# iwanders/spread_spectrum_watermarking

Hardware: AMD Instinct MI355X
Metric: Mpixels/sec embed+extract (4K batch) (higher is better)
Workload: dtype f64

## Files before the change

### include/ssw.h

```cpp
#ifndef SSW_H
#define SSW_H

#include <stddef.h>
#include <stdint.h>

#ifdef __cplusplus
extern "C" {
#endif

typedef enum ssw_status {
    SSW_OK = 0,
    SSW_ERR_BAD_ARG = 1,
    SSW_ERR_BAD_DIMS = 2,
    SSW_ERR_LENGTH_MISMATCH = 3,
    SSW_ERR_K_TOO_LARGE = 4,
    SSW_ERR_NOT_BASE = 5,
    SSW_ERR_UNSUPPORTED = 6,
    SSW_ERR_CONSUMED = 7,
    SSW_ERR_HIP = 8,
    SSW_ERR_NO_DEVICE = 9,
    SSW_ERR_OUT_OF_MEMORY = 10
} ssw_status;

typedef enum ssw_ordering {
    SSW_ORDER_ENERGY = 0,
    SSW_ORDER_ENERGY_ORTHOGONAL = 1,
    SSW_ORDER_LEGACY = 2,
    SSW_ORDER_CUSTOM = 3
} ssw_ordering;

typedef enum ssw_method {
    SSW_OPTION1 = 1,
    SSW_OPTION2 = 2,
    SSW_OPTION3 = 3,
    SSW_METHOD_CUSTOM = 4
} ssw_method;

typedef enum ssw_dct_type {
    SSW_DCT2 = 0,
    SSW_DCT2_ORTHOGONAL = 1,
    SSW_DCT3 = 2
} ssw_dct_type;

typedef enum ssw_precision {
    SSW_PRECISION_F32 = 0,
    SSW_PRECISION_F64 = 1
} ssw_precision;

typedef struct ssw_config {
    int32_t ordering;
    int32_t method;
    float alpha;
    int32_t precision;
} ssw_config;

typedef struct ssw_ctx ssw_ctx;
typedef struct ssw_writer ssw_writer;
typedef struct ssw_reader ssw_reader;

const char* ssw_version(void);
int ssw_build_all_strategies(void);
enum { SSW_PLAN_PAIR_F64 = 1, SSW_PLAN_ROWS_DEEP = 2, SSW_PLAN_COLS_DEEP = 4, SSW_PLAN_ROWS_LEVEL2 = 8, SSW_PLAN_COLS_LEVEL2 = 16,
       SSW_PLAN_CLASS_MAJOR = 32, SSW_PLAN_FUSED_COLS = 64 };
int ssw_ctx_transform_plan(ssw_ctx* ctx, size_t n_frames, size_t w, size_t h, int dct_type, uint32_t* flags);
const char* ssw_status_string(int status);
const char* ssw_last_error(void);
void ssw_config_default(ssw_config* cfg);

int ssw_ctx_create(int device_id, ssw_ctx** out);
int ssw_ctx_destroy(ssw_ctx* ctx);
int ssw_ctx_synchronize(ssw_ctx* ctx);
void* ssw_ctx_stream(ssw_ctx* ctx);
int ssw_ctx_set_stream(ssw_ctx* ctx, void* hip_stream);
int ssw_ctx_wait_event(ssw_ctx* ctx, void* hip_event);
int ssw_ctx_record_event(ssw_ctx* ctx, void* hip_event);
int ssw_ctx_set_chunk_frames(ssw_ctx* ctx, size_t frames);
size_t ssw_ctx_pass_frames(ssw_ctx* ctx, size_t n_frames, size_t w, size_t h);

int ssw_ctx_set_overlap(ssw_ctx* ctx, int enable);
int ssw_ctx_set_prune(ssw_ctx* ctx, int enable);
int ssw_ctx_get_prune_stats(ssw_ctx* ctx, uint64_t* stats);
int ssw_ctx_get_select_stats(ssw_ctx* ctx, uint64_t* stats);

#define SSW_DCT_FOLDING_DEFAULT 5
int ssw_ctx_set_dct_folding(ssw_ctx* ctx, int level);
int ssw_ctx_set_odd_split(ssw_ctx* ctx, int enable);

int ssw_tuning_set(const char* name, long long value);
int ssw_tuning_get(const char* name, long long* value);
int ssw_tuning_reset(const char* name);

typedef enum ssw_stage {
    SSW_STAGE_RGB_TO_YIQ = 0,
    SSW_STAGE_DCT_ROW = 1,
    SSW_STAGE_DCT_COL = 2,
    SSW_STAGE_SELECT = 3,
    SSW_STAGE_EMBED = 4,
    SSW_STAGE_EXTRACT = 5,
    SSW_STAGE_SIMILARITY = 6,
    SSW_STAGE_YIQ_TO_RGB = 7,
    SSW_STAGE_RESIZE = 8,
    SSW_STAGE_CONVERT = 9,
    SSW_STAGE_DCT_PREP = 10,
    SSW_STAGE_DCT_ROW_MAIN = 11,
    SSW_STAGE_DCT_COL_MAIN = 12,
    SSW_STAGE_LOCATE = 13,
    SSW_STAGE_LOCATE_COARSE = 14,
    SSW_STAGE_COUNT = 15
} ssw_stage;
int ssw_ctx_enable_timing(ssw_ctx* ctx, int enable);
int ssw_ctx_reset_timing(ssw_ctx* ctx);
int ssw_ctx_get_timing(ssw_ctx* ctx, double* ms, uint64_t* launches);
int ssw_ctx_get_work(ssw_ctx* ctx, double* work);
int ssw_ctx_get_traffic(ssw_ctx* ctx, double* bytes);

int ssw_dev_mem_info(ssw_ctx* ctx, size_t* free_bytes, size_t* total_bytes);
int ssw_dev_alloc(ssw_ctx* ctx, size_t bytes, void** dev_ptr);
int ssw_dev_free(ssw_ctx* ctx, void* dev_ptr);
int ssw_copy_to_dev(ssw_ctx* ctx, void* dev_dst, const void* host_src, size_t bytes);
int ssw_copy_to_host(ssw_ctx* ctx, void* host_dst, const void* dev_src, size_t bytes);

int ssw_host_alloc(ssw_ctx* ctx, size_t bytes, void** host_ptr);
int ssw_host_free(ssw_ctx* ctx, void* host_ptr);
int ssw_ctx_set_copy_threads(ssw_ctx* ctx, int threads);
typedef enum ssw_transfer_stat {
    SSW_TRANSFER_H2D_BYTES = 0,
    SSW_TRANSFER_D2H_BYTES = 1,
    SSW_TRANSFER_H2D_SECONDS = 2,
    SSW_TRANSFER_D2H_SECONDS = 3,
    SSW_TRANSFER_STAGED_BYTES = 4,
    SSW_TRANSFER_DIRECT_BYTES = 5,
    SSW_TRANSFER_STAT_COUNT = 6
} ssw_transfer_stat;
int ssw_ctx_get_transfer_stats(ssw_ctx* ctx, double* stats, int reset);


int ssw_rgb_to_yiq(ssw_ctx* ctx, const float* dev_rgb, size_t n_frames, size_t w, size_t h,
                   float* dev_y, float* dev_i, float* dev_q);
int ssw_yiq_to_rgb(ssw_ctx* ctx, const float* dev_y, const float* dev_i, const float* dev_q,
                   size_t n_frames, size_t w, size_t h, float* dev_rgb);
int ssw_dct2d(ssw_ctx* ctx, int dct_type, int precision, size_t n_frames, size_t w, size_t h,
              float* dev_planes);

int ssw_topk_indices(ssw_ctx* ctx, const float* dev_coef, size_t n_frames, size_t w, size_t h,
                     int ordering, size_t k, uint32_t* dev_indices);

int ssw_embed_coefficients(ssw_ctx* ctx, float* dev_coef, size_t n_frames, size_t plane_len,
                           const uint32_t* dev_indices, size_t k, int method, float alpha,
                           const float* dev_marks, size_t n_marks);
int ssw_extract_coefficients(ssw_ctx* ctx, const float* dev_base, const float* dev_derived,
                             size_t n_frames, size_t plane_len, const uint32_t* dev_indices,
                             size_t k, int method, float alpha, float* dev_out);
int ssw_similarity_batch(ssw_ctx* ctx, const float* dev_extracted, const float* dev_marks,
                         size_t n_pairs, size_t k, float* dev_sims);

int ssw_similarity_matrix(ssw_ctx* ctx, const float* dev_extracted, size_t n_extracted, const float* dev_marks,
                          size_t n_marks, size_t k, float* dev_sims);

int ssw_batch_embed(ssw_ctx* ctx, const ssw_config* cfg, const float* dev_rgb, size_t n_frames,
                    size_t w, size_t h, const float* dev_marks, size_t k, float* dev_rgb_out,
                    float* dev_coef_out, uint32_t* dev_indices_out);
int ssw_batch_extract(ssw_ctx* ctx, const ssw_config* cfg, const float* dev_base_rgb,
                      const float* dev_derived_rgb, size_t n_frames, size_t w, size_t h, size_t k,
                      float* dev_extracted, const float* dev_marks, float* dev_sims);
// ... 113 lines not shown
```

### spread_spectrum_watermarking_amd/_lib.py

```python
from __future__ import annotations

import ctypes as C
import os

_HERE = os.path.dirname(os.path.abspath(__file__))
LIB_PATH = os.environ.get("SSW_LIB_PATH") or os.path.join(_HERE, "lib", "libssw_hip.so")

SSW_OK = 0
STATUS_NAMES = {
    0: "SSW_OK", 1: "SSW_ERR_BAD_ARG", 2: "SSW_ERR_BAD_DIMS", 3: "SSW_ERR_LENGTH_MISMATCH",
    4: "SSW_ERR_K_TOO_LARGE", 5: "SSW_ERR_NOT_BASE", 6: "SSW_ERR_UNSUPPORTED", 7: "SSW_ERR_CONSUMED",
    8: "SSW_ERR_HIP", 9: "SSW_ERR_NO_DEVICE", 10: "SSW_ERR_OUT_OF_MEMORY",
}
(SSW_ERR_BAD_ARG, SSW_ERR_BAD_DIMS, SSW_ERR_LENGTH_MISMATCH, SSW_ERR_K_TOO_LARGE, SSW_ERR_NOT_BASE,
 SSW_ERR_UNSUPPORTED, SSW_ERR_CONSUMED, SSW_ERR_HIP, SSW_ERR_NO_DEVICE, SSW_ERR_OUT_OF_MEMORY) = range(1, 11)

ORDER_ENERGY, ORDER_ENERGY_ORTHOGONAL, ORDER_LEGACY, ORDER_CUSTOM = 0, 1, 2, 3
OPTION1, OPTION2, OPTION3, METHOD_CUSTOM = 1, 2, 3, 4
DCT2, DCT2_ORTHOGONAL, DCT3 = 0, 1, 2
PRECISION_F32, PRECISION_F64 = 0, 1
STAGES = ["rgb_to_yiq", "dct_row", "dct_col", "select", "embed", "extract", "similarity", "yiq_to_rgb",
          "resize", "convert", "dct_prep", "dct_row_main", "dct_col_main", "locate", "locate_coarse"]
DCT_FOLDING_DEFAULT = 5
TRACE_NONE = 0xFFFFFFFF
PLAN_FLAGS = {"pair_f64": 1, "rows_deep": 2, "cols_deep": 4, "rows_level2": 8, "cols_level2": 16, "class_major": 32, "fused_cols": 64}
TRANSFER_STATS = ["h2d_bytes", "d2h_bytes", "h2d_seconds", "d2h_seconds", "staged_bytes", "direct_bytes"]


class Config(C.Structure):
    _fields_ = [("ordering", C.c_int32), ("method", C.c_int32), ("alpha", C.c_float), ("precision", C.c_int32)]


class Placement(C.Structure):
    _fields_ = [("w", C.c_uint32), ("h", C.c_uint32), ("channels", C.c_uint32),
                ("x", C.c_uint32), ("y", C.c_uint32), ("pw", C.c_uint32), ("ph", C.c_uint32)]


class ScaleRange(C.Structure):
    _fields_ = [("wmin", C.c_uint32), ("wmax", C.c_uint32)]


_vp, _f32p, _u32p, _u64p, _sz = C.c_void_p, C.c_void_p, C.c_void_p, C.c_void_p, C.c_size_t
_cfgp = C.POINTER(Config)
_plp = C.POINTER(Placement)

SIGNATURES = {
    "ssw_version": (C.c_char_p, []),
    "ssw_build_all_strategies": (C.c_int, []),
    "ssw_ctx_transform_plan": (C.c_int, [_vp, _sz, _sz, _sz, C.c_int, C.POINTER(C.c_uint32)]),
    "ssw_status_string": (C.c_char_p, [C.c_int]),
    "ssw_last_error": (C.c_char_p, []),
    "ssw_config_default": (None, [_cfgp]),
    "ssw_ctx_create": (C.c_int, [C.c_int, C.POINTER(_vp)]),
    "ssw_ctx_destroy": (C.c_int, [_vp]),
    "ssw_ctx_synchronize": (C.c_int, [_vp]),
    "ssw_ctx_stream": (_vp, [_vp]),
    "ssw_ctx_set_stream": (C.c_int, [_vp, _vp]),
    "ssw_ctx_wait_event": (C.c_int, [_vp, _vp]),
    "ssw_ctx_record_event": (C.c_int, [_vp, _vp]),
    "ssw_ctx_set_chunk_frames": (C.c_int, [_vp, _sz]),
    "ssw_ctx_pass_frames": (_sz, [_vp, _sz, _sz, _sz]),
    "ssw_ctx_set_dct_folding": (C.c_int, [_vp, C.c_int]),
    "ssw_ctx_enable_timing": (C.c_int, [_vp, C.c_int]),
    "ssw_ctx_reset_timing": (C.c_int, [_vp]),
    "ssw_ctx_get_timing": (C.c_int, [_vp, C.POINTER(C.c_double), C.POINTER(C.c_uint64)]),
    "ssw_ctx_get_work": (C.c_int, [_vp, C.POINTER(C.c_double)]),
    "ssw_ctx_get_traffic": (C.c_int, [_vp, C.POINTER(C.c_double)]),
    "ssw_ctx_set_overlap": (C.c_int, [_vp, C.c_int]),
    "ssw_ctx_set_prune": (C.c_int, [_vp, C.c_int]),
    "ssw_ctx_set_odd_split": (C.c_int, [_vp, C.c_int]),
    "ssw_tuning_set": (C.c_int, [C.c_char_p, C.c_longlong]),
    "ssw_tuning_get": (C.c_int, [C.c_char_p, C.POINTER(C.c_longlong)]),
    "ssw_tuning_reset": (C.c_int, [C.c_char_p]),
    "ssw_ctx_get_prune_stats": (C.c_int, [_vp, C.POINTER(C.c_uint64)]),
    "ssw_ctx_get_select_stats": (C.c_int, [_vp, C.POINTER(C.c_uint64)]),
    "ssw_dev_mem_info": (C.c_int, [_vp, C.POINTER(_sz), C.POINTER(_sz)]),
    "ssw_dev_alloc": (C.c_int, [_vp, _sz, C.POINTER(_vp)]),
    "ssw_dev_free": (C.c_int, [_vp, _vp]),
    "ssw_copy_to_dev": (C.c_int, [_vp, _vp, _vp, _sz]),
    "ssw_copy_to_host": (C.c_int, [_vp, _vp, _vp, _sz]),
    "ssw_host_alloc": (C.c_int, [_vp, _sz, C.POINTER(_vp)]),
    "ssw_host_free": (C.c_int, [_vp, _vp]),
    "ssw_ctx_set_copy_threads": (C.c_int, [_vp, C.c_int]),
    "ssw_ctx_get_transfer_stats": (C.c_int, [_vp, C.POINTER(C.c_double), C.c_int]),
    "ssw_rgb_to_yiq": (C.c_int, [_vp, _f32p, _sz, _sz, _sz, _f32p, _f32p, _f32p]),
    "ssw_yiq_to_rgb": (C.c_int, [_vp, _f32p, _f32p, _f32p, _sz, _sz, _sz, _f32p]),
    "ssw_dct2d": (C.c_int, [_vp, C.c_int, C.c_int, _sz, _sz, _sz, _f32p]),
    "ssw_topk_indices": (C.c_int, [_vp, _f32p, _sz, _sz, _sz, C.c_int, _sz, _u32p]),
    "ssw_embed_coefficients": (C.c_int, [_vp, _f32p, _sz, _sz, _u32p, _sz, C.c_int, C.c_float, _f32p, _sz]),
    "ssw_extract_coefficients": (C.c_int, [_vp, _f32p, _f32p, _sz, _sz, _u32p, _sz, C.c_int, C.c_float, _f32p]),
    "ssw_similarity_batch": (C.c_int, [_vp, _f32p, _f32p, _sz, _sz, _f32p]),
    "ssw_similarity_matrix": (C.c_int, [_vp, _f32p, _sz, _f32p, _sz, _sz, _f32p]),
    "ssw_batch_embed": (C.c_int, [_vp, _cfgp, _f32p, _sz, _sz, _sz, _f32p, _sz, _f32p, _f32p, _u32p]),
    "ssw_batch_extract": (C.c_int, [_vp, _cfgp, _f32p, _f32p, _sz, _sz, _sz, _sz, _f32p, _f32p, _f32p]),
    "ssw_convert_rgb8_to_f32": (C.c_int, [_vp, _vp, _sz, _f32p]),
    "ssw_convert_f32_to_rgb8": (C.c_int, [_vp, _f32p, _sz, _vp]),
    "ssw_resize_rgb8": (C.c_int, [_vp, _vp, _sz, _sz, _sz, _sz, _sz, _vp]),
    "ssw_batch_embed_rgb8": (C.c_int, [_vp, _cfgp, _vp, _sz, _sz, _sz, _f32p, _sz, _vp]),
    "ssw_batch_embed_host_rgb8": (C.c_int, [_vp, _cfgp, C.POINTER(_vp), _sz, _sz, _sz, _f32p, _sz, C.POINTER(_vp)]),
    "ssw_batch_extract_host_rgb8": (C.c_int, [_vp, _cfgp, C.POINTER(_vp), C.POINTER(_vp), _sz, _sz, _sz, _sz, _f32p, _f32p, _f32p]),
    "ssw_convert_rgb16_to_f32": (C.c_int, [_vp, _vp, _sz, _f32p]),
    "ssw_convert_f32_to_rgb16": (C.c_int, [_vp, _f32p, _sz, _vp]),
    "ssw_batch_embed_rgb16": (C.c_int, [_vp, _cfgp, _vp, _sz, _sz, _sz, _f32p, _sz, _f32p]),
    "ssw_batch_extract_rgb16": (C.c_int, [_vp, _cfgp, _vp, _vp, _sz, _sz, _sz, _sz, _f32p, _f32p, _f32p]),
    "ssw_batch_extract_rgb8": (C.c_int, [_vp, _cfgp, _vp, _vp, _sz, _sz, _sz, _sz, _f32p, _f32p, _f32p]),
    "ssw_writer_create": (C.c_int, [_vp, _vp, _sz, _sz, _cfgp, C.POINTER(_vp)]),
    "ssw_writer_create_rgb8": (C.c_int, [_vp, _vp, _sz, _sz, _cfgp, C.POINTER(_vp)]),
    "ssw_writer_create_rgb16": (C.c_int, [_vp, _vp, _sz, _sz, _cfgp, C.POINTER(_vp)]),
    "ssw_writer_coefficients": (C.c_int, [_vp, _vp]),
    "ssw_writer_embed": (C.c_int, [_vp, C.POINTER(_vp), C.POINTER(_sz), _sz]),
    "ssw_writer_result": (C.c_int, [_vp, _vp]),
    "ssw_writer_mark": (C.c_int, [_vp, C.POINTER(_vp), C.POINTER(_sz), _sz, _vp]),
    "ssw_writer_result_rgb8": (C.c_int, [_vp, _vp]),
    "ssw_writer_mark_rgb8": (C.c_int, [_vp, C.POINTER(_vp), C.POINTER(_sz), _sz, _vp]),
    "ssw_fingerprint_embed": (C.c_int, [_vp, _cfgp, _f32p, _sz, _sz, _f32p, _sz, _sz, _f32p, _u32p]),
    "ssw_fingerprint_embed_rgb8": (C.c_int, [_vp, _cfgp, _vp, _sz, _sz, _f32p, _sz, _sz, _vp, _u32p]),
    "ssw_fingerprint_trace": (C.c_int, [_vp, _cfgp, _f32p, _f32p, _sz, _sz, _sz, _sz, _f32p, _sz, C.c_float, _f32p, _f32p, _u32p, _f32p, _u32p]),
    "ssw_fingerprint_trace_rgb8": (C.c_int, [_vp, _cfgp, _vp, _vp, _sz, _sz, _sz, _sz, _f32p, _sz, C.c_float, _f32p, _f32p, _u32p, _f32p, _u32p]),
    "ssw_fingerprint_trace_host_rgb8": (C.c_int, [_vp, _cfgp, _vp, C.POINTER(_vp), _sz, _sz, _sz, _sz, _f32p, _sz, C.c_float, _f32p, _f32p, _u32p,
                                                  _f32p, _u32p]),
    "ssw_reader_trace_host_rgb8": (C.c_int, [_vp, C.POINTER(_vp), _sz, _sz, _f32p, _sz, C.c_float, _f32p, _f32p, _u32p, _f32p, _u32p]),
    "ssw_restore_rgb8": (C.c_int, [_vp, _vp, _sz, _sz, C.POINTER(_vp), _plp, _sz, _vp]),
    "ssw_locate_rgb8": (C.c_int, [_vp, _vp, _sz, _sz, C.POINTER(_vp), _plp, _sz, C.POINTER(C.c_uint64)]),
    "ssw_locate_scaled_rgb8": (C.c_int, [_vp, _vp, _sz, _sz, C.POINTER(_vp), _plp, C.POINTER(ScaleRange), _sz, C.POINTER(C.c_uint64)]),
    "ssw_locate_rung_boxes": (C.c_int, [_vp, _vp, _sz, _sz, _sz, _sz, _sz, _vp]),
    "ssw_fingerprint_trace_restored_host_rgb8": (C.c_int, [_vp, _cfgp, _vp, _sz, _sz, C.POINTER(_vp), _plp, _sz, _sz, _f32p, _sz, C.c_float,
                                                           _f32p, _f32p, _u32p, _f32p, _u32p]),
    "ssw_reader_trace_restored_host_rgb8": (C.c_int, [_vp, _vp, C.POINTER(_vp), _plp, _sz, _sz, _f32p, _sz, C.c_float, _f32p, _f32p, _u32p,
                                                      _f32p, _u32p]),
    "ssw_writer_mark_copies": (C.c_int, [_vp, _f32p, _sz, _sz, _vp]),
    "ssw_writer_mark_copies_rgb8": (C.c_int, [_vp, _f32p, _sz, _sz, _vp]),
    "ssw_writer_destroy": (C.c_int, [_vp]),
    "ssw_reader_create": (C.c_int, [_vp, _vp, _sz, _sz, C.c_int, _cfgp, C.POINTER(_vp)]),
    "ssw_reader_create_rgb8": (C.c_int, [_vp, _vp, _sz, _sz, C.c_int, _cfgp, C.POINTER(_vp)]),
    "ssw_reader_create_rgb16": (C.c_int, [_vp, _vp, _sz, _sz, C.c_int, _cfgp, C.POINTER(_vp)]),
    "ssw_reader_coefficients": (C.c_int, [_vp, _vp]),
    "ssw_reader_indices": (C.c_int, [_vp, _sz, _vp]),
    "ssw_reader_extract": (C.c_int, [_vp, _vp, _vp, _sz]),
    "ssw_reader_destroy": (C.c_int, [_vp]),
    "ssw_similarity": (C.c_int, [_vp, _vp, _sz, _vp, _sz, C.POINTER(C.c_float)]),
    "ssw_synth_frames": (C.c_int, [_vp, C.c_uint32, C.c_uint32, _sz, _sz, _sz, _f32p]),
}

_lib = None


class SswLibraryMissing(ImportError):
    pass


def load() -> C.CDLL:
    global _lib
    if _lib is not None:
        return _lib
    if not os.path.exists(LIB_PATH):
        raise SswLibraryMissing(
            f"{LIB_PATH} not found: build it with `python -c 'import __graft_entry__ as g; g.build()'` "
# ... 28 lines not shown
```

### spread_spectrum_watermarking_amd/api.py

```python
from __future__ import annotations

import ctypes as C
import math
from dataclasses import dataclass, field
from typing import Callable, Optional, Sequence, Tuple

import numpy as np

from . import _lib as L
from ._lib import SswError, check


class Context:

    def __init__(self, device_id: int = 0):
        self._lib = L.load()
        h = C.c_void_p()
        check(self._lib.ssw_ctx_create(device_id, C.byref(h)), "ssw_ctx_create")
        self.handle = h
        self.device_id = device_id

    def close(self):
        if getattr(self, "handle", None):
            self._lib.ssw_ctx_destroy(self.handle)
            self.handle = None

    def __del__(self):
        try:
            self.close()
        except Exception:
            pass

    def synchronize(self):
        check(self._lib.ssw_ctx_synchronize(self.handle), "ssw_ctx_synchronize")

    def set_stream(self, hip_stream=None):
        check(self._lib.ssw_ctx_set_stream(self.handle, C.c_void_p(hip_stream) if hip_stream else None), "ssw_ctx_set_stream")

    def wait_event(self, hip_event):
        check(self._lib.ssw_ctx_wait_event(self.handle, C.c_void_p(hip_event)), "ssw_ctx_wait_event")

    def record_event(self, hip_event):
        check(self._lib.ssw_ctx_record_event(self.handle, C.c_void_p(hip_event)), "ssw_ctx_record_event")

    def set_chunk_frames(self, n: int):
        check(self._lib.ssw_ctx_set_chunk_frames(self.handle, n), "ssw_ctx_set_chunk_frames")

    def pass_frames(self, n_frames: int, w: int, h: int) -> int:
        return int(self._lib.ssw_ctx_pass_frames(self.handle, n_frames, w, h))

    def set_dct_folding(self, level=True):
        lvl = (L.DCT_FOLDING_DEFAULT if level else 0) if isinstance(level, bool) else int(level)
        check(self._lib.ssw_ctx_set_dct_folding(self.handle, lvl), "ssw_ctx_set_dct_folding")

    def enable_timing(self, on: bool = True):
        check(self._lib.ssw_ctx_enable_timing(self.handle, int(on)), "ssw_ctx_enable_timing")

    def reset_timing(self):
        check(self._lib.ssw_ctx_reset_timing(self.handle), "ssw_ctx_reset_timing")

    def timing(self) -> dict:
        ms = (C.c_double * len(L.STAGES))()
        n = (C.c_uint64 * len(L.STAGES))()
        work = (C.c_double * len(L.STAGES))()
        check(self._lib.ssw_ctx_get_timing(self.handle, ms, n), "ssw_ctx_get_timing")
        check(self._lib.ssw_ctx_get_work(self.handle, work), "ssw_ctx_get_work")
        traffic = (C.c_double * len(L.STAGES))()
        check(self._lib.ssw_ctx_get_traffic(self.handle, traffic), "ssw_ctx_get_traffic")
        return {s: {"ms": ms[i], "launches": int(n[i]), "work": work[i], "bytes": traffic[i]} for i, s in enumerate(L.STAGES)}

    def transform_plan(self, n_frames: int, w: int, h: int, dct_type: int = L.DCT2) -> dict:
        f = C.c_uint32()
        check(self._lib.ssw_ctx_transform_plan(self.handle, n_frames, w, h, dct_type, C.byref(f)), "ssw_ctx_transform_plan")
        return {name: bool(f.value & bit) for name, bit in L.PLAN_FLAGS.items()}

    def set_overlap(self, on: bool = True):
        check(self._lib.ssw_ctx_set_overlap(self.handle, int(on)), "ssw_ctx_set_overlap")

    def set_prune(self, on: bool = True):
        check(self._lib.ssw_ctx_set_prune(self.handle, int(on)), "ssw_ctx_set_prune")

    def set_odd_split(self, on: bool = True):
        check(self._lib.ssw_ctx_set_odd_split(self.handle, int(on)), "ssw_ctx_set_odd_split")

    def prune_stats(self) -> dict:
        st = (C.c_uint64 * 3)()
        check(self._lib.ssw_ctx_get_prune_stats(self.handle, st), "ssw_ctx_get_prune_stats")
        return {"pruned_chunks": int(st[0]), "redone_chunks": int(st[1]), "columns_needed": int(st[2])}

    def select_stats(self) -> dict:
        st = (C.c_uint64 * 2)()
        check(self._lib.ssw_ctx_get_select_stats(self.handle, st), "ssw_ctx_get_select_stats")
        return {"frames": int(st[0]), "exact_fallback_frames": int(st[1])}

    def set_copy_threads(self, n: int = 0):
        check(self._lib.ssw_ctx_set_copy_threads(self.handle, int(n)), "ssw_ctx_set_copy_threads")

    def transfer_stats(self, reset: bool = False) -> dict:
        st = (C.c_double * len(L.TRANSFER_STATS))()
        check(self._lib.ssw_ctx_get_transfer_stats(self.handle, st, int(reset)), "ssw_ctx_get_transfer_stats")
        return {n: float(st[i]) for i, n in enumerate(L.TRANSFER_STATS)}

    def pinned_empty(self, shape, dtype) -> np.ndarray:
        dt = np.dtype(dtype)
        n = int(np.prod(shape)) * dt.itemsize
        p = C.c_void_p()
        check(self._lib.ssw_host_alloc(self.handle, n, C.byref(p)), "ssw_host_alloc")
        return np.asarray(_PinnedBlock(self, p, n))[:n].view(dt).reshape(shape)

    def mem_info(self):
        free, total = C.c_size_t(), C.c_size_t()
        check(self._lib.ssw_dev_mem_info(self.handle, C.byref(free), C.byref(total)), "ssw_dev_mem_info")
        return int(free.value), int(total.value)

    def alloc(self, nbytes: int) -> "DeviceBuffer":
        return DeviceBuffer(self, nbytes)

    def to_device(self, array: np.ndarray) -> "DeviceBuffer":
        a = np.ascontiguousarray(array)
        buf = DeviceBuffer(self, a.nbytes)
        check(self._lib.ssw_copy_to_dev(self.handle, buf.ptr, a.ctypes.data, a.nbytes), "ssw_copy_to_dev")
        return buf


class _PinnedBlock:

    def __init__(self, ctx: Context, ptr, nbytes: int):
        self.ctx, self.ptr, self.nbytes = ctx, ptr, nbytes
        self.__array_interface__ = {"data": (int(ptr.value), False), "shape": (max(nbytes, 1),), "typestr": "|u1", "version": 3}

    def __del__(self):
        try:
            if self.ptr and self.ctx.handle:
                self.ctx._lib.ssw_host_free(self.ctx.handle, self.ptr)
            self.ptr = None
        except Exception:
            pass


class DeviceBuffer:
    def __init__(self, ctx: Context, nbytes: int):
        self.ctx, self.nbytes = ctx, nbytes
        p = C.c_void_p()
        check(ctx._lib.ssw_dev_alloc(ctx.handle, nbytes, C.byref(p)), "ssw_dev_alloc")
        self.ptr = p

    def to_host(self, dtype, shape) -> np.ndarray:
        out = np.empty(shape, dtype)
        assert out.nbytes <= self.nbytes
        check(self.ctx._lib.ssw_copy_to_host(self.ctx.handle, out.ctypes.data, self.ptr, out.nbytes), "ssw_copy_to_host")
        return out

    def free(self):
        if self.ptr and self.ctx.handle:
            self.ctx._lib.ssw_dev_free(self.ctx.handle, self.ptr)
        self.ptr = None

    def __del__(self):
        try:
            self.free()
        except Exception:
            pass


_default_ctx: Optional[Context] = None


class tuning:

    def __init__(self, **values):
        self._values = values
# ... 644 lines not shown
```

### spread_spectrum_watermarking_amd/csrc/dct_pair_common.hpp

```cpp
#pragma once
#include "dct_common.hpp"
#include "dct_pair_class.hpp"

namespace ssw {

typedef unsigned int u32x4 __attribute__((ext_vector_type(4)));
typedef unsigned int u32x2 __attribute__((ext_vector_type(2)));
typedef unsigned int u32x3 __attribute__((ext_vector_type(3)));
template <typename T> using vec4_t = T __attribute__((ext_vector_type(4)));
template <typename T> using vec2_t = T __attribute__((ext_vector_type(2)));

template <typename T> struct KBlock { static constexpr unsigned KB = 64 / sizeof(T); };
template <typename T>
__host__ __device__ inline size_t blk_index(size_t line, unsigned k, size_t rows) {
    constexpr unsigned KB = KBlock<T>::KB;
    return ((size_t)(k / KB) * rows + line) * KB + (k % KB);
}

template <typename T>
struct PairOutT {
    float* out;
    T* tmp;
    unsigned W, H;
    unsigned n;
    unsigned c1, c2, cs;
    const float* iq_i = nullptr;
    const float* iq_q = nullptr;
    void* rgb = nullptr;
    unsigned rgb_u8 = 0;
    unsigned wide = 0;
    unsigned bn32 = 0;
    unsigned pm = 0;
    unsigned np1 = 0xFFFFFFFFu, p2lo = 0;
    unsigned fold0 = 0;
    T* tmp_out = nullptr;
    unsigned cm = 0;
    unsigned tcm = 0;
    unsigned cmt = 0;
    unsigned ft = 0, gsh = 31, e2off = 0;
    T* cop = nullptr;
    unsigned cop_k16 = 0, cop_lines = 0, cop_hup = 0;
    const double *crot1 = nullptr, *crot2 = nullptr, *crot3 = nullptr;
    unsigned xperm = 0;
};

struct ForwardClassLayout {
    unsigned n, t;
    bool level2;
    enum { R1 = 0, R2, E2P, E2M, O2P, O2M, EP, EM, OP, OM, NCLASS1 };
    enum { R1A = 0, R1B, R2A, R2B, F_E2P, F_E2M, F_O2P, F_O2M, EEP, EEM, EOP, EOM, O5, O11, O3, O13, NCLASS2 };
    __host__ __device__ ForwardClassLayout(unsigned n_, unsigned t_ = 0, bool level2_ = false) : n(n_), t(t_ ? t_ : n_), level2(level2_) {}
    __host__ __device__ int classes() const { return level2 ? (int)NCLASS2 : (int)NCLASS1; }
    __host__ __device__ unsigned mod(int c) const { return level2 ? 16u : ((c >= E2P && c <= O2M) ? 16u : 8u); }
    __host__ __device__ unsigned res(int c) const {
        if (level2) {
            const unsigned char r[16] = {0, 8, 4, 12, 2, 14, 10, 6, 1, 15, 9, 7, 5, 11, 3, 13};
            return r[c & 15];
        }
        const unsigned char r[10] = {0, 4, 2, 14, 10, 6, 1, 7, 5, 3};
        return r[c];
    }
    __host__ __device__ unsigned group(int c) const { return t / mod(c); }
    __host__ __device__ unsigned base(int c) const {
        const unsigned e = t / 8, s = t / 16;
        if (level2) return (unsigned)c * s;
        return c < 2 ? c * e : c < 6 ? 2 * e + (c - 2) * s : t / 2 + (c - 6) * e;
    }
    __host__ __device__ unsigned pos(int c, unsigned i) const {
        const unsigned g = group(c);
        return (i / g) * t + base(c) + i % g;
    }
    __host__ __device__ unsigned natural(unsigned p) const {
        const unsigned e = t / 8, s = t / 16, tb = (p / t) * t;
        p -= tb;
        int c;
        unsigned i;
        if (level2) { c = (int)(p / s); i = p - c * s; }
        else if (p < 2 * e) { c = (int)(p / e); i = p - c * e; }
        else if (p < t / 2) { const unsigned q = p - 2 * e; c = 2 + (int)(q / s); i = q - (q / s) * s; }
        else { const unsigned q = p - t / 2; c = 6 + (int)(q / e); i = q - (q / e) * e; }
        return tb + mod(c) * i + res(c);
    }
};
__host__ __device__ inline unsigned class_tile(unsigned n) { return n % 128 == 0 ? 128u : n; }

__host__ __device__ inline unsigned inverse_class_pos(unsigned m, unsigned len, unsigned t = 0, bool l2 = false) {
    t = t ? t : len;
    const unsigned tb = (m / t) * t, r = m - tb;
    if (l2) {
        const unsigned run = (0x17523460u >> (4 * (r & 7u))) & 7u;
        return tb + run * (t / 8) + (r >> 3);
    }
    const unsigned c = r & 3u, q = t / 4;
    return tb + (c == 0 ? 0u : c == 3 ? q : c == 1 ? 2 * q : 3 * q) + (r >> 2);
}
__host__ __device__ inline unsigned inverse_class_natural(unsigned p, unsigned len, unsigned t = 0, bool l2 = false) {
    t = t ? t : len;
    const unsigned tb = (p / t) * t, r = p - tb;
    if (l2) {
        const unsigned q = t / 8, run = r / q, i = r - run * q;
        return tb + 8 * i + ((0x61523470u >> (4 * run)) & 7u);
    }
    const unsigned q = t / 4, c = r / q, i = r - c * q;
    return tb + 4 * i + (c == 0 ? 0u : c == 1 ? 3u : c == 2 ? 1u : 2u);
}

__device__ inline float pair_clamp01(float x) {
    if (x < 0.0f) return 0.0f;
    if (x > 1.0f) return 1.0f;
    return x;
}
template <typename T, int NB>
__device__ inline void pair_store_rgb_batch(const PairOutT<T>& po, size_t base, const unsigned (&px)[NB], const float (&y)[NB], bool ok) {
    if (!ok) return;
    const float* __restrict__ ip = po.iq_i + base;
    const float* __restrict__ qp = po.iq_q + base;
    float iv[NB], qv[NB];
#pragma unroll
    for (int t = 0; t < NB; ++t) {
        iv[t] = ip[px[t]];
        qv[t] = qp[px[t]];
    }
#pragma unroll
    for (int t = 0; t < NB; ++t) {
        const float r = pair_clamp01(1.0f * y[t] + 0.948262f * iv[t] + 0.624013f * qv[t]);
        const float g = pair_clamp01(1.0f * y[t] + -0.276066f * iv[t] + -0.639810f * qv[t]);
// ... 61 lines not shown
```

### spread_spectrum_watermarking_amd/csrc/dct_pair_f64.hip

```cpp
#include "dct_pair_common.hpp"

#include <cstdlib>
#include <type_traits>

#ifdef SSW_TILE_TRACE
namespace ssw {
__device__ unsigned long long* g_tile_trace = nullptr;
__device__ unsigned int g_tile_trace_cap = 0;
__device__ unsigned int g_tile_trace_n = 0;
__device__ unsigned int* g_tile_kstep = nullptr;
extern "C" int ssw_debug_set_tile_kstep(void* dev_ptr) {
    unsigned int* p = static_cast<unsigned int*>(dev_ptr);
    return hipMemcpyToSymbol(HIP_SYMBOL(g_tile_kstep), &p, sizeof(p)) == hipSuccess ? 0 : -1;
}
extern "C" int ssw_debug_set_tile_trace(void* dev_ptr, unsigned cap) {
    unsigned long long* p = static_cast<unsigned long long*>(dev_ptr);
    unsigned zero = 0;
    if (hipMemcpyToSymbol(HIP_SYMBOL(g_tile_trace), &p, sizeof(p)) != hipSuccess) return -1;
    if (hipMemcpyToSymbol(HIP_SYMBOL(g_tile_trace_cap), &cap, sizeof(cap)) != hipSuccess) return -1;
    if (hipMemcpyToSymbol(HIP_SYMBOL(g_tile_trace_n), &zero, sizeof(zero)) != hipSuccess) return -1;
    return 0;
}
extern "C" int ssw_debug_get_tile_trace_count(unsigned* n) {
    return hipMemcpyFromSymbol(n, HIP_SYMBOL(g_tile_trace_n), sizeof(*n)) == hipSuccess ? 0 : -1;
}
}
#endif
#include "dct_pair_f64_kernel.hpp"
#if defined(SSW_TILE_TRACE) && !defined(SSW_TILE_TRACE_FWD_ONLY)
#define SSW_INV_PART -1
#include "dct_pair_f64_inv.inc"
#endif

namespace ssw {



int launch_dct_pair_gemm_multi_f64(hipStream_t st, bool is_row, bool inverse, int n_classes, const PairClassDesc* desc, float* out,
                                   double* tmp, size_t n_frames, size_t w, size_t h, Epilogue ep, const RgbSink* sink, double* tmp_out,
                                   const PairLayout& lay, const FuseCols* fuse) {
    if (n_frames == 0 || n_classes == 0) return SSW_OK;
    if (n_classes < 0 || n_classes > 8 || !desc) return SSW_ERR_BAD_ARG;
    if (w > 0xFFFFFFull || h > 0xFFFFFFull) return SSW_ERR_BAD_DIMS;
    const bool fuse_rows = fuse && fuse->mode == FUSE_ROWS_COP, fuse_cols = fuse && fuse->mode == FUSE_COLS;
    if (fuse && (!(fuse_rows || fuse_cols) || fuse_rows != is_row || inverse || w % 128 != 0 || h % 16 != 0 ||
                 pair_kpad(h / 8) != dct_pair_fused_units(h))) return SSW_ERR_BAD_ARG;
    if (fuse_rows && (!lay.class_major || sink || !fuse->cop || !fuse->rot1 || !fuse->rot2 || !fuse->rot3)) return SSW_ERR_BAD_ARG;
    const size_t lines = fuse_rows ? n_frames * 16 * dct_pair_fused_units(h) : is_row ? n_frames * h : n_frames * w;
    const size_t len = is_row ? w : h;
    if (lines > 0xFFFFFFFFull) return SSW_ERR_BAD_DIMS;
    const unsigned L = (unsigned)lines;
    const bool with_sink = sink && sink->rgb;
    PairMulti ml;
    PairInstance inst{0, false, 0};
    unsigned tiles_n = 0, leff0 = 0;
    const bool tile48 = tuning(TUNE_TILE48) != 0;
    for (int c = 0; c < n_classes; ++c) {
        PairInstance ic{0, false, 0};
        PairClassArgs& ca = ml.c[c];
        SSW_TRY(pair_class_args(desc[c].cls, is_row, inverse, len, lay, with_sink, tmp_out != nullptr, tile48, ca, ic));
        ca.x1 = desc[c].x1; ca.x2 = desc[c].x2; ca.y1 = desc[c].y1; ca.y2 = desc[c].y2;
        const unsigned ninv = inverse ? (unsigned)(len / pair_class_row(desc[c].cls).inv_ndiv) : 0u;
        if (c == 0) { inst = ic; leff0 = ninv; }
        else if (!(ic == inst) && !(ic.epi == inst.epi && ic.samex == inst.samex && n_classes > 1)) return SSW_ERR_BAD_ARG;
        if (ninv != leff0) return SSW_ERR_BAD_ARG;
        if ((unsigned long long)ml.c[c].Kp * L * 8 > 0xFFFFFFFFull) return SSW_ERR_BAD_DIMS;
        tiles_n += ml.c[c].tiles_n;
    }
    if (n_classes > 1) inst.subname = inverse ? inst.subname : 3;
    const bool small = (unsigned long long)((L + 127) / 128) * tiles_n < 448;
    if (fuse && small) return SSW_ERR_BAD_ARG;
    const unsigned BM = small ? 64 : 128;
    if (small)
        for (int c = 0; c < n_classes; ++c)
            if (ml.c[c].bn32 == 2) { tiles_n -= ml.c[c].tiles_n; ml.c[c].bn32 = 0; ml.c[c].tiles_n = (ml.c[c].NP + 63) / 64; tiles_n += ml.c[c].tiles_n; }
    const unsigned tiles_m = (L + BM - 1) / BM;
    if (small && n_classes == 1) {
        const int force = (int)tuning(TUNE_BN32);
        auto balance = [](unsigned long long n) { return (double)n / (256.0 * (double)((n + 255) / 256)); };
        const unsigned tn32 = (ml.c[0].NP + 31) / 32;
        const bool bn32 = force >= 0 ? force != 0 : 0.92 * balance((unsigned long long)tiles_m * tn32) > balance((unsigned long long)tiles_m * tiles_n);
        if (bn32) { ml.c[0].tiles_n = tiles_n = tn32; ml.c[0].bn32 = 1; }
    }
    const unsigned long long nblk = (unsigned long long)tiles_m * tiles_n;
    if (nblk > 0x7FFFFFFFull) return SSW_ERR_BAD_DIMS;
    ml.n_classes = (unsigned)n_classes; ml.L = L; ml.tiles_m = tiles_m; ml.tiles_n_total = tiles_n;
    PairOut po{out, tmp, (unsigned)w, (unsigned)h, (unsigned)(inverse ? leff0 : len), 0, 1, 2};
    po.tmp_out = tmp_out;
    const PairClass c0 = desc[0].cls;
    if (lay.class_major && inverse && pair_class_row(c0).split && c0 != PairClass::R2A) { po.cm = lay.rows_l2 ? 2u : 1u; po.cmt = lay.tile; }
    if (lay.class_major && inverse && c0 == PairClass::R2A) po.cm = 1;
    if (lay.class_major && inverse && is_row && lay.rows_l2 && (c0 == PairClass::E2 || c0 == PairClass::O2)) po.tcm = 1;
    if (lay.class_major && !inverse) po.ft = lay.tile;
    if (fuse_rows) {
        if (inst.samex || inst.epi != EPI_FWD || po.ft != 128) return SSW_ERR_BAD_ARG;
        po.cop = fuse->cop; po.cop_k16 = (unsigned)pair_kpad(h / 8); po.cop_lines = (unsigned)(n_frames * w);
        po.cop_hup = (unsigned)dct_pair_fused_units(h);
        po.crot1 = fuse->rot1; po.crot2 = fuse->rot2; po.crot3 = fuse->rot3;
        inst.epi = EPI_FWD_COLOP;
    }
    if (fuse_cols) po.xperm = 1;
    auto al = [](const void* p, unsigned a) { return (reinterpret_cast<uintptr_t>(p) & (a - 1)) == 0; };
    po.wide = (!is_row && w % 4 == 0 && al(out, 16) && (n_frames * w) % 4 == 0 && (!tmp || al(tmp, 16)) && (!tmp_out || al(tmp_out, 16))) ? 1u : 0u;
    if (with_sink && !(al(sink->iq_i, 16) && al(sink->iq_q, 16) && al(sink->rgb, sink->u8 ? 4 : 16))) po.wide = 0;
    if (with_sink) {
        if (is_row) return SSW_ERR_BAD_ARG;
        po.iq_i = sink->iq_i; po.iq_q = sink->iq_q; po.rgb = sink->rgb; po.rgb_u8 = sink->u8 ? 1u : 0u;
    }
    ml.po = po;
    switch (inst.epi) {
    case EPI_FWD_COLOP:
        if (inst.subname == 4) SSW_LAUNCH_PAIR_BM(false, EPI_FWD_COLOP, false, 4, 128);
        else SSW_LAUNCH_PAIR_BM(false, EPI_FWD_COLOP, false, 3, 128);
        break;
    case EPI_FWD_ADJ: SSW_LAUNCH_PAIR(false, EPI_FWD_ADJ, false); break;
    case EPI_FWD:
        if (inst.subname == 4) SSW_LAUNCH_PAIR_SUB(false, EPI_FWD, false, 4);
        else if (inst.subname == 3) { if (is_row) SSW_LAUNCH_PAIR_SUB(false, EPI_FWD, false, 3); else SSW_LAUNCH_PAIR_SUB(true, EPI_FWD, false, 3); }
        else if (inst.samex) SSW_LAUNCH_ROWCOL(EPI_FWD, true);
        else SSW_LAUNCH_ROWCOL(EPI_FWD, false);
        break;
    default: return launch_pair_gemm_inverse_instances(st, ml, ep, inst, is_row, small, nblk);
    }
    SSW_HIP_CHECK(hipGetLastError());
    return SSW_OK;
}

int launch_dct_pair_gemm_rows_subset_f64(hipStream_t st, const double* x, const double* y, unsigned cap, unsigned Kp, float* out,
                                         unsigned out_stride, unsigned off, size_t lines) {
    if (lines == 0 || cap == 0) return SSW_OK;
    if (lines > 0xFFFFFFFFull || (cap & 1)) return SSW_ERR_BAD_DIMS;
    const unsigned L = (unsigned)lines, NP = cap / 2;
    const unsigned tiles_m = (L + 127) / 128, tiles_n = (NP + 63) / 64;
    const unsigned long long nblk = (unsigned long long)tiles_m * tiles_n;
    if (nblk > 0x7FFFFFFFull) return SSW_ERR_BAD_DIMS;
    if ((unsigned long long)Kp * L * sizeof(double) > 0xFFFFFFFFull) return SSW_ERR_BAD_DIMS;
    PairMulti ml;
    ml.c[0] = PairClassArgs{x, x, y, y + (size_t)NP * 8, NP, Kp, cap, tiles_n, off, off + NP, 1, 0, 0xFFFFFFFFu, 0, 0, 0};
    ml.n_classes = 1; ml.L = L; ml.tiles_m = tiles_m; ml.tiles_n_total = tiles_n;
    ml.po = PairOut{out, nullptr, out_stride, 0, 0, off, off + NP, 1};
    const Epilogue ep{1.f, 1.f};
    pair_gemm_f64_kernel<false, EPI_FWD, true, 2><<<(unsigned)nblk, PT, 0, st>>>(ml, ep);
    SSW_HIP_CHECK(hipGetLastError());
    return SSW_OK;
}

int launch_dct_pair_gemm_rows_subset_split_f64(hipStream_t st, const double* x1, const double* x2, const double* y1, const double* y2,
                                               unsigned cap, unsigned Kp, float* out, unsigned out_stride, unsigned off, size_t lines) {
    if (lines == 0 || cap == 0) return SSW_OK;
    if (lines > 0xFFFFFFFFull) return SSW_ERR_BAD_DIMS;
    const unsigned L = (unsigned)lines, NP = cap;
    const unsigned tiles_m = (L + 127) / 128, tiles_n = (NP + 63) / 64;
    const unsigned long long nblk = (unsigned long long)tiles_m * tiles_n;
    if (nblk > 0x7FFFFFFFull) return SSW_ERR_BAD_DIMS;
    if ((unsigned long long)Kp * L * sizeof(double) > 0xFFFFFFFFull) return SSW_ERR_BAD_DIMS;
    PairMulti ml;
    ml.c[0] = PairClassArgs{x1, x2, y1, y2, NP, Kp, cap, tiles_n, off, 0, 1, 2, 0xFFFFFFFFu, 0, 0, 0};
    ml.n_classes = 1; ml.L = L; ml.tiles_m = tiles_m; ml.tiles_n_total = tiles_n;
    ml.po = PairOut{out, nullptr, out_stride, 0, 0, off, 0, 1};
    const Epilogue ep{1.f, 1.f};
    pair_gemm_f64_kernel<false, EPI_FWD, false, 3><<<(unsigned)nblk, PT, 0, st>>>(ml, ep);
    SSW_HIP_CHECK(hipGetLastError());
    return SSW_OK;
}

int launch_dct_pair_gemm_rows_subset_merged_f64(hipStream_t st, const PairSubsetClass* classes, unsigned n_classes, float* out,
                                                unsigned out_stride, size_t lines) {
    if (lines == 0) return SSW_OK;
    if (lines > 0xFFFFFFFFull) return SSW_ERR_BAD_DIMS;
    const unsigned L = (unsigned)lines, tiles_m = (L + 127) / 128;
    for (int split = 0; split < 2; ++split) {
        PairMulti ml;
        ml.n_classes = 0; ml.L = L; ml.tiles_m = tiles_m; ml.tiles_n_total = 0;
        auto flush = [&]() -> int {
            if (ml.n_classes == 0) return SSW_OK;
            const unsigned long long nblk = (unsigned long long)tiles_m * ml.tiles_n_total;
            if (nblk > 0x7FFFFFFFull) return SSW_ERR_BAD_DIMS;
            ml.po = PairOut{out, nullptr, out_stride, 0, 0, 0, 0, 1};
            const Epilogue ep{1.f, 1.f};
            if (split) pair_gemm_f64_kernel<false, EPI_FWD, false, 3><<<(unsigned)nblk, PT, 0, st>>>(ml, ep);
            else       pair_gemm_f64_kernel<false, EPI_FWD, true, 2><<<(unsigned)nblk, PT, 0, st>>>(ml, ep);
            SSW_HIP_CHECK(hipGetLastError());
            ml.n_classes = 0; ml.tiles_n_total = 0;
            return SSW_OK;
        };
        for (unsigned c = 0; c < n_classes; ++c) {
            const PairSubsetClass& k = classes[c];
            if ((k.x2 != nullptr) != (split != 0) || k.cap == 0) continue;
            if (!split && (k.cap & 1)) return SSW_ERR_BAD_DIMS;
            if ((unsigned long long)k.Kp * L * sizeof(double) > 0xFFFFFFFFull) return SSW_ERR_BAD_DIMS;
            const unsigned NP = split ? k.cap : k.cap / 2, tiles_n = (NP + 63) / 64;
            if (split) ml.c[ml.n_classes] = PairClassArgs{k.x1, k.x2, k.y1, k.y2, NP, k.Kp, k.cap, tiles_n, k.off, 0, 1, 2, 0xFFFFFFFFu, 0, 0, 0};
            else       ml.c[ml.n_classes] = PairClassArgs{k.x1, k.x1, k.y1, k.y1 + (size_t)NP * 8, NP, k.Kp, k.cap, tiles_n, k.off, k.off + NP, 1, 0, 0xFFFFFFFFu, 0, 0, 0};
            ml.tiles_n_total += tiles_n;
            if (++ml.n_classes == 8) SSW_TRY(flush());
        }
        SSW_TRY(flush());
    }
    return SSW_OK;
}
// ... 3 lines not shown
```

### spread_spectrum_watermarking_amd/csrc/dct_pair_f64_kernel.hpp

```cpp
#pragma once
#include "dct_pair_common.hpp"
#include "dct_pair_colops.hpp"

#include <cstdlib>
#include <type_traits>


namespace ssw {

constexpr int PT = 256;
constexpr int PBK = 8;
constexpr int RGB_NB = 2;

#ifdef SSW_TILE_TRACE
#define SSW_TT(i) do { if (threadIdx.x == 0) tt[i] = wall_clock64(); } while (0)
#define SSW_KT(t) do { if (threadIdx.x == 0 && (t) < 32u) kst_lds[t] = (unsigned)wall_clock64(); } while (0)
#else
#define SSW_TT(i) do { } while (0)
#define SSW_KT(t) do { } while (0)
#endif
typedef PairOutT<double> PairOut;


struct PairMulti {
    PairClassArgs c[8];
    unsigned n_classes, L, tiles_m, tiles_n_total;
    PairOut po;
};

template <bool COLS, int EPI, bool SAMEX, int SUB = 0, int BM = 128>
__global__ __launch_bounds__(PT, 2) void pair_gemm_f64_kernel(const PairMulti ml, Epilogue ep) {
#if defined(__HIP_DEVICE_COMPILE__)
    constexpr int NX = SAMEX ? 1 : 2;
    constexpr int BN = 64, XQ = BM / 64;
    constexpr int STG = NX * BM * PBK + 2 * BN * PBK;
    constexpr int SXD = 2 * STG;
    constexpr int TRD = COLS ? 4 * 32 * (BM / 2 + 16) / 2 : 0;
#ifdef SSW_TILE_TRACE
    __shared__ __attribute__((aligned(16))) double lds[(SXD > TRD ? SXD : TRD) + 16];
    unsigned* kst_lds = reinterpret_cast<unsigned*>(lds + (SXD > TRD ? SXD : TRD));
#else
    __shared__ __attribute__((aligned(16))) double lds[SXD > TRD ? SXD : TRD];
#endif

#ifdef SSW_TILE_TRACE
    unsigned long long tt[5] = {0, 0, 0, 0, 0};
    const unsigned long long cyc0 = clock64();
    unsigned kslot = 0xFFFFFFFFu;
    if (threadIdx.x == 0 && g_tile_trace) kslot = atomicAdd(&g_tile_trace_n, 1u);
#endif
    SSW_TT(0);
    unsigned tm, tn, cls = 0;
    tile_of_block(blockIdx.x, gridDim.x, ml.tiles_m, ml.tiles_n_total, tm, tn);
    while (cls + 1 < ml.n_classes && tn >= ml.c[cls].tiles_n) { tn -= ml.c[cls].tiles_n; ++cls; }
    const PairClassArgs& ca = ml.c[cls];
    const double* __restrict__ X1g = ca.x1;
    const double* __restrict__ X2g = ca.x2;
    const double* __restrict__ Y1g = ca.y1;
    const double* __restrict__ Y2g = ca.y2;
    const unsigned L = ml.L, NP = ca.NP, Kp = ca.Kp, yrows = ca.yrows;
    PairOut po = ml.po;
    po.c1 = ca.c1; po.c2 = ca.c2; po.cs = ca.cs; po.pm = ca.pm; po.np1 = ca.np1; po.p2lo = ca.p2lo; po.bn32 = ca.bn32; po.fold0 = ca.fold0;
    po.gsh = ca.gsh; po.e2off = ca.e2off;
    const unsigned m0 = tm * BM, p0 = tn * (po.bn32 == 1 ? 32u : po.bn32 == 2 ? 48u : (unsigned)BN);
    const unsigned tid = threadIdx.x;
    const unsigned lane = tid & 63, wave = tid >> 6;
    const unsigned li = lane & 15, lq = lane >> 4;

    const unsigned wv = (unsigned)__builtin_amdgcn_readfirstlane((int)wave);
    const unsigned drow = 16 * wave + (lane >> 2), dch = lane & 3;
    unsigned xoff[XQ];
#pragma unroll
    for (int q = 0; q < XQ; ++q) {
        const unsigned j = drow + 64 * q;
        unsigned r = m0 + ((COLS && BM == 128 && po.xperm) ? fwd_cm128_pos(j) : j);
        r = r < L ? r : L - 1;
        xoff[q] = (r - m0) * 64u + 16u * (dch ^ ((j >> 2) & 3u));
    }
    unsigned yr = p0 + drow;
    yr = yr < NP ? yr : NP - 1;
    const unsigned yoff = (yr - p0) * 64u + 16u * (dch ^ ((drow >> 2) & 3u));
#ifdef SSW_ABL_X0
    const size_t m0x = 0;
#else
    const size_t m0x = m0;
#endif
    const __amdgpu_buffer_rsrc_t x1r = __builtin_amdgcn_make_buffer_rsrc((void*)(X1g + m0x * 8), 0, 0xFFFFFFFFu, 0x00020000);
    const __amdgpu_buffer_rsrc_t x2r = __builtin_amdgcn_make_buffer_rsrc((void*)(X2g + m0x * 8), 0, 0xFFFFFFFFu, 0x00020000);
    const __amdgpu_buffer_rsrc_t y1r = __builtin_amdgcn_make_buffer_rsrc((void*)(Y1g + (size_t)p0 * 8), 0, 0xFFFFFFFFu, 0x00020000);
    const __amdgpu_buffer_rsrc_t y2r = __builtin_amdgcn_make_buffer_rsrc((void*)(Y2g + (size_t)p0 * 8), 0, 0xFFFFFFFFu, 0x00020000);
    const unsigned xstep = L * 64u, ystep = yrows * 64u;

    constexpr int LPT = XQ * NX + 2;
    typedef __attribute__((address_space(3))) void* lds_ptr_t;
    auto issue = [&](unsigned t, unsigned sb) {
        const unsigned xadv = t * xstep, yadv = t * ystep;
        double* b = lds + sb + 16 * wv * PBK;
#pragma unroll
        for (int q = 0; q < XQ; ++q) {
            __builtin_amdgcn_raw_ptr_buffer_load_lds(x1r, (lds_ptr_t)(b + 64 * q * PBK), 16, xoff[q], xadv, 0, 0);
            if (!SAMEX) __builtin_amdgcn_raw_ptr_buffer_load_lds(x2r, (lds_ptr_t)(b + BM * PBK + 64 * q * PBK), 16, xoff[q], xadv, 0, 0);
        }
        __builtin_amdgcn_raw_ptr_buffer_load_lds(y1r, (lds_ptr_t)(b + NX * BM * PBK), 16, yoff, yadv, 0, 0);
        __builtin_amdgcn_raw_ptr_buffer_load_lds(y2r, (lds_ptr_t)(b + NX * BM * PBK + BN * PBK), 16, yoff, yadv, 0, 0);
    };
    auto run = [&](auto nic, auto njc) {
    constexpr int NI = decltype(nic)::value;
    constexpr int NJ = decltype(njc)::value;
    constexpr int NJA = NJ < 2 ? 2 : NJ;
    constexpr bool FULL = NI == BM / 32;
    const unsigned wm = FULL ? (wave >> 1) * (BM / 2) : wave * (BM / 4), wn = FULL ? (wave & 1) * 32 : 0;
    f64x4 acc1[NI][NJA], acc2[NI][NJA];
#pragma unroll
    for (int i = 0; i < NI; ++i)
#pragma unroll
        for (int j = 0; j < NJA; ++j) { acc1[i][j] = (f64x4){0, 0, 0, 0}; acc2[i][j] = (f64x4){0, 0, 0, 0}; }

    const unsigned fsw = (li >> 2) & 3;
    unsigned rdx[2], rdy[2];
#pragma unroll
    for (int sh = 0; sh < 2; ++sh) {
        rdx[sh] = (wm + li) * PBK + 2 * ((2 * sh + (lq >> 1)) ^ fsw) + (lq & 1);
        rdy[sh] = NX * BM * PBK + (wn + li) * PBK + 2 * ((2 * sh + (lq >> 1)) ^ fsw) + (lq & 1);
    }
    struct Frag { double x1[NI], x2[NI], y1[NJA], y2[NJA]; };
    auto fread = [&](unsigned sb, auto shc, Frag& f) {
        constexpr int sh = decltype(shc)::value;
        const double* b = lds + sb;
#pragma unroll
        for (int jn = 0; jn < NJ; ++jn) {
            f.y1[jn] = b[rdy[sh] + 16 * jn * PBK];
            f.y2[jn] = b[rdy[sh] + BN * PBK + 16 * jn * PBK];
        }
#pragma unroll
        for (int i = 0; i < NI; ++i) {
            f.x1[i] = b[rdx[sh] + 16 * i * PBK];
            if (!SAMEX) f.x2[i] = b[rdx[sh] + BM * PBK + 16 * i * PBK];
// ... 109 lines not shown
                    double s = a1 + a2, d = a1 - a2;
                    if (jn == 0 && has0) {
                        const bool p = COLS ? (lq == 0 && r == 0) : (li == 0);
                        s = p ? a1 : s;
                        d = p ? 0.0 - a2 : d;
                    }
                    acc1[i][jn][r] = s;
                    acc2[i][jn][r] = d;
                }
    }
    const bool second_out = po.pm != 2;
    auto p2 = [&](unsigned pair) { return (po.fold0 && pair == 0) ? po.fold0 : pair; };

    const unsigned n = po.n, W = po.W, H = po.H;
    auto opos = [&](unsigned m, unsigned len) { return (!COLS && po.cm) ? inverse_class_pos(m, len, 0, po.cm == 2) : m; };
    auto tpos = [&](unsigned m) { return (!COLS && po.tcm) ? inverse_class_pos(m, n / 2, 0, false) : m; };
    auto oposf = [&](unsigned m, unsigned len) { return (!COLS && po.cm) ? inverse_class_pos(m, len, po.cmt, po.cm == 2) : m; };
    auto fpos1 = [&](unsigned pair) {
        return po.ft ? po.c1 + (pair >> po.gsh) * po.ft + (pair & ((1u << po.gsh) - 1u)) : po.c1 + po.cs * pair;
    };
    auto fpos2 = [&](unsigned pair) {
        const unsigned q = p2(pair), e = q - po.e2off;
        return po.ft ? po.c2 + (e >> po.gsh) * po.ft + (e & ((1u << po.gsh) - 1u)) : po.c2 + po.cs * q;
    };
    auto emit = [&](float* lp, double* tp, double* to, unsigned es, unsigned pair, double a1, double a2) {
        if (EPI == EPI_FWD || EPI == EPI_FWD_ADJ) {
            const unsigned i1 = fpos1(pair), i2 = fpos2(pair);
            if (EPI == EPI_FWD_ADJ) {
                const f32x2 v = {apply_epilogue(ep, (float)a1, i1), apply_epilogue(ep, (float)a2, i2)};
                *reinterpret_cast<f32x2*>(lp + i1) = v;
            } else {
                if (pair < po.np1) lp[i1 * es] = apply_epilogue(ep, (float)a1, i1);
                if (pair >= po.p2lo && second_out) lp[i2 * es] = apply_epilogue(ep, (float)a2, i2);
            }
        } else if (EPI == EPI_INV) {
            lp[pair * es] = apply_epilogue(ep, (float)(a1 + a2), pair);
            lp[(n - 1 - pair) * es] = apply_epilogue(ep, (float)(a1 - a2), n - 1 - pair);
        } else if (EPI == EPI_INV_E) {
            tp[pair * es] = a1 + a2;
            tp[(n / 2 - 1 - pair) * es] = a1 - a2;
        } else if (EPI == EPI_INV_OT) {
            const unsigned n1 = po.c1 + po.cs * pair, n2 = po.c2 + po.cs * p2(pair);
            if (n1 < n / 2) { const double e1 = tp[tpos(n1) * es]; to[opos(n1, n) * es] = e1 + a1; to[opos(n - 1 - n1, n) * es] = e1 - a1; }
            if (n2 < n / 2) { const double e2 = tp[tpos(n2) * es]; to[opos(n2, n) * es] = e2 + a2; to[opos(n - 1 - n2, n) * es] = e2 - a2; }
        } else {
            const unsigned n1 = po.c1 + po.cs * pair, n2 = po.c2 + po.cs * p2(pair);
            if (n1 < n / 2) {
                const double e1 = tp[opos(n1, n / 2) * es];
                lp[oposf(n1, n) * es] = apply_epilogue(ep, (float)(e1 + a1), n1);
                lp[oposf(n - 1 - n1, n) * es] = apply_epilogue(ep, (float)(e1 - a1), n - 1 - n1);
            }
            if (n2 < n / 2) {
                const double e2 = tp[opos(n2, n / 2) * es];
                lp[oposf(n2, n) * es] = apply_epilogue(ep, (float)(e2 + a2), n2);
                lp[oposf(n - 1 - n2, n) * es] = apply_epilogue(ep, (float)(e2 - a2), n - 1 - n2);
            }
        }
    };
    if constexpr (!COLS && EPI == EPI_FWD_COLOP) {
        constexpr int NIT = 32 * NJ, NC = (NIT + 63) / 64;
        constexpr int NPT = FULL ? 64 : 16 * NJ, NLT = 2 * NPT;
        static_assert(4 * NIT * 16 * 4 <= (int)sizeof(lds) && 4 * NLT * 64 <= (int)sizeof(lds), "transpose area, store slabs");
        static_assert(BM == 128, "a tile is one k-block of eight units");
        __syncthreads();
        float* tw = reinterpret_cast<float*>(lds) + wave * (NIT * 16);
        auto lds_order = [&]() {
            __builtin_amdgcn_fence(__ATOMIC_RELEASE, "wavefront");
            __builtin_amdgcn_wave_barrier();
            __builtin_amdgcn_fence(__ATOMIC_ACQUIRE, "wavefront");
        };
        const unsigned Hc = po.H, HU = Hc / 16;
        const unsigned tpf = po.cop_hup / 8;
        const unsigned z = tm / tpf, g = tm - z * tpf;
        const unsigned u0 = (unsigned)__builtin_amdgcn_readfirstlane((int)(wm / 16));
        const bool plain = ep.first == 1.0f && ep.base == 1.0f;
        auto lpos = [&](unsigned f, unsigned v) { return f * 16u + 4u * ((v >> 2) ^ ((f >> 2) & 3u)) + (v & 3u); };
        float f1[NJ], f2[NJ];
#pragma unroll
        for (int jn = 0; jn < NJ; ++jn) {
            const unsigned pair = p0 + wn + 16 * jn + li;
            f1[jn] = fpos1(pair) == 0 ? ep.first : ep.base;
            f2[jn] = fpos2(pair) == 0 ? ep.first : ep.base;
        }
        double o[NC][NI][16];
#pragma unroll
        for (int i = 0; i < NI; ++i) {
            lds_order();
#pragma unroll
            for (int jn = 0; jn < NJ; ++jn)
#pragma unroll
                for (int r = 0; r < 4; ++r) {
                    float v1 = (float)acc1[i][jn][r], v2 = (float)acc2[i][jn][r];
                    if (!plain) { v1 *= f1[jn]; v2 *= f2[jn]; }
                    tw[lpos(32 * jn + li, lq + 4 * r)] = v1;
                    tw[lpos(32 * jn + 16 + li, lq + 4 * r)] = v2;
                }
            lds_order();
            const unsigned e = (unsigned)__builtin_amdgcn_readfirstlane((int)(8 * g + u0 + i));
            const bool unit_ok = e < HU;
            const ColL2Tab tab = col_l2_tab(po.crot1, po.crot2, po.crot3, unit_ok ? e : 0u, Hc);
#pragma unroll
            for (int c = 0; c < NC; ++c) {
                const unsigned f = (lane + 64 * c) < (unsigned)NIT ? lane + 64 * c : 0u;
                float x[16];
#pragma unroll
                for (int q = 0; q < 4; ++q) {
                    const f32x4 t4 = *reinterpret_cast<const f32x4*>(tw + lpos(f, 4 * q));
                    x[4 * q] = t4[0]; x[4 * q + 1] = t4[1]; x[4 * q + 2] = t4[2]; x[4 * q + 3] = t4[3];
                }
                col_l2_unit(x, tab, o[c][i]);
                if (!unit_ok) {
#pragma unroll
                    for (int a = 0; a < 16; ++a) o[c][i][a] = 0.0;
                }
            }
        }
        double* slab = lds;
        unsigned tl[NC];
#pragma unroll
        for (int c = 0; c < NC; ++c) {
            const unsigned f = lane + 64 * c, pl = wn + 16 * (f >> 5) + (f & 15u);
            tl[c] = f < (unsigned)NIT ? 16u * (pl >> 3) + 8u * ((f >> 4) & 1u) + (pl & 7u) : 0u;
        }
        constexpr int NSW = (NLT * 4 + 255) / 256;
        bool st_ok[NSW];
        size_t st_off[NSW];
        unsigned st_lds[NSW];
#pragma unroll
        for (int j = 0; j < NSW; ++j) {
            const unsigned idx = tid + 256 * j, T = idx >> 2, p4 = idx & 3u;
            const unsigned pl = ((T >> 4) << 3) | (T & 7u), pair = p0 + pl;
            const bool second = ((T >> 3) & 1u) != 0;
            st_ok[j] = T < (unsigned)NLT && pair < NP && (second ? (pair >= po.p2lo && second_out) : pair < po.np1);
            const unsigned mc = st_ok[j] ? (second ? fpos2(pair) : fpos1(pair)) : 0u;
            st_off[j] = ((size_t)g * po.cop_lines + (size_t)z * po.W + mc) * 8u + 2u * p4;
            st_lds[j] = (T < (unsigned)NLT ? T : 0u) * 8u + 2u * (p4 ^ ((T >> 2) & 3u));
        }
        const size_t pstride = (size_t)po.cop_lines * po.cop_k16;
#pragma unroll
        for (int rnd = 0; rnd < 4; ++rnd) {
            __syncthreads();
#pragma unroll
            for (int c = 0; c < NC; ++c) {
                if ((lane + 64 * c) >= (unsigned)NIT) continue;
#pragma unroll
                for (int a = 0; a < 4; ++a)
#pragma unroll
                    for (int i = 0; i < NI; i += 2) {
                        const unsigned ch = ((u0 + i) >> 1) ^ ((tl[c] >> 2) & 3u);
                        *reinterpret_cast<f64x2*>(slab + (a * NLT + tl[c]) * 8 + 2 * ch) = (f64x2){o[c][i][4 * rnd + a], o[c][i + 1][4 * rnd + a]};
                    }
            }
            __syncthreads();
#pragma unroll
            for (int j = 0; j < NSW; ++j) {
                if (!st_ok[j]) continue;
#pragma unroll
                for (int a = 0; a < 4; ++a) {
                    const f64x2 v = *reinterpret_cast<const f64x2*>(slab + a * NLT * 8 + st_lds[j]);
                    *reinterpret_cast<f64x2*>(po.cop + (size_t)(4 * rnd + a) * pstride + st_off[j]) = v;
                }
            }
        }
        trace_end();
        return;
    }
    if constexpr (!COLS && (EPI == EPI_FWD || EPI == EPI_INV_O || EPI == EPI_INV_OT)) {
        const unsigned rows_valid = L - m0 < (unsigned)BM ? L - m0 : (unsigned)BM;
        const unsigned long long region = (unsigned long long)rows_valid * W * 4ull;
        if (region < 0x80000000ull && (EPI == EPI_FWD || (EPI == EPI_INV_O && n == W) || EPI == EPI_INV_OT)) {
            constexpr unsigned OOB = 0x80000000u;
            const bool plain = ep.first == 1.0f && ep.base == 1.0f;
            const __amdgpu_buffer_rsrc_t orr = __builtin_amdgcn_make_buffer_rsrc((void*)(po.out + (size_t)m0 * W), 0, (unsigned)region, 0x00020000);
            const unsigned swm = __builtin_amdgcn_readfirstlane(wm);
            auto st = [&](float v, unsigned voff, unsigned soff) {
                __builtin_amdgcn_raw_buffer_store_b32(__float_as_uint(v), orr, voff, soff, 0);
            };
            if constexpr (EPI == EPI_FWD) {
                unsigned vo1[NJ], vo2[NJ];
                float f1[NJ], f2[NJ];
#pragma unroll
                for (int jn = 0; jn < NJ; ++jn) {
                    const unsigned pair = p0 + wn + 16 * jn + li;
                    const unsigned i1 = fpos1(pair), i2 = fpos2(pair);
                    vo1[jn] = (pair < NP && pair < po.np1) ? (lq * W + i1) * 4u : OOB;
                    vo2[jn] = (pair < NP && pair >= po.p2lo && second_out) ? (lq * W + i2) * 4u : OOB;
                    f1[jn] = i1 == 0 ? ep.first : ep.base;
                    f2[jn] = i2 == 0 ? ep.first : ep.base;
                }
#pragma unroll
                for (int i = 0; i < NI; ++i)
#pragma unroll
                    for (int r = 0; r < 4; ++r) {
                        const unsigned soff = (swm + 16 * i + 4 * r) * W * 4u;
#pragma unroll
                        for (int jn = 0; jn < NJ; ++jn) {
                            float v1 = (float)acc1[i][jn][r], v2 = (float)acc2[i][jn][r];
                            if (!plain) { v1 *= f1[jn]; v2 *= f2[jn]; }
                            st(v1, vo1[jn], soff);
                            st(v2, vo2[jn], soff);
                        }
                    }
            } else if constexpr (EPI == EPI_INV_OT) {
                const unsigned tregion = rows_valid * n * 8u;
                const __amdgpu_buffer_rsrc_t irr = __builtin_amdgcn_make_buffer_rsrc((void*)(po.tmp + (size_t)m0 * (n / 2)), 0, tregion / 2, 0x00020000);
                const __amdgpu_buffer_rsrc_t trr = __builtin_amdgcn_make_buffer_rsrc((void*)(po.tmp_out + (size_t)m0 * n), 0, tregion, 0x00020000);
                unsigned vt[NJ][2], vp[NJ][2], vm[NJ][2];
#pragma unroll
                for (int jn = 0; jn < NJ; ++jn) {
                    const unsigned pair = p0 + wn + 16 * jn + li;
#pragma unroll
                    for (int h2 = 0; h2 < 2; ++h2) {
                        const unsigned nn = h2 ? po.c2 + po.cs * p2(pair) : po.c1 + po.cs * pair;
                        const bool ok = pair < NP && nn < n / 2;
                        vt[jn][h2] = ok ? (lq * (n / 2) + tpos(nn)) * 8u : OOB;
                        vp[jn][h2] = ok ? (lq * n + opos(nn, n)) * 8u : OOB;
                        vm[jn][h2] = ok ? (lq * n + opos(n - 1 - nn, n)) * 8u : OOB;
                    }
                }
                auto std64 = [&](double v, unsigned voff, unsigned soff) {
                    const u32x2 raw = {(unsigned)__double2loint(v), (unsigned)__double2hiint(v)};
                    __builtin_amdgcn_raw_buffer_store_b64(raw, trr, voff, soff, 0);
                };
                auto load_e = [&](int i, double (&e)[4][NJ][2]) {
// ... 450 lines not shown
```

### spread_spectrum_watermarking_amd/csrc/select.hip

```cpp
#include "ssw_internal.hpp"
#include "embed_fn.hpp"

#include <atomic>

#include <type_traits>

namespace ssw {

typedef float f32x4 __attribute__((ext_vector_type(4)));

constexpr int DIGIT_BITS = 11;
constexpr int NBINS = 1 << DIGIT_BITS;
constexpr size_t MAX_K = 16384;
constexpr unsigned SAMPLE_STRIDE = 64, SAMPLE_STRIDE_MID = 128, SAMPLE_STRIDE_LONG = 256;
static inline unsigned sample_stride_for(size_t k) { return k >= 8192 ? SAMPLE_STRIDE_LONG : k >= 4096 ? SAMPLE_STRIDE_MID : SAMPLE_STRIDE; }
constexpr unsigned FINISH_THREADS = 1024;

size_t select_max_k() { return MAX_K; }
size_t select_cand_capacity(size_t k) { size_t c = 16 * k; return c < 65536 ? 65536 : c; }

struct KeyParams {
    int ordering;
    unsigned w;
    float s[2][2];
// ... 326 lines not shown
            base = __shfl(base, __builtin_ctzll(m), 64);
            const unsigned pos = base + (unsigned)__popcll(m & ((1ull << lane) - 1ull));
            if (keep && pos < n_pow2) lbuf[pos] = comp;
        };
        walk(take);
        __syncthreads();
        const unsigned gathered = (unsigned)lstate[4];
        for (unsigned i = tid; i < n_pow2; i += blockDim.x)
            if (i >= gathered) lbuf[i] = 0ull;
        __syncthreads();
    }
    if (n_pow2 <= blockDim.x) {
        const unsigned N = blockDim.x;
        uint64_t v = tid < n_pow2 ? lbuf[tid] : 0ull;
        __syncthreads();
        for (unsigned size = 2; size <= N; size <<= 1) {
            const bool up = (tid & size) == 0;
            for (unsigned stride = size >> 1; stride > 0; stride >>= 1) {
                uint64_t other;
                if (stride >= 64) {
                    lbuf[tid] = v;
                    __syncthreads();
                    other = lbuf[tid ^ stride];
                    __syncthreads();
                } else {
                    const uint32_t lo = __shfl_xor((uint32_t)v, (int)stride, 64);
                    const uint32_t hi = __shfl_xor((uint32_t)(v >> 32), (int)stride, 64);
                    other = ((uint64_t)hi << 32) | lo;
                }
                const bool lower = (tid & stride) == 0;
                const uint64_t mx = v > other ? v : other, mn = v > other ? other : v;
                v = (lower == up) ? mx : mn;
            }
        }
        if (tid < k) indices[tid] = ~(uint32_t)(v & 0xFFFFFFFFull);
        return;
    }
    if (blockDim.x == FINISH_THREADS && n_pow2 <= 16 * FINISH_THREADS) {
        const unsigned gathered = (unsigned)lstate[4] < n_pow2 ? (unsigned)lstate[4] : n_pow2;
        const unsigned rows = (gathered + FINISH_THREADS - 1) / FINISH_THREADS;
        block_radix_sort_desc(lbuf, rows, reinterpret_cast<uint16_t*>(lhist), lpart, 0);
        for (unsigned i = tid; i < k; i += blockDim.x) indices[i] = ~(uint32_t)(lbuf[i] & 0xFFFFFFFFull);
        return;
    }
    for (unsigned size = 2; size <= n_pow2; size <<= 1) {
        for (unsigned stride = size >> 1; stride > 0; stride >>= 1) {
            for (unsigned i = tid; i < n_pow2 / 2; i += blockDim.x) {
                const unsigned lo = 2 * i - (i & (stride - 1));
                const unsigned hi = lo + stride;
                const bool desc = ((lo & size) == 0);
                const uint64_t a = lbuf[lo], b = lbuf[hi];
                if ((a < b) == desc) { lbuf[lo] = b; lbuf[hi] = a; }
            }
            __syncthreads();
        }
    }
    for (unsigned i = tid; i < k; i += blockDim.x) indices[i] = ~(uint32_t)(lbuf[i] & 0xFFFFFFFFull);
}

__global__ __launch_bounds__(FINISH_THREADS) void select_finish_kernel(
    const float* __restrict__ coef, size_t plane_len, KeyParams kp, uint32_t* __restrict__ ctrl,
    uint32_t* __restrict__ hist, const uint64_t* __restrict__ cand, size_t cap, size_t k, unsigned n_pow2,
    uint32_t* __restrict__ indices, uint32_t* __restrict__ fallbacks) {
    extern __shared__ __attribute__((aligned(16))) unsigned char smem_raw[];
    uint64_t* lbuf = reinterpret_cast<uint64_t*>(smem_raw);
    uint64_t* lstate = lbuf + (n_pow2 > blockDim.x ? n_pow2 : blockDim.x);
    uint32_t* lhist = reinterpret_cast<uint32_t*>(lstate + 8);
    uint32_t* lpart = lhist + NBINS;
    const size_t f = blockIdx.x;
    const uint32_t n = ctrl[f * 4 + 1];
    __syncthreads();
    for (unsigned i = threadIdx.x; i < NBINS; i += blockDim.x) hist[f * NBINS + i] = 0;
    if (threadIdx.x == 0) { ctrl[f * 4 + 0] = 0; ctrl[f * 4 + 1] = 0; }
    if (n >= k && n <= cap) {
        CandSource src{cand + f * cap};
        block_select_sort(src, n, k, n_pow2, lhist, lpart, lbuf, lstate, indices + f * k);
    } else {
        if (threadIdx.x == 0 && fallbacks) atomicAdd(fallbacks, 1u);
        PlaneSource src{coef + f * plane_len, kp};
        block_select_sort(src, plane_len - 1, k, n_pow2, lhist, lpart, lbuf, lstate, indices + f * k);
    }
}

int launch_topk(hipStream_t st, const float* coef, size_t n_frames, size_t w, size_t h, int ordering,
                size_t k, const SelectWorkspace& ws, uint32_t* indices) {
    const size_t plane_len = w * h;
    if (n_frames == 0 || k == 0) return SSW_OK;
    if (plane_len > 0xFFFFFFFFull) return SSW_ERR_BAD_DIMS;
    if (k > plane_len - 1) return SSW_ERR_K_TOO_LARGE;
    if (k > MAX_K) return SSW_ERR_UNSUPPORTED;
    if (ws.frames < n_frames || ws.cap < select_cand_capacity(k)) return SSW_ERR_BAD_ARG;
    if (ordering < SSW_ORDER_ENERGY || ordering > SSW_ORDER_LEGACY) return SSW_ERR_UNSUPPORTED;

    KeyParams kp;
    kp.ordering = ordering;
    kp.w = (unsigned)w;
    {
        const float s_k0_w = sqrtf(1.0f / (4.0f * (float)w));
        const float s_k0_h = sqrtf(1.0f / (4.0f * (float)h));
        const float s_w = sqrtf(1.0f / (2.0f * (float)w));
        const float s_h = sqrtf(1.0f / (2.0f * (float)h));
        for (int fr = 0; fr < 2; ++fr)
            for (int fc = 0; fc < 2; ++fc) {
                volatile float sc = 1.0f;
                sc = sc * (fr ? s_k0_w : s_w);
                sc = sc * (fc ? s_k0_h : s_h);
                kp.s[fr][fc] = sc;
            }
    }
    const unsigned stride_s = sample_stride_for(k);
    const size_t groups = (plane_len + stride_s * 4 - 1) / (stride_s * 4);
    size_t sb = (groups + 256 * 2 - 1) / (256 * 2);
    if (sb < 1) sb = 1;
    if (sb > 256) sb = 256;

    uint32_t m = (uint32_t)((3 * k + stride_s - 1) / stride_s);
    if (m < 32) m = 32;
    select_sample_kernel<<<dim3((unsigned)sb, (unsigned)n_frames), 256, 0, st>>>(coef, plane_len, kp, ws.hist, stride_s);
    size_t bpf = (plane_len + 256 * 32 - 1) / (256 * 32);
    if (bpf < 1) bpf = 1;
    if (bpf > 2048) bpf = 2048;
    if (ordering == SSW_ORDER_ENERGY)
        select_compact_kernel<true><<<dim3((unsigned)bpf, (unsigned)n_frames), 256, 0, st>>>(coef, plane_len, kp, ws.ctrl, ws.hist, m, ws.cand, ws.cap);
    else
        select_compact_kernel<false><<<dim3((unsigned)bpf, (unsigned)n_frames), 256, 0, st>>>(coef, plane_len, kp, ws.ctrl, ws.hist, m, ws.cand, ws.cap);
    unsigned n_pow2 = 2;
    while (n_pow2 < k) n_pow2 <<= 1;
    const size_t smem = (size_t)(n_pow2 > FINISH_THREADS ? n_pow2 : FINISH_THREADS) * sizeof(uint64_t) + 8 * sizeof(uint64_t) +
                        (NBINS + 256) * sizeof(uint32_t);
    constexpr size_t LDS_LIMIT = 160 * 1024;
    {
        static std::atomic<bool> attr_set[64];
        int dev = 0;
        SSW_HIP_CHECK(hipGetDevice(&dev));
        if (dev < 0 || dev >= 64 || !attr_set[dev].load(std::memory_order_acquire)) {
            SSW_HIP_CHECK(hipFuncSetAttribute(reinterpret_cast<const void*>(select_finish_kernel),
                                              hipFuncAttributeMaxDynamicSharedMemorySize, (int)LDS_LIMIT));
            if (dev >= 0 && dev < 64) attr_set[dev].store(true, std::memory_order_release);
        }
    }
    select_finish_kernel<<<(unsigned)n_frames, FINISH_THREADS, smem, st>>>(coef, plane_len, kp, ws.ctrl, ws.hist,
                                                                            ws.cand, ws.cap, k, n_pow2, indices, ws.fallbacks);
    SSW_HIP_CHECK(hipGetLastError());
    return SSW_OK;
}

__device__ inline float extract_fn(int method, float alpha, float base, float derived) {
    if (method == SSW_OPTION1) return (derived - base) / alpha;
    if (method == SSW_OPTION2) return (derived - base) / (base * alpha);
    return logf(derived / base) / alpha;
}

__global__ __launch_bounds__(256) void embed_kernel(float* __restrict__ coef, size_t plane_len,
                                                    const uint32_t* __restrict__ indices, size_t idx_stride,
                                                    const float* __restrict__ marks,
                                                    const uint32_t* __restrict__ mark_offsets,
                                                    const uint32_t* __restrict__ mark_lens, size_t n_marks,
                                                    size_t max_len, size_t mark_stride, int method, float alpha) {
    const size_t f = blockIdx.y;
    const size_t i = blockIdx.x * (size_t)blockDim.x + threadIdx.x;
    if (i >= max_len) return;
    const uint32_t j = indices[f * idx_stride + i];
    float* c = coef + f * plane_len + j;
    const float original = *c;
    if (n_marks == 1) {
        const size_t off = mark_offsets ? mark_offsets[f] : f * mark_stride;
        const size_t len = mark_lens ? mark_lens[f] : max_len;
        if (i < len) *c = insert_fn(method, alpha, original, marks[off + i]);
    } else {
        float cur = original;
        for (size_t m = 0; m < n_marks; ++m) {
            const size_t off = mark_offsets ? mark_offsets[f * n_marks + m] : (f * n_marks + m) * mark_stride;
            const size_t len = mark_lens ? mark_lens[f * n_marks + m] : max_len;
            if (i < len) {
                const float updated = insert_fn(method, alpha, original, marks[off + i]);
                const float change = updated - original;
                cur += change;
            }
        }
        *c = cur;
    }
}

int launch_embed(hipStream_t st, float* coef, size_t n_frames, size_t plane_len,
                 const uint32_t* indices, size_t idx_stride, const float* marks,
                 const uint32_t* mark_offsets, const uint32_t* mark_lens, size_t n_marks,
                 size_t max_len, size_t mark_stride, int method, float alpha) {
    if (n_frames == 0 || n_marks == 0 || max_len == 0) return SSW_OK;
    const dim3 grid((unsigned)((max_len + 255) / 256), (unsigned)n_frames);
    embed_kernel<<<grid, 256, 0, st>>>(coef, plane_len, indices, idx_stride, marks, mark_offsets,
                                       mark_lens, n_marks, max_len, mark_stride, method, alpha);
    SSW_HIP_CHECK(hipGetLastError());
// ... 242 lines not shown
```

### spread_spectrum_watermarking_amd/csrc/ssw_host.hpp

```cpp
#pragma once

#include <functional>
#include <vector>

#include "ssw_internal.hpp"

namespace ssw {
namespace host {

struct DeviceGuard {
    int prev = -1, dev;
    explicit DeviceGuard(int d) : dev(d) {
        if (hipGetDevice(&prev) != hipSuccess) prev = -1;
        if (prev != dev) (void)hipSetDevice(dev);
    }
    ~DeviceGuard() {
        if (prev >= 0 && prev != dev) (void)hipSetDevice(prev);
    }
    DeviceGuard(const DeviceGuard&) = delete;
    DeviceGuard& operator=(const DeviceGuard&) = delete;
};

struct CtxGuard {
    DeviceGuard dg;
    ssw_ctx* prev;
    explicit CtxGuard(ssw_ctx* ctx);
    ~CtxGuard();
};
size_t plane_pool_flush(ssw_ctx* ctx);

int dev_malloc(void** p, size_t bytes);
#define SSW_ALLOC(pp, bytes) SSW_TRY(::ssw::host::dev_malloc((void**)(pp), (bytes)))
int grow(ssw_ctx::Buf& b, size_t bytes);
void release(ssw_ctx::Buf& b);
int grow_select(hipStream_t st, SelectWorkspace& s, size_t frames, size_t k);
void release_select(SelectWorkspace& s);

int upload(ssw_ctx* ctx, void* dev_dst, const void* host_src, size_t bytes, hipStream_t st);
int download(ssw_ctx* ctx, void* host_dst, const void* dev_src, size_t bytes, hipStream_t st);
int upload_nowait(ssw_ctx* ctx, void* dev_dst, const void* host_src, size_t bytes, hipStream_t st, bool* async_out);
int download_nowait(ssw_ctx* ctx, void* host_dst, const void* dev_src, size_t bytes, hipStream_t st, bool* async_out);
void transfer_destroy(ssw_ctx* ctx);
int transfer_set_threads(ssw_ctx* ctx, int threads);
int transfer_stats(ssw_ctx* ctx, double* out, bool reset);

struct StageTimer {
    ssw_ctx* ctx;
    int stage;
    hipStream_t st;
    hipEvent_t a = nullptr, b = nullptr;
    bool armed = false;
    int alias = -1;
    StageTimer(ssw_ctx* c, int s, hipStream_t stream, double work = 0.0, int alias_stage = -1);
    ~StageTimer();
    void traffic(double bytes);
    StageTimer(const StageTimer&) = delete;
    StageTimer& operator=(const StageTimer&) = delete;
};
int flush_timers(ssw_ctx* ctx);
inline void untimed_work(ssw_ctx* ctx) { if (ctx) ctx->tail_fresh = false; }

int get_basis(ssw_ctx* ctx, size_t n, bool inverse, bool f64, BasisKind kind, const void** out);

bool valid_method(int m);
bool valid_ordering(int o);
bool valid_precision(int p);
int check_config(const ssw_config* cfg);
size_t effective_chunk(const ssw_ctx* ctx, size_t w, size_t h, size_t n_frames);

struct Stage {
    bool hbm;
    std::function<int(hipStream_t)> run;
    int tag = 0;
};
typedef std::vector<Stage> Chain;

struct Xform {
    int type, precision;
    size_t n, w, h;
    float* data;
    float* tmp;
    const void* rgb = nullptr;
    int rgb_u8 = 0;
    float* iq_i = nullptr;
    float* iq_q = nullptr;
    void* rgb_out = nullptr;
    bool rgb_out_u8 = false;
    size_t full_h = 0;
    bool natural_order = false;
};
int build_transform(ssw_ctx* ctx, ssw_ctx::Lane& ws, const Xform& x, Chain& ch, bool* fused_rgb = nullptr);
bool can_fuse_rgb(const ssw_ctx* ctx, bool f64, size_t w, size_t h, const float* y, const float* tmp, const void* rgb, int u8);
int build_forward_from_rgb(ssw_ctx* ctx, ssw_ctx::Lane& ws, int precision, const void* rgb, int u8, size_t n, size_t w,
                           size_t h, float* y, float* i, float* q, float* tmp, Chain& ch);
bool can_split_forward_rows(const ssw_ctx* ctx, bool f64, size_t w, size_t h, size_t bands, const float* y, const float* tmp, const void* rgb, int u8);
int build_forward_rows_band(ssw_ctx* ctx, ssw_ctx::Lane& ws, int precision, const void* rgb, int u8, size_t w, size_t rows,
                            size_t frame_h, float* tmp, float* i, float* q, Chain& ch);
int build_forward_cols_after_rows(ssw_ctx* ctx, ssw_ctx::Lane& ws, int precision, size_t w, size_t h, float* tmp, float* y, Chain& ch);
int run_serial(Chain& ch, hipStream_t st);
int dct2d_planes(ssw_ctx* ctx, int type, int precision, size_t n, size_t w, size_t h, float* data, float* tmp);

int topk(ssw_ctx* ctx, hipStream_t st, SelectWorkspace& sel, const float* coef, size_t n, size_t w, size_t h, int ordering,
         size_t k, uint32_t* idx);

int batch_embed_impl(ssw_ctx* ctx, const ssw_config* cfg, const void* dev_rgb, int u8_in, size_t n_frames, size_t w,
                     size_t h, const float* dev_marks, size_t k, void* dev_rgb_out, bool u8_out, float* dev_coef_out,
                     uint32_t* dev_indices_out);
int batch_extract_impl(ssw_ctx* ctx, const ssw_config* cfg, const void* dev_base_rgb, const void* dev_derived_rgb, int u8,
                       size_t n_frames, size_t w, size_t h, size_t k, float* dev_extracted, const float* dev_marks,
                       float* dev_sims);

int trace_base(ssw_ctx* ctx, const ssw_config& c, const void* dev_base_rgb, int u8, size_t w, size_t h, size_t k, const float** y,
               const uint32_t** idx);
int trace_extract(ssw_ctx* ctx, const ssw_config& c, const float* base_y, const uint32_t* base_idx, const void* dev_suspect_rgb, int u8,
                  size_t n_frames, size_t w, size_t h, size_t k, float* dev_extracted);
int trace_check_args(const ssw_ctx* ctx, const ssw_config* cfg, size_t w, size_t h, size_t k, const void* marks, size_t n_marks,
                     const void* sims, const void* best, const void* best_sim, const void* n_exceed);
int trace_score(ssw_ctx* ctx, const float* dev_extracted, size_t n_suspects, const float* dev_marks, size_t n_marks, size_t k,
                float threshold, float* dev_sims, uint32_t* dev_best, float* dev_best_sim, uint32_t* dev_n_exceed);
int stream_trace_rgb8(ssw_ctx* ctx, const ssw_config& c, const float* base_y, const uint32_t* base_idx, const uint8_t* const* host_suspects,
                      size_t n_suspects, size_t w, size_t h, size_t k, const float* host_marks, size_t n_marks, float threshold,
                      float* host_extracted, float* host_sims, uint32_t* host_best, float* host_best_sim, uint32_t* host_n_exceed,
                      const ssw_placement* placements = nullptr, const uint8_t* dev_base = nullptr);

struct RestoreJob { const uint8_t* src; uint8_t* out; ssw_placement p; };
bool restore_untouched(const ssw_placement& p, size_t w, size_t h);
bool restore_reads_base(const ssw_placement& p, size_t w, size_t h);
int restore_normalise(const ssw_placement* pl, size_t n, size_t w, size_t h, std::vector<ssw_placement>* out);
int restore_prepare(ssw_ctx* ctx, const std::vector<ssw_placement>& pl);
int restore_enqueue(ssw_ctx* ctx, const uint8_t* dev_base, size_t w, size_t h, const RestoreJob* jobs, size_t n);
struct LocWindow { uint32_t x0, x1, y0, y1; bool share; };
int locate_impl(ssw_ctx* ctx, const uint8_t* dev_base, size_t w, size_t h, const void* const* dev_suspects,
                const std::vector<ssw_placement>& pl, uint64_t* host_res, const std::vector<LocWindow>* win = nullptr);
int get_taps(ssw_ctx* ctx, size_t in_len, size_t out_len, DeviceTaps* out);

int fingerprint_copies(ssw_ctx* ctx, const ssw_config& c, const float* coef, const uint32_t* idx, size_t k_eff, const float* iq_i,
                       const float* iq_q, size_t w, size_t h, const float* marks, size_t mark_stride, size_t n_copies, void* out,
                       bool u8_out, float* t32);

int extract_single_pruned(ssw_ctx* ctx, int precision, const void* derived_rgb, int u8, size_t w, size_t h, const float* base_y,
                          const uint32_t* idx, size_t k, int method, float alpha, float* dev_out, uint32_t** dev_info,
                          bool* applicable);

}
}
```

### spread_spectrum_watermarking_amd/csrc/ssw_internal.hpp

```cpp
#pragma once

#include <hip/hip_runtime.h>

#include <cstddef>
#include <cstdint>
#include <map>
#include <string>
#include <tuple>
#include <utility>
#include <vector>

#include "../../include/ssw.h"
#include "dct_plan.hpp"
#include "dct_pair_class.hpp"

namespace ssw {

void set_last_error(const std::string& s);

#define SSW_HIP_CHECK(expr)                                                              \
    do {                                                                                 \
        hipError_t e__ = (expr);                                                         \
        if (e__ != hipSuccess) {                                                         \
            ::ssw::set_last_error(std::string(#expr) + ": " + hipGetErrorString(e__));   \
            return (e__ == hipErrorOutOfMemory) ? SSW_ERR_OUT_OF_MEMORY : SSW_ERR_HIP;   \
        }                                                                                \
    } while (0)

#define SSW_TRY(expr)                         \
    do {                                      \
        int s__ = (expr);                     \
        if (s__ != SSW_OK) return s__;        \
    } while (0)


int launch_rgb_to_yiq(hipStream_t st, const float* rgb, size_t npix, float* y, float* i, float* q);
int launch_yiq_to_rgb(hipStream_t st, const float* y, const float* i, const float* q, size_t npix,
                      float* rgb);
int launch_synth(hipStream_t st, uint32_t seed, uint32_t first_frame, size_t n_frames, size_t w,
                 size_t h, float* rgb);

size_t dense_basis_kpad(size_t n);
int launch_make_basis_f32(hipStream_t st, size_t n, bool inverse, float* out);
int launch_make_basis_f64(hipStream_t st, size_t n, bool inverse, double* out);

struct Epilogue {
    float first, base;
};
int launch_dct_rows(hipStream_t st, int precision, const float* in, float* out, size_t rows, size_t w,
                    const void* basis, Epilogue ep);
int launch_dct_cols(hipStream_t st, int precision, const float* in, float* out, size_t n_frames,
                    size_t w, size_t h, const void* basis, Epilogue ep);
int launch_dct_rows_f64out(hipStream_t st, const float* in, double* out, size_t rows, size_t w, const double* basis);
int launch_dct_cols_f64out(hipStream_t st, const float* in, double* out, size_t n_frames, size_t w, size_t h, const double* basis);

size_t dct_pair_kpad(size_t n);
size_t dct_pair_operand_elems(size_t n_frames, size_t w, size_t h);
int launch_make_half_basis_blocked(hipStream_t st, size_t n, bool inverse, int parity, double* out);
int launch_dct_pair_prep(hipStream_t st, bool is_row, bool inverse, const float* in, size_t n_frames, size_t w, size_t h,
                         double* o1, double* o2);
int launch_dct_pair_prep4(hipStream_t st, bool is_row, bool inverse, const float* in, size_t n_frames, size_t w, size_t h,
                          double* q1, double* q2, double* p);
enum { SSW_PIX_F32 = 0, SSW_PIX_U8 = 1, SSW_PIX_U16 = 2 };
inline size_t pix_bytes(int fmt) { return fmt == SSW_PIX_U8 ? 1 : fmt == SSW_PIX_U16 ? 2 : 4; }
inline unsigned pix_align_mask(int fmt) { return fmt == SSW_PIX_U8 ? 3u : fmt == SSW_PIX_U16 ? 7u : 15u; }
inline int pix_src_kind(int fmt) { return fmt + 1; }
int launch_dct_pair_prep4_rows_rgb(hipStream_t st, int u8, const void* rgb, size_t n_frames, size_t w, size_t h,
                                   double* q1, double* q2, double* p, float* ip, float* qp);
int launch_dct_pair_prep8_rows(hipStream_t st, int src_kind, const void* src, size_t n_frames, size_t w, size_t h,
                               double* r1, double* r2, double* m, double* p, float* ip, float* qp);
struct RgbSink {
    const float* iq_i = nullptr;
    const float* iq_q = nullptr;
    void* rgb = nullptr;
    bool u8 = false;
};
int launch_dct_pair_prep8_cols(hipStream_t st, const float* in, size_t n_frames, size_t w, size_t h,
                               double* r1, double* r2, double* m, double* p);
enum { FUSE_ROWS_COP = 1, FUSE_COLS = 2 };
struct FuseCols { int mode = 0; double* cop = nullptr; const double *rot1 = nullptr, *rot2 = nullptr, *rot3 = nullptr; };
struct PairClassDesc { PairClass cls; const double *x1, *x2, *y1, *y2; };
int launch_dct_pair_gemm_multi_f64(hipStream_t st, bool is_row, bool inverse, int n_classes, const PairClassDesc* desc, float* out,
                                   double* tmp, size_t n_frames, size_t w, size_t h, Epilogue ep, const RgbSink* sink = nullptr,
                                   double* tmp_out = nullptr, const PairLayout& layout = PairLayout(), const FuseCols* fuse = nullptr);

int launch_dct_pair_gemm_rows_subset_f64(hipStream_t st, const double* x, const double* y, unsigned cap, unsigned Kp, float* out,
                                         unsigned out_stride, unsigned off, size_t lines);
int launch_dct_pair_gemm_rows_subset_split_f64(hipStream_t st, const double* x1, const double* x2, const double* y1, const double* y2,
                                               unsigned cap, unsigned Kp, float* out, unsigned out_stride, unsigned off, size_t lines);
struct PairSubsetClass {
    const double *x1, *x2, *y1, *y2;
    unsigned cap, Kp, off;
};
int launch_dct_pair_gemm_rows_subset_merged_f64(hipStream_t st, const PairSubsetClass* classes, unsigned n_classes, float* out,
                                                unsigned out_stride, size_t lines);
size_t dct_pair_split_kpad(size_t len);
enum { TUNE_EFOLD_MIN, TUNE_EFOLD_INV_MIN, TUNE_EFOLD_COLS_MIN, TUNE_CLASS_TILE, TUNE_DEEP_MIN_ROWS, TUNE_DEEP_MIN_COLS, TUNE_PREP_STAGED,
       TUNE_MERGE_MAX_LINES, TUNE_BN32, TUNE_BAND_SPLIT, TUNE_FUSE_COLS, TUNE_UPLOAD_BANDS, TUNE_SPECULATE_K, TUNE_PREP_LIGHT, TUNE_LANE_STAGGER, TUNE_DERIVED_FUSED, TUNE_TILE48, TUNE_COUNT };
long long tuning(int which);
int launch_prep16_cols_l2(hipStream_t st, const float* in, size_t n_frames, size_t w, size_t h, double* base,
                          const double* rot1, const double* rot2, const double* rot3, bool class_major, bool in_l2, unsigned K16);
int launch_prep16_inv_cols_l2(hipStream_t st, const float* in, size_t n_frames, size_t w, size_t h, double* base,
                              const double* rot1, const double* rot2, const double* rot3, bool class_major, bool in_l2, unsigned K16);
int launch_prep16_cols_staged(hipStream_t st, const float* in, size_t n_frames, size_t w, size_t h, double* base,
                              const double* rot1, const double* rot2, bool class_major, bool semi, unsigned K8, unsigned K16, bool efold);
int launch_prep16_inv_cols_staged(hipStream_t st, const float* in, size_t n_frames, size_t w, size_t h, double* base,
                                  const double* rot1, const double* rot2, bool class_major, bool semi, unsigned K8, unsigned K16, bool l2);
int launch_prep16_inv_rows_l2(hipStream_t st, const float* in, size_t rows, size_t w, double* base,
                              const double* rot1, const double* rot2, const double* rot3, unsigned K16);
int launch_prep16_inv_rows_staged(hipStream_t st, const float* in, size_t rows, size_t w, double* base,
                                  const double* rot1, const double* rot2, unsigned K8, unsigned K16);
size_t dct_pair_split_elems(size_t n_frames, size_t w, size_t h);
size_t dct_pair_split_basis_rows(size_t len, int which);
int launch_make_split_basis_blocked(hipStream_t st, size_t n, bool inverse, int which, double* out);
int launch_make_rot_table(hipStream_t st, size_t n, double* out);
int launch_dct_pair_rotate(hipStream_t st, const double* p, const double* rot, double* sp, size_t lines, size_t len);
size_t dct_pair_semi_deep_elems(size_t lines, size_t len);
int launch_dct_pair_prep16_inv_rows(hipStream_t st, const float* in, size_t n_frames, size_t w, size_t h, double* base,
                                    const double* rot1, const double* rot2, const double* rot3, PrepFamily prep);
int launch_dct_pair_prep16_inv_cols(hipStream_t st, const float* in, size_t n_frames, size_t w, size_t h, double* base,
                                    const double* rot1, const double* rot2, const double* rot3, PrepFamily prep, const PairLayout& lay);
int launch_dct_pair_prep16_cols(hipStream_t st, const float* in, size_t n_frames, size_t w, size_t h, double* base,
                                const double* rot1, const double* rot2, const double* rot3, PrepFamily prep, const PairLayout& lay);
size_t dct_pair_deep_elems(size_t lines, size_t len);
int launch_dct_pair_prep16_rows(hipStream_t st, int src_kind, const void* src, size_t n_frames, size_t w, size_t h, double* base,
                                const double* rot1, const double* rot2, const double* rot3, float* ip, float* qp, bool l2, bool unit_order = false);
inline size_t dct_pair_fused_units(size_t h) { return ((h / 16 + 7) / 8) * 8; }

constexpr unsigned PRUNE_NO_REM = 0xFFFFFFFFu;
constexpr uint32_t PRUNE_NEG = 0x40000000u;
constexpr unsigned SSW_PRUNE_INFO = 16;
struct PruneClass { unsigned mod, rem, cap, off, rem2 = PRUNE_NO_REM, radd = 0; };
struct PrunePlan {
    unsigned n_classes = 0;
    PruneClass c[9];
    unsigned W = 0, cap_total = 0;
};
static_assert(SSW_PRUNE_INFO >= 1 + sizeof(PrunePlan::c) / sizeof(PruneClass), "a chunk's info block holds the flag and one count per class");
int launch_prune_build(hipStream_t st, const uint32_t* idx, size_t n_frames, size_t k, const PrunePlan& plan,
                       uint32_t* flag , uint32_t* rows , uint32_t* pos , uint32_t* info );
struct PruneGatherJob {
    const uint32_t* rows;
    const char* src;
    char* dst;
    unsigned cap, src_rows, kblocks, first_block;
    bool negate;
    bool frag = false;
};
struct PruneGatherJobs {
    PruneGatherJob j[18];
    unsigned n;
};
int launch_prune_gather_bases(hipStream_t st, PruneGatherJobs jobs);
int launch_extract_pruned(hipStream_t st, const float* base, const float* compact, size_t n_frames, size_t w, size_t h,
                          size_t cap, const uint32_t* pos, const uint32_t* indices, size_t k, int method, float alpha,
                          float* out);

struct SelectWorkspace {
    uint32_t* hist = nullptr;
    uint32_t* ctrl = nullptr;
    uint64_t* cand = nullptr;
    size_t frames = 0, cap = 0;
    uint32_t* fallbacks = nullptr;
};
size_t select_cand_capacity(size_t k);
size_t select_max_k();
int launch_topk(hipStream_t st, const float* coef, size_t n_frames, size_t w, size_t h, int ordering,
                size_t k, const SelectWorkspace& ws, uint32_t* indices);
struct ResizeTaps {
    uint32_t max_taps = 0;
    std::vector<uint32_t> left, count;
    std::vector<float> weights;
};
struct DeviceTaps {
    uint32_t* left = nullptr;
    uint32_t* count = nullptr;
    float* weights = nullptr;
    uint32_t max_taps = 0;
    uint32_t span[8] = {0};
    bool quad_uniform = false;
};
void build_resize_taps(size_t in_len, size_t out_len, ResizeTaps& t);
int launch_u8_to_f32(hipStream_t st, const uint8_t* in, size_t n, float* out);
int launch_f32_to_u8(hipStream_t st, const float* in, size_t n, uint8_t* out);
int launch_rgb8_to_yiq(hipStream_t st, const uint8_t* rgb, size_t npix, float* y, float* i, float* q);
int launch_u16_to_f32(hipStream_t st, const uint16_t* in, size_t n, float* out);
int launch_f32_to_u16(hipStream_t st, const float* in, size_t n, uint16_t* out);
int launch_rgb16_to_yiq(hipStream_t st, const uint16_t* rgb, size_t npix, float* y, float* i, float* q);
int launch_yiq_to_rgb8(hipStream_t st, const float* y, const float* i, const float* q, size_t npix, uint8_t* rgb);
size_t resize_tmp_bytes(const uint8_t* in, size_t n_frames, size_t w, size_t h, size_t nw, size_t nh, const DeviceTaps& vt,
                        const DeviceTaps& ht, const uint8_t* out);
int launch_resize_rgb8(hipStream_t st, const uint8_t* in, size_t n_frames, size_t w, size_t h, size_t nw, size_t nh,
                       const DeviceTaps& vt, const DeviceTaps& ht, float* tmp, uint8_t* out);

int full_sort_scratch_bytes(size_t plane_len, size_t n_frames, size_t* bytes);
int launch_full_sort(hipStream_t st, const float* coef, size_t n_frames, size_t w, size_t h, int ordering, void* scratch,
                     size_t scratch_bytes, uint32_t* indices_out, size_t k);
int launch_embed(hipStream_t st, float* coef, size_t n_frames, size_t plane_len,
                 const uint32_t* indices, size_t idx_stride, const float* marks,
                 const uint32_t* mark_offsets, const uint32_t* mark_lens, size_t n_marks,
                 size_t max_len, size_t mark_stride , int method, float alpha);
int launch_extract(hipStream_t st, const float* base, const float* derived, size_t n_frames,
                   size_t plane_len, const uint32_t* indices, size_t k, int method, float alpha,
                   float* out);
int launch_similarity(hipStream_t st, const float* extracted, const float* marks, size_t n_pairs,
                      size_t k, float* sims);
int launch_extract_shared(hipStream_t st, const float* base, const float* derived, size_t n_frames, size_t plane_len,
                          const uint32_t* indices, size_t k, int method, float alpha, float* out);
int launch_extract_shared_pruned(hipStream_t st, const float* base, const float* compact, size_t n_frames, size_t w, size_t h,
                                 size_t cap, const uint32_t* pos, const uint32_t* indices, size_t k, int method, float alpha,
                                 float* out);
int launch_trace_finish(hipStream_t st, const float* sims, size_t n_rows, size_t n_marks, float threshold, const float* extracted,
                        const float* marks, size_t k, uint32_t* best, float* best_sim, uint32_t* n_exceed);
int launch_gemm_nt_f32(hipStream_t st, const float* A, size_t M, const float* B, size_t N, size_t K, float* out);
int launch_sim_den(hipStream_t st, const float* extracted, size_t n_ext, size_t k, float* den);
int launch_sim_scale(hipStream_t st, float* sims, const float* den, size_t n_ext, size_t n_marks);
int launch_widen_indices(hipStream_t st, const uint32_t* in, size_t n, uint64_t* out);

}

namespace ssw { namespace host { struct Transfer; } }

struct ssw_ctx {
    int device = 0;
    hipStream_t stream = nullptr;
    hipStream_t own_stream = nullptr;
    size_t chunk_frames = 0;

    std::map<std::tuple<size_t, bool, bool, ssw::BasisKind>, void*> basis;
    bool fold = true;
    int fold_level = SSW_DCT_FOLDING_DEFAULT;

    struct Buf {
        void* p = nullptr;
        size_t bytes = 0;
    };
    struct Lane {
        Buf plane[4];
        Buf operand[6];
        Buf idx;
        ssw::SelectWorkspace sel;
        Buf compact[2];
        Buf gathered;
        Buf prune_u32;
        hipStream_t cur = nullptr;
        hipEvent_t done = nullptr;
    };
    static constexpr int MAX_LANES = 2;
    Lane lane[MAX_LANES];
    hipStream_t aux_stream = nullptr;
    bool overlap = true;
    bool prune = true;
    bool split = true;
    std::vector<hipEvent_t> sync_events;
    size_t sync_next = 0;
    Buf overflow;
    uint64_t pruned_chunks = 0, redone_chunks = 0;
    uint64_t pruned_columns = 0;
    hipStream_t copy_stream = nullptr;
    struct FrameStage {
        Buf buf;
        static constexpr int MAX_BANDS = 4;
        hipEvent_t uploaded[MAX_BANDS] = {nullptr, nullptr, nullptr, nullptr};
        hipEvent_t consumed = nullptr;
        bool in_use = false;
    };
    FrameStage frame_stage[2];
    unsigned frame_stage_next = 0;
    size_t expected_k = 0;
    std::multimap<size_t, void*> plane_pool;
    size_t plane_pool_bytes = 0;
    struct RgbSpare { void* p; size_t bytes; hipEvent_t released; };
    std::vector<RgbSpare> rgb_spares;
    std::vector<void*> retired;
    uint32_t* select_fallbacks = nullptr;
    uint64_t select_frames = 0;
    ssw::host::Transfer* xfer = nullptr;
    hipStream_t down_stream = nullptr;
    struct HostStream {
        static constexpr int NB = 3;
        Buf in[NB], in2[NB], out[NB];
        Buf marks, ext, sims;
        hipEvent_t up_done[NB] = {}, k_done[NB] = {}, down_done[NB] = {};
        bool active = false;
    };
    HostStream hs;
    Buf small;
    Buf sort_scratch;
    Buf resize_tmp;
    Buf restore_base;
    Buf trace[6];
    Buf locate[6];
    Buf fingerprint[6];
    std::map<std::pair<size_t, size_t>, ssw::DeviceTaps> taps;

    bool timing = false;
    double stage_ms[SSW_STAGE_COUNT] = {0};
    uint64_t stage_launches[SSW_STAGE_COUNT] = {0};
    double stage_bytes[SSW_STAGE_COUNT] = {0};
    double stage_work[SSW_STAGE_COUNT] = {0};
    struct Pending {
        int stage;
        hipEvent_t a, b;
        int alias = -1;
    };
    std::vector<Pending> pending;
    std::vector<hipEvent_t> free_events;
    hipEvent_t tail_event = nullptr;
    hipStream_t tail_stream = nullptr;
    bool tail_fresh = false;
};
namespace ssw { inline PlanSettings plan_settings(const ssw_ctx* ctx) { return PlanSettings{ctx->fold, ctx->fold_level, ctx->split}; } }
```

### spread_spectrum_watermarking_amd/csrc/ssw_lib.hip

```cpp
#include <algorithm>
#include <cmath>
#include <cstdlib>
#include <cstring>
#include <new>

#include "resize_common.hpp"
#include "ssw_host.hpp"

namespace ssw {
static thread_local std::string g_last_error;
void set_last_error(const std::string& s) { g_last_error = s; }
}

using namespace ssw;
using namespace ssw::host;

struct ssw_writer {
    ssw_ctx* ctx;
    size_t w, h;
    ssw_config cfg;
    float *y = nullptr, *i = nullptr, *q = nullptr;
    float* y0 = nullptr;
    uint32_t* idx = nullptr;
    size_t idx_k = 0;
// ... 229 lines not shown
    }
}

const char* ssw_last_error(void) { return g_last_error.c_str(); }

void ssw_config_default(ssw_config* cfg) {
    if (!cfg) return;
    cfg->ordering = SSW_ORDER_ENERGY;
    cfg->method = SSW_OPTION2;
    cfg->alpha = 0.1f;
    cfg->precision = SSW_PRECISION_F64;
}

int ssw_ctx_create(int device_id, ssw_ctx** out) {
    if (!out) return SSW_ERR_BAD_ARG;
    *out = nullptr;
    int count = 0;
    if (hipGetDeviceCount(&count) != hipSuccess || count <= 0) {
        set_last_error("hipGetDeviceCount: no device");
        return SSW_ERR_NO_DEVICE;
    }
    if (device_id < 0 || device_id >= count) return SSW_ERR_BAD_ARG;
    DeviceGuard g(device_id);
    ssw_ctx* ctx = new (std::nothrow) ssw_ctx();
    if (!ctx) return SSW_ERR_OUT_OF_MEMORY;
    ctx->device = device_id;
    hipError_t e = hipStreamCreateWithFlags(&ctx->own_stream, hipStreamNonBlocking);
    if (e != hipSuccess) { delete ctx; set_last_error(hipGetErrorString(e)); return SSW_ERR_HIP; }
    ctx->stream = ctx->own_stream;
    e = hipStreamCreateWithFlags(&ctx->aux_stream, hipStreamNonBlocking);
    if (e != hipSuccess) { (void)hipStreamDestroy(ctx->own_stream); delete ctx; set_last_error(hipGetErrorString(e)); return SSW_ERR_HIP; }
    e = hipStreamCreateWithFlags(&ctx->copy_stream, hipStreamNonBlocking);
    if (e != hipSuccess) {
        (void)hipStreamDestroy(ctx->aux_stream); (void)hipStreamDestroy(ctx->own_stream);
        delete ctx; set_last_error(hipGetErrorString(e)); return SSW_ERR_HIP;
    }
    if (hipMalloc((void**)&ctx->select_fallbacks, sizeof(uint32_t)) != hipSuccess ||
        hipMemset(ctx->select_fallbacks, 0, sizeof(uint32_t)) != hipSuccess) {
        (void)hipGetLastError();
        if (ctx->select_fallbacks) (void)hipFree(ctx->select_fallbacks);
        (void)hipStreamDestroy(ctx->copy_stream); (void)hipStreamDestroy(ctx->aux_stream); (void)hipStreamDestroy(ctx->own_stream);
        delete ctx; set_last_error("hipMalloc: selection counter"); return SSW_ERR_OUT_OF_MEMORY;
    }
    const char* ov = std::getenv("SSW_OVERLAP");
    if (ov) ctx->overlap = std::atoi(ov) != 0;
    const char* pr = std::getenv("SSW_PRUNE");
    if (pr) ctx->prune = std::atoi(pr) != 0;
    const char* sp = std::getenv("SSW_ODD_SPLIT");
    if (sp) ctx->split = std::atoi(sp) != 0;
    *out = ctx;
    return SSW_OK;
}

int ssw_ctx_destroy(ssw_ctx* ctx) {
    if (!ctx) return SSW_OK;
    CtxGuard g(ctx);
    (void)hipStreamSynchronize(ctx->stream);
    if (ctx->aux_stream) (void)hipStreamSynchronize(ctx->aux_stream);
    if (ctx->copy_stream) (void)hipStreamSynchronize(ctx->copy_stream);
    if (ctx->down_stream) (void)hipStreamSynchronize(ctx->down_stream);
    transfer_destroy(ctx);
    for (int s = 0; s < ssw_ctx::HostStream::NB; ++s) {
        release(ctx->hs.in[s]); release(ctx->hs.in2[s]); release(ctx->hs.out[s]);
        for (hipEvent_t e : {ctx->hs.up_done[s], ctx->hs.k_done[s], ctx->hs.down_done[s]}) if (e) (void)hipEventDestroy(e);
    }
    release(ctx->hs.marks); release(ctx->hs.ext); release(ctx->hs.sims);
    for (void* p : ctx->retired) (void)hipFree(p);
    ctx->retired.clear();
    (void)plane_pool_flush(ctx);
    for (auto& fs : ctx->frame_stage) {
        release(fs.buf);
        for (hipEvent_t e : fs.uploaded)
            if (e) (void)hipEventDestroy(e);
        if (fs.consumed) (void)hipEventDestroy(fs.consumed);
    }
    for (auto& kv : ctx->basis) (void)hipFree(kv.second);
    for (auto& ln : ctx->lane) {
        for (auto& b : ln.plane) release(b);
        for (auto& b : ln.operand) release(b);
        for (auto& b : ln.compact) release(b);
        release(ln.idx);
        release(ln.gathered);
        release(ln.prune_u32);
        release_select(ln.sel);
    }
    if (ctx->select_fallbacks) (void)hipFree(ctx->select_fallbacks);
    release(ctx->overflow);
    release(ctx->small);
    release(ctx->sort_scratch);
    release(ctx->resize_tmp);
    release(ctx->restore_base);
    for (auto& b : ctx->fingerprint) release(b);
    for (auto& b : ctx->trace) release(b);
    for (auto& b : ctx->locate) release(b);
    for (auto& kv : ctx->taps) { (void)hipFree(kv.second.left); (void)hipFree(kv.second.count); (void)hipFree(kv.second.weights); }
    for (auto& e : ctx->sync_events) (void)hipEventDestroy(e);
    for (auto& p : ctx->pending) { (void)hipEventDestroy(p.a); (void)hipEventDestroy(p.b); }
    for (auto& e : ctx->free_events) (void)hipEventDestroy(e);
    if (ctx->aux_stream) (void)hipStreamDestroy(ctx->aux_stream);
    if (ctx->copy_stream) (void)hipStreamDestroy(ctx->copy_stream);
    if (ctx->down_stream) (void)hipStreamDestroy(ctx->down_stream);
    (void)hipStreamDestroy(ctx->own_stream);
    delete ctx;
    return SSW_OK;
}

int ssw_ctx_synchronize(ssw_ctx* ctx) {
    if (!ctx) return SSW_ERR_BAD_ARG;
    CtxGuard g(ctx);
    SSW_HIP_CHECK(hipStreamSynchronize(ctx->stream));
    return SSW_OK;
}

void* ssw_ctx_stream(ssw_ctx* ctx) { return ctx ? (void*)ctx->stream : nullptr; }

int ssw_ctx_set_stream(ssw_ctx* ctx, void* hip_stream) {
    if (!ctx) return SSW_ERR_BAD_ARG;
    CtxGuard g(ctx);
    SSW_TRY(flush_timers(ctx));
    SSW_HIP_CHECK(hipStreamSynchronize(ctx->stream));
    ctx->stream = hip_stream ? (hipStream_t)hip_stream : ctx->own_stream;
    return SSW_OK;
}

int ssw_ctx_wait_event(ssw_ctx* ctx, void* hip_event) {
    if (!ctx || !hip_event) return SSW_ERR_BAD_ARG;
    CtxGuard g(ctx);
    SSW_HIP_CHECK(hipStreamWaitEvent(ctx->stream, (hipEvent_t)hip_event, 0));
    return SSW_OK;
}

int ssw_ctx_record_event(ssw_ctx* ctx, void* hip_event) {
    if (!ctx || !hip_event) return SSW_ERR_BAD_ARG;
    CtxGuard g(ctx);
    SSW_HIP_CHECK(hipEventRecord((hipEvent_t)hip_event, ctx->stream));
    return SSW_OK;
}

int ssw_ctx_set_chunk_frames(ssw_ctx* ctx, size_t frames) {
    if (!ctx) return SSW_ERR_BAD_ARG;
    ctx->chunk_frames = frames;
    return SSW_OK;
}

size_t ssw_ctx_pass_frames(ssw_ctx* ctx, size_t n_frames, size_t w, size_t h) {
    return ctx ? effective_chunk(ctx, w, h, n_frames) : 0;
}

int ssw_ctx_set_dct_folding(ssw_ctx* ctx, int enable) {
    if (!ctx) return SSW_ERR_BAD_ARG;
    if (enable < 0 || enable > 6) return SSW_ERR_BAD_ARG;
    ctx->fold = enable != 0;
    ctx->fold_level = enable;
    return SSW_OK;
}

int ssw_ctx_enable_timing(ssw_ctx* ctx, int enable) {
    if (!ctx) return SSW_ERR_BAD_ARG;
    CtxGuard g(ctx);
    SSW_TRY(flush_timers(ctx));
    ctx->timing = enable != 0;
    return SSW_OK;
}

int ssw_ctx_reset_timing(ssw_ctx* ctx) {
    if (!ctx) return SSW_ERR_BAD_ARG;
    CtxGuard g(ctx);
    SSW_TRY(flush_timers(ctx));
    for (int s = 0; s < SSW_STAGE_COUNT; ++s) { ctx->stage_ms[s] = 0; ctx->stage_launches[s] = 0; ctx->stage_work[s] = 0; ctx->stage_bytes[s] = 0; }
    ctx->pruned_chunks = ctx->redone_chunks = ctx->pruned_columns = 0;
    ctx->select_frames = 0;
    SSW_HIP_CHECK(hipStreamSynchronize(ctx->stream));
    if (ctx->aux_stream) SSW_HIP_CHECK(hipStreamSynchronize(ctx->aux_stream));
    SSW_HIP_CHECK(hipMemset(ctx->select_fallbacks, 0, sizeof(uint32_t)));
    return SSW_OK;
}

int ssw_ctx_get_timing(ssw_ctx* ctx, double* ms, uint64_t* launches) {
    if (!ctx) return SSW_ERR_BAD_ARG;
    CtxGuard g(ctx);
    SSW_TRY(flush_timers(ctx));
    for (int s = 0; s < SSW_STAGE_COUNT; ++s) {
        if (ms) ms[s] = ctx->stage_ms[s];
        if (launches) launches[s] = ctx->stage_launches[s];
    }
    return SSW_OK;
}

int ssw_ctx_get_work(ssw_ctx* ctx, double* work) {
    if (!ctx || !work) return SSW_ERR_BAD_ARG;
    CtxGuard g(ctx);
    SSW_TRY(flush_timers(ctx));
    for (int s = 0; s < SSW_STAGE_COUNT; ++s) work[s] = ctx->stage_work[s];
    return SSW_OK;
}

int ssw_ctx_get_traffic(ssw_ctx* ctx, double* bytes) {
    if (!ctx || !bytes) return SSW_ERR_BAD_ARG;
    CtxGuard g(ctx);
    SSW_TRY(flush_timers(ctx));
    for (int s = 0; s < SSW_STAGE_COUNT; ++s) bytes[s] = ctx->stage_bytes[s];
    return SSW_OK;
}

int ssw_ctx_set_overlap(ssw_ctx* ctx, int enable) {
    if (!ctx) return SSW_ERR_BAD_ARG;
    ctx->overlap = enable != 0;
    return SSW_OK;
}

int ssw_ctx_set_prune(ssw_ctx* ctx, int enable) {
    if (!ctx) return SSW_ERR_BAD_ARG;
    ctx->prune = enable != 0;
    return SSW_OK;
}

int ssw_ctx_set_odd_split(ssw_ctx* ctx, int enable) {
    if (!ctx) return SSW_ERR_BAD_ARG;
    ctx->split = enable != 0;
    return SSW_OK;
}

int ssw_ctx_get_prune_stats(ssw_ctx* ctx, uint64_t* stats) {
    if (!ctx || !stats) return SSW_ERR_BAD_ARG;
    stats[0] = ctx->pruned_chunks;
    stats[1] = ctx->redone_chunks;
    stats[2] = ctx->pruned_columns;
    return SSW_OK;
}

int ssw_ctx_get_select_stats(ssw_ctx* ctx, uint64_t* stats) {
    if (!ctx || !stats) return SSW_ERR_BAD_ARG;
    CtxGuard g(ctx);
    stats[0] = ctx->select_frames;
    stats[1] = 0;
    if (ctx->select_fallbacks) {
        uint32_t v = 0;
        SSW_HIP_CHECK(hipStreamSynchronize(ctx->stream));
        if (ctx->aux_stream) SSW_HIP_CHECK(hipStreamSynchronize(ctx->aux_stream));
        SSW_HIP_CHECK(hipMemcpy(&v, ctx->select_fallbacks, sizeof(v), hipMemcpyDeviceToHost));
        stats[1] = v;
    }
    return SSW_OK;
}

int ssw_dev_mem_info(ssw_ctx* ctx, size_t* free_bytes, size_t* total_bytes) {
    if (!ctx || !free_bytes || !total_bytes) return SSW_ERR_BAD_ARG;
    CtxGuard g(ctx);
    SSW_HIP_CHECK(hipMemGetInfo(free_bytes, total_bytes));
    return SSW_OK;
}

int ssw_dev_alloc(ssw_ctx* ctx, size_t bytes, void** dev_ptr) {
    if (!ctx || !dev_ptr) return SSW_ERR_BAD_ARG;
    CtxGuard g(ctx);
    SSW_ALLOC(dev_ptr, bytes);
    return SSW_OK;
}
int ssw_dev_free(ssw_ctx* ctx, void* dev_ptr) {
    if (!ctx) return SSW_ERR_BAD_ARG;
    CtxGuard g(ctx);
    SSW_HIP_CHECK(hipStreamSynchronize(ctx->stream));
    if (dev_ptr) SSW_HIP_CHECK(hipFree(dev_ptr));
    return SSW_OK;
}
int ssw_copy_to_dev(ssw_ctx* ctx, void* dev_dst, const void* host_src, size_t bytes) {
    if (!ctx || (bytes && (!dev_dst || !host_src))) return SSW_ERR_BAD_ARG;
    CtxGuard g(ctx);
    SSW_TRY(upload(ctx, dev_dst, host_src, bytes, ctx->stream));
    SSW_HIP_CHECK(hipStreamSynchronize(ctx->stream));
    return SSW_OK;
}
int ssw_copy_to_host(ssw_ctx* ctx, void* host_dst, const void* dev_src, size_t bytes) {
    if (!ctx || (bytes && (!host_dst || !dev_src))) return SSW_ERR_BAD_ARG;
    CtxGuard g(ctx);
    return download(ctx, host_dst, dev_src, bytes, ctx->stream);
}

int ssw_host_alloc(ssw_ctx* ctx, size_t bytes, void** host_ptr) {
    if (!ctx || !host_ptr) return SSW_ERR_BAD_ARG;
    *host_ptr = nullptr;
    CtxGuard g(ctx);
    const hipError_t e = hipHostMalloc(host_ptr, bytes ? bytes : 16, hipHostMallocDefault);
    if (e != hipSuccess) {
        (void)hipGetLastError();
        *host_ptr = nullptr;
        set_last_error(std::string("hipHostMalloc(") + std::to_string(bytes) + " bytes): " + hipGetErrorString(e));
        return SSW_ERR_OUT_OF_MEMORY;
    }
    return SSW_OK;
}
int ssw_host_free(ssw_ctx* ctx, void* host_ptr) {
    if (!ctx) return SSW_ERR_BAD_ARG;
    CtxGuard g(ctx);
    if (host_ptr) SSW_HIP_CHECK(hipHostFree(host_ptr));
    return SSW_OK;
}
int ssw_ctx_set_copy_threads(ssw_ctx* ctx, int threads) {
    if (!ctx || threads < 0) return SSW_ERR_BAD_ARG;
    return transfer_set_threads(ctx, threads);
}
int ssw_ctx_get_transfer_stats(ssw_ctx* ctx, double* stats, int reset) {
    if (!ctx) return SSW_ERR_BAD_ARG;
    return transfer_stats(ctx, stats, reset != 0);
}

int ssw_rgb_to_yiq(ssw_ctx* ctx, const float* dev_rgb, size_t n_frames, size_t w, size_t h,
                   float* dev_y, float* dev_i, float* dev_q) {
    if (!ctx || !dev_rgb || !dev_y || ((dev_i == nullptr) != (dev_q == nullptr))) return SSW_ERR_BAD_ARG;
    CtxGuard g(ctx);
    StageTimer t(ctx, SSW_STAGE_RGB_TO_YIQ, ctx->stream);
// ... 699 lines not shown
```

### spread_spectrum_watermarking_amd/csrc/ssw_pipeline.hip

```cpp
#include <algorithm>
#include <cmath>
#include <cstring>

#include "ssw_host.hpp"
#include "dct_pair_split.hpp"

#include <array>
#include <cstdlib>

namespace ssw {
namespace host {

namespace { thread_local ssw_ctx* tl_ctx = nullptr; }
CtxGuard::CtxGuard(ssw_ctx* ctx) : dg(ctx->device), prev(tl_ctx) {
    tl_ctx = ctx;
    if (prev != ctx) { ctx->tail_event = nullptr; ctx->tail_fresh = false; }
    if (prev != ctx && !ctx->retired.empty()) {
        for (void* p : ctx->retired) (void)hipFree(p);
        ctx->retired.clear();
    }
}
CtxGuard::~CtxGuard() { tl_ctx = prev; }

size_t plane_pool_flush(ssw_ctx* ctx) {
// ... 43 lines not shown
        if (tl_ctx) tl_ctx->retired.push_back(b.p);
        else SSW_HIP_CHECK(hipFree(b.p));
        b.p = nullptr; b.bytes = 0;
    }
    SSW_ALLOC(&b.p, bytes);
    b.bytes = bytes ? bytes : 16;
    return SSW_OK;
}

void release(ssw_ctx::Buf& b) {
    if (b.p) (void)hipFree(b.p);
    b.p = nullptr;
    b.bytes = 0;
}

void release_select(SelectWorkspace& s) {
    if (s.hist) (void)hipFree(s.hist);
    if (s.ctrl) (void)hipFree(s.ctrl);
    if (s.cand) (void)hipFree(s.cand);
    s = SelectWorkspace();
}

int grow_select(hipStream_t st, SelectWorkspace& s, size_t frames, size_t k) {
    const size_t want = select_cand_capacity(k);
    if (s.frames >= frames && s.cap >= want && s.hist) return SSW_OK;
    const size_t nf = std::max(frames, s.frames), cap = std::max(want, s.cap);
    release_select(s);
    SSW_ALLOC(&s.hist, nf * 2048 * sizeof(uint32_t));
    SSW_ALLOC(&s.ctrl, nf * 4 * sizeof(uint32_t));
    SSW_ALLOC(&s.cand, nf * cap * sizeof(uint64_t));
    SSW_HIP_CHECK(hipMemsetAsync(s.hist, 0, nf * 2048 * sizeof(uint32_t), st));
    SSW_HIP_CHECK(hipMemsetAsync(s.ctrl, 0, nf * 4 * sizeof(uint32_t), st));
    untimed_work(tl_ctx);
    s.frames = nf;
    s.cap = cap;
    return SSW_OK;
}

static hipEvent_t timer_event(ssw_ctx* ctx, hipStream_t st) {
    if (ctx->tail_event && ctx->tail_fresh && ctx->tail_stream == st) return ctx->tail_event;
    hipEvent_t e = nullptr;
    if (!ctx->free_events.empty()) { e = ctx->free_events.back(); ctx->free_events.pop_back(); }
    else if (hipEventCreateWithFlags(&e, hipEventReleaseToDevice) != hipSuccess) return nullptr;
    if (hipEventRecord(e, st) != hipSuccess) { ctx->free_events.push_back(e); return nullptr; }
    ctx->tail_event = e; ctx->tail_stream = st; ctx->tail_fresh = true;
    return e;
}
StageTimer::StageTimer(ssw_ctx* c, int s, hipStream_t stream, double work, int alias_stage) : ctx(c), stage(s), st(stream), alias(alias_stage) {
    if (!ctx->timing) return;
    ctx->stage_work[stage] += work;
    if (alias >= 0) ctx->stage_work[alias] += work;
    const bool gemm = stage == SSW_STAGE_DCT_ROW || stage == SSW_STAGE_DCT_COL || stage == SSW_STAGE_DCT_ROW_MAIN || stage == SSW_STAGE_DCT_COL_MAIN;
    if (!gemm) ctx->stage_bytes[stage] += work;
    a = timer_event(ctx, st);
    ctx->tail_fresh = false;
    armed = a != nullptr;
}
void StageTimer::traffic(double bytes) {
    if (ctx->timing) ctx->stage_bytes[stage] += bytes;
}
StageTimer::~StageTimer() {
    if (!ctx->timing || !armed) return;
    b = timer_event(ctx, st);
    if (b) ctx->pending.push_back({stage, a, b, alias});
}

int flush_timers(ssw_ctx* ctx) {
    std::vector<hipEvent_t> used;
    for (auto& p : ctx->pending) {
        float ms = 0.f;
        SSW_HIP_CHECK(hipEventSynchronize(p.b));
        SSW_HIP_CHECK(hipEventElapsedTime(&ms, p.a, p.b));
        ctx->stage_ms[p.stage] += ms;
        ctx->stage_launches[p.stage] += 1;
        if (p.alias >= 0) { ctx->stage_ms[p.alias] += ms; ctx->stage_launches[p.alias] += 1; }
        used.push_back(p.a);
        used.push_back(p.b);
    }
    ctx->pending.clear();
    std::sort(used.begin(), used.end());
    used.erase(std::unique(used.begin(), used.end()), used.end());
    for (hipEvent_t e : used) ctx->free_events.push_back(e);
    ctx->tail_event = nullptr; ctx->tail_fresh = false;
    return SSW_OK;
}

int get_basis(ssw_ctx* ctx, size_t n, bool inverse, bool f64, BasisKind kind, const void** out) {
    typedef BasisKind B;
    auto key = std::make_tuple(n, inverse, f64, kind);
    auto it = ctx->basis.find(key);
    if (it != ctx->basis.end()) { *out = it->second; return SSW_OK; }
    void* p = nullptr;
    if (kind != B::Dense && !f64) return SSW_ERR_BAD_ARG;
    const bool half = kind == B::HalfEven || kind == B::HalfOdd, rot = kind == B::Rot;
    const int split_which = kind == B::SinELaunch ? 4 : (int)kind - (int)B::CosE;
    const size_t elems = kind == B::Dense ? n * dense_basis_kpad(n)
                       : rot  ? n / 2
                       : half ? (n / 2) * dct_pair_kpad(n)
                              : dct_pair_split_basis_rows(n, split_which) * dct_pair_split_kpad(n);
    SSW_ALLOC(&p, std::max<size_t>(elems, 1) * (f64 ? sizeof(double) : sizeof(float)));
    int rc = rot  ? launch_make_rot_table(ctx->stream, n, (double*)p)
             : half ? launch_make_half_basis_blocked(ctx->stream, n, inverse, kind == B::HalfOdd ? 1 : 0, (double*)p)
             : kind != B::Dense ? launch_make_split_basis_blocked(ctx->stream, n, inverse, split_which, (double*)p)
             : f64  ? launch_make_basis_f64(ctx->stream, n, inverse, (double*)p)
                    : launch_make_basis_f32(ctx->stream, n, inverse, (float*)p);
    untimed_work(ctx);
    if (rc != SSW_OK) { (void)hipFree(p); return rc; }
    ctx->basis[key] = p;
    *out = p;
    return SSW_OK;
}

bool valid_method(int m) { return m == SSW_OPTION1 || m == SSW_OPTION2 || m == SSW_OPTION3; }
bool valid_ordering(int o) { return o == SSW_ORDER_ENERGY || o == SSW_ORDER_ENERGY_ORTHOGONAL || o == SSW_ORDER_LEGACY; }
bool valid_precision(int p) { return p == SSW_PRECISION_F32 || p == SSW_PRECISION_F64; }

int check_config(const ssw_config* cfg) {
    if (!cfg) return SSW_ERR_BAD_ARG;
    if (cfg->method == SSW_METHOD_CUSTOM || cfg->ordering == SSW_ORDER_CUSTOM) return SSW_ERR_UNSUPPORTED;
    if (!valid_method(cfg->method) || !valid_ordering(cfg->ordering) || !valid_precision(cfg->precision))
        return SSW_ERR_BAD_ARG;
    return SSW_OK;
}

namespace {
size_t lane_bytes_held(const ssw_ctx* ctx) {
    size_t held = 0;
    for (const auto& ln : ctx->lane) {
        for (const auto& b : ln.plane) held += b.bytes;
        for (const auto& b : ln.operand) held += b.bytes;
        for (const auto& b : ln.compact) held += b.bytes;
        held += ln.idx.bytes + ln.gathered.bytes + ln.prune_u32.bytes;
    }
    return held;
}
}

size_t effective_chunk(const ssw_ctx* ctx, size_t w, size_t h, size_t n_frames) {
    size_t c = ctx->chunk_frames;
    if (c == 0) {
        const size_t px = std::max<size_t>(w * h, 1);
        c = std::max<size_t>(1, ((size_t)1 << 30) / px);
        const size_t per_frame = dct_pair_operand_elems(1, w, h) * sizeof(double);
        if (per_frame) c = std::max<size_t>(1, std::min(c, (size_t)0xFFFFFFFFull / per_frame));
        if (c >= 16) c &= ~(size_t)7;
        c = std::min(c, std::max<size_t>(n_frames, 1));
        size_t free_b = 0, total_b = 0;
        DeviceGuard g(ctx->device);
        if (hipMemGetInfo(&free_b, &total_b) == hipSuccess) {
            const size_t budget = (free_b + lane_bytes_held(ctx) + ctx->plane_pool_bytes) / 2;
            size_t c1 = std::max<size_t>(1, std::min(c, budget / (44 * px)));
            if (ctx->overlap && n_frames > c1) c1 = std::max<size_t>(1, std::min(c1, budget / (2 * 44 * px)));
            c = c1;
        } else {
            (void)hipGetLastError();
        }
    }
    return std::min(c, std::max<size_t>(n_frames, 1));
}

namespace {

bool aligned_planes(const float* a, const float* b) { return ((reinterpret_cast<uintptr_t>(a) | reinterpret_cast<uintptr_t>(b)) & 15) == 0; }
struct PassBuild {
    ssw_ctx* ctx; Xform x; PassPlan p;
    bool first_pass, is_row, inverse, from_rgb;
// ... 151 lines not shown
    PairClassDesc even;
    SSW_TRY(odd_half(b, pp, x2, odd));
    SSW_TRY(class_desc(b, PairClass::EvenHalf, xx1, xx2, even));
    const double f_main = odd.flop, f_all = f_main + b.flop(PairClass::EvenHalf);
    const RgbSink sink = rgb_sink(b, fused_rgb);
    ch.push_back({false, [=](hipStream_t st) -> int {
        StageTimer t(ctx, b.st_pass, st, f_all);
        t.traffic(b.gemm_bytes(b.inverse ? 8.0 : 0.0));
        SSW_TRY(b.gemm(st, 1, &even, tmpE));
        StageTimer tm(ctx, b.st_main, st, f_main);
        return odd_gemm(b, odd, st, tmpE, sink.rgb ? &sink : nullptr);
    }});
    return SSW_OK;
}

int build_pair_three(const PassBuild& b, ssw_ctx::Lane& ws, Chain& ch) {
    ssw_ctx* ctx = b.ctx;
    PairPlanes pp;
    SSW_TRY(pair_planes(b, ws, pp));
    for (int i = 0; i < 4; ++i) SSW_TRY(grow(ws.operand[i], pp.bytes));
    double *d1 = (double*)ws.operand[1].p, *d2 = (double*)ws.operand[0].p, *r1 = (double*)ws.operand[2].p, *r2 = (double*)ws.operand[3].p;
    ch.push_back({true, [=](hipStream_t st) -> int {
        StageTimer t(ctx, b.st_prep, st, b.prep_bytes);
        if (!b.is_row) SSW_TRY(launch_dct_pair_prep8_cols(st, b.src, b.n, b.w, b.h, r1, r2, d2, d1));
        else SSW_TRY(launch_dct_pair_prep8_rows(st, b.rgb_kind(), b.prep_src(), b.n, b.w, b.h, r1, r2, d2, d1, b.prep_i(), b.prep_q()));
        return odd_rotate(b, pp, st, d1);
    }});
    OddHalfLaunch odd;
    PairClassDesc r, m;
    SSW_TRY(odd_half(b, pp, d1, odd));
    SSW_TRY(class_desc(b, PairClass::R1R2, r1, r2, r));
    SSW_TRY(class_desc(b, PairClass::OddHalf2, d2, d2, m));
    const double f_main = odd.flop, f_all = f_main + b.flop(PairClass::R1R2) + b.flop(PairClass::OddHalf2);
    ch.push_back({false, [=](hipStream_t st) -> int {
        StageTimer t(ctx, b.st_pass, st, f_all);
        t.traffic(b.gemm_bytes(0.0));
        SSW_TRY(b.gemm(st, 1, &r));
        SSW_TRY(b.gemm(st, 1, &m));
        StageTimer tm(ctx, b.st_main, st, f_main);
        return odd_gemm(b, odd, st, nullptr, nullptr);
    }});
    return SSW_OK;
}


int build_deep(const PassBuild& b, ssw_ctx::Lane& ws, Chain& ch) {
    typedef PairClass C;
    ssw_ctx* ctx = b.ctx;
    PairPlanes pp;
    const void *rot2 = nullptr, *rot3 = nullptr;
    SSW_TRY(pair_planes(b, ws, pp));
    SSW_TRY(deep_rot(b, false, &rot2, &rot3));
    double* sp = pp.sp;
    ch.push_back({true, [=](hipStream_t st) -> int {
        StageTimer t(ctx, b.st_prep, st, b.prep_bytes);
        if (!b.is_row) return launch_dct_pair_prep16_cols(st, b.src, b.n, b.w, b.h, sp, (const double*)pp.rot, (const double*)rot2, nullptr, b.p.prep, b.p.layout);
        return launch_dct_pair_prep16_rows(st, b.rgb_kind(), b.prep_src(), b.n, b.w, b.h, sp, (const double*)pp.rot, (const double*)rot2, nullptr,
                                           b.prep_i(), b.prep_q(), false);
    }});
    const double f_main = b.flop(C::O), f_all = f_main + b.flop(C::E) + b.flop(C::R1R2) + b.flop(C::E2) + b.flop(C::O2);
    std::array<PairClassDesc, 5> merged, single;
    SSW_TRY(deep_descs(b, pp, false, {C::R1R2, C::E2, C::O2, C::O, C::E}, merged.data()));
    SSW_TRY(deep_descs(b, pp, false, {C::R1R2, C::E2, C::O2, C::E, C::O}, single.data()));
    ch.push_back({false, [=](hipStream_t st) -> int {
        StageTimer t(ctx, b.st_pass, st, f_all);
        t.traffic(b.gemm_bytes(0.0));
        auto launch = [&](int nc, const PairClassDesc* d) { return b.gemm(st, nc, d, nullptr, nullptr, nullptr, b.gemm_layout()); };
        if (!b.p.merge) return launch_classes(ctx, st, false, 5, single.data(), launch, b.st_main, f_main);
        StageTimer tm(ctx, b.st_main, st, f_all);
        return launch(5, merged.data());
    }});
    return SSW_OK;
}

int build_deep_l2(const PassBuild& b, ssw_ctx::Lane& ws, Chain& ch) {
    ssw_ctx* ctx = b.ctx;
    const bool fused = b.p.strategy == PassStrategy::FusedRows || b.p.strategy == PassStrategy::FusedCols;
    PairPlanes pp;
    const void *rot2 = nullptr, *rot3 = nullptr;
    SSW_TRY(pair_planes(b, ws, pp));
    SSW_TRY(deep_rot(b, true, &rot2, &rot3));
    const size_t n = b.n, w = b.w, h = b.h;
    FuseCols fc;
    double pad = 1.0;
    double bytes = b.gemm_bytes(0.0);
    float* out = b.dst;
    if (fused) {
        const size_t cplane = n * w * dct_pair_split_kpad(h / 2);
        SSW_TRY(grow(ws.operand[0], 16 * cplane * sizeof(double)));
        double* cop = (double*)ws.operand[0].p;
        fc = FuseCols{FUSE_COLS};
        if (!b.is_row) { pp.l2 = cop; pp.l2_plane = cplane; }
        else {
            const void *crot1 = nullptr, *crot2 = nullptr, *crot3 = nullptr;
            SSW_TRY(get_basis(ctx, h, false, true, BasisKind::Rot, &crot1));
            SSW_TRY(get_basis(ctx, h / 2, false, true, BasisKind::Rot, &crot2));
            SSW_TRY(get_basis(ctx, h / 4, false, true, BasisKind::Rot, &crot3));
            const size_t lpad = n * 16 * dct_pair_fused_units(h);
            pp.l2_plane = lpad * dct_pair_split_kpad(b.len / 2);
            pad = (double)lpad / (double)(n * h);
            fc = FuseCols{FUSE_ROWS_COP, cop, (const double*)crot1, (const double*)crot2, (const double*)crot3};
            bytes = b.px * 16.0;
            out = nullptr;
        }
    }
    double* sp = pp.sp;
    if (!fused || b.is_row)
        ch.push_back({true, [=](hipStream_t st) -> int {
            StageTimer t(ctx, b.st_prep, st, b.prep_bytes);
            if (!b.is_row) return launch_dct_pair_prep16_cols(st, b.src, n, w, h, sp, (const double*)pp.rot, (const double*)rot2, (const double*)rot3,
                                                              b.p.prep, b.p.layout);
            return launch_dct_pair_prep16_rows(st, b.rgb_kind(), b.prep_src(), n, w, h, sp, (const double*)pp.rot, (const double*)rot2,
                                               (const double*)rot3, b.prep_i(), b.prep_q(), true, fused);
        }});
    const double f_main = b.flop(PairClass::O5), f_all = 8.0 * f_main;
    std::array<PairClassDesc, 8> d;
    for (int c = 0; c < 8; ++c) SSW_TRY(deep_desc(b, pp, true, kLevel2Classes[c], d[c]));
    ch.push_back({false, [=](hipStream_t st) -> int {
        StageTimer t(ctx, b.st_pass, st, f_all * pad, b.p.merge ? b.st_main : -1);
        t.traffic(bytes);
        auto launch = [&](int nc, const PairClassDesc* dd) {
            return launch_dct_pair_gemm_multi_f64(st, b.is_row, false, nc, dd, out, nullptr, n, w, h, b.ep, nullptr, nullptr, b.gemm_layout(),
                                                  fused ? &fc : nullptr);
        };
        return launch_classes(ctx, st, b.p.merge, 8, d.data(), launch, b.st_main, f_main * pad);
    }});
    return SSW_OK;
}

int build_semi_deep(const PassBuild& b, ssw_ctx::Lane& ws, Chain& ch, bool* fused_rgb) {
    typedef PairClass C;
    ssw_ctx* ctx = b.ctx;
    const bool inv = b.inverse;
    PairPlanes pp;
    SSW_TRY(pair_planes(b, ws, pp));
    if (inv) for (int i : {1, 4}) SSW_TRY(grow(ws.operand[i], pp.bytes));
    double* T2 = inv ? (double*)ws.operand[1].p : nullptr;
    double* TE = inv ? (double*)ws.operand[4].p : nullptr;
    double* sp = pp.sp;
    const double* rot = (const double*)pp.rot;
    ch.push_back({true, [=](hipStream_t st) -> int {
        StageTimer t(ctx, b.st_prep, st, b.prep_bytes);
        if (inv) return launch_dct_pair_prep16_inv_cols(st, b.src, b.n, b.w, b.h, sp, rot, rot, nullptr, b.p.prep, b.p.layout);
        return launch_dct_pair_prep16_cols(st, b.src, b.n, b.w, b.h, sp, rot, rot, nullptr, b.p.prep, b.p.layout);
    }});
    const RgbSink sink = rgb_sink(b, fused_rgb);
    PairClassDesc r1, sd, eo[2];
    SSW_TRY(deep_desc(b, pp, false, C::R1R2, r1));
    SSW_TRY(deep_desc(b, pp, false, C::OddHalf2, sd));
    SSW_TRY(deep_descs(b, pp, false, {C::E, C::O}, eo));
    const double f_sd = b.flop(C::OddHalf2);
    const double f_main = b.flop(C::E), f_all = f_main + b.flop(C::O) + b.flop(C::R1R2) + f_sd;
    ch.push_back({false, [=](hipStream_t st) -> int {
        StageTimer t(ctx, b.st_pass, st, f_all);
        t.traffic(b.gemm_bytes(inv ? 12.0 : 0.0));
        if (inv) {
            SSW_TRY(b.gemm(st, 1, &r1, T2));
            SSW_TRY(b.gemm(st, 1, &sd, T2, TE));
            return launch_classes(ctx, st, b.p.merge, 2, eo, [&](int nc, const PairClassDesc* d) { return b.gemm(st, nc, d, TE, nullptr, sink.rgb ? &sink : nullptr); });
        }
        if (b.p.merge) {
            SSW_TRY(b.gemm(st, 1, &sd));
            const PairClassDesc d[3] = {r1, eo[1], eo[0]};
            StageTimer tm(ctx, b.st_main, st, f_all - f_sd);
            return b.gemm(st, 3, d);
        }
        SSW_TRY(b.gemm(st, 1, &r1));
        SSW_TRY(b.gemm(st, 1, &sd));
        SSW_TRY(b.gemm(st, 1, &eo[1]));
        StageTimer tm(ctx, b.st_main, st, f_main);
        return b.gemm(st, 1, &eo[0]);
    }});
    return SSW_OK;
}

int build_deep_inv(const PassBuild& b, ssw_ctx::Lane& ws, Chain& ch, bool* fused_rgb) {
    typedef PairClass C;
    ssw_ctx* ctx = b.ctx;
    const bool l2 = b.p.strategy == PassStrategy::DeepInvL2;
    const size_t len = b.len, lines = b.lines;
    PairPlanes pp;
    const void *rot2 = nullptr, *rot3 = nullptr;
    SSW_TRY(pair_planes(b, ws, pp));
    SSW_TRY(deep_rot(b, l2, &rot2, &rot3));
    SSW_TRY(grow(ws.operand[1], std::max<size_t>(pp.bytes, lines * (len / 4) * sizeof(double))));
    SSW_TRY(grow(ws.operand[4], std::max<size_t>(pp.bytes, lines * (len / 2) * sizeof(double))));
    double* A1 = nullptr;
    if (l2) {
        SSW_TRY(grow(ws.operand[2], std::max<size_t>(pp.bytes, lines * (len / 8) * sizeof(double))));
        A1 = (double*)ws.operand[2].p;
    }
    double* T2 = (double*)ws.operand[1].p;
    double* TE = (double*)ws.operand[4].p;
    double* sp = pp.sp;
    const RgbSink sink = rgb_sink(b, fused_rgb);
    ch.push_back({true, [=](hipStream_t st) -> int {
        StageTimer t(ctx, b.st_prep, st, b.prep_bytes);
        if (!b.is_row) return launch_dct_pair_prep16_inv_cols(st, b.src, b.n, b.w, b.h, sp, (const double*)pp.rot, (const double*)rot2, (const double*)rot3,
                                                              b.p.prep, b.p.layout);
        return launch_dct_pair_prep16_inv_rows(st, b.src, b.n, b.w, b.h, sp, (const double*)pp.rot, (const double*)rot2, (const double*)rot3, b.p.prep);
    }});
// ... 20 lines not shown
}

int build_pass(ssw_ctx* ctx, ssw_ctx::Lane& ws, const Xform& x, bool first_pass, bool is_row, const float* src, float* dst,
               Epilogue ep, Chain& ch, bool* fused_rgb = nullptr) {
    const PlanInput in{x.type, x.precision, x.n, x.w, x.h, x.full_h, x.natural_order, aligned_planes(src, dst), plan_settings(ctx)};
    PassBuild b{ctx, x, plan_pass(in, first_pass, is_row), first_pass, is_row, x.type == SSW_DCT3, x.rgb && first_pass, x.n, x.w, x.h,
                is_row ? x.w : x.h, is_row ? x.n * x.h : x.n * x.w, src, dst, ep};
    if (b.from_rgb && !(is_row && b.p.levels >= 2)) return SSW_ERR_BAD_ARG;
    b.st_pass = is_row ? SSW_STAGE_DCT_ROW : SSW_STAGE_DCT_COL;
    b.st_main = is_row ? SSW_STAGE_DCT_ROW_MAIN : SSW_STAGE_DCT_COL_MAIN;
    b.st_prep = b.from_rgb ? SSW_STAGE_RGB_TO_YIQ : SSW_STAGE_DCT_PREP;
    b.px = (double)b.n * (double)b.w * (double)b.h;
    b.prep_bytes = b.from_rgb ? b.px * (3.0 * (double)pix_bytes(x.rgb_u8) + (x.iq_i ? 8.0 : 0.0) + 8.0) : b.px * (4.0 + 8.0);
    const bool sink_pass = b.inverse && !first_pass && !is_row && x.rgb_out && x.iq_i && x.iq_q;
    b.out_bpp = sink_pass ? 8.0 + 3.0 * (double)pix_bytes(x.rgb_out_u8) : 4.0;
    const size_t first = ch.size();
    typedef PassStrategy S;
    const S s = b.p.strategy;
    SSW_TRY(s == S::Dense                   ? build_dense(b, ch)
            : s == S::PairL1                ? build_pair_l1(b, ws, ch)
            : s == S::PairTwo               ? build_pair_two(b, ws, ch, fused_rgb)
            : s == S::PairThree             ? build_pair_three(b, ws, ch)
            : s == S::Deep                  ? build_deep(b, ws, ch)
            : s == S::SemiDeep || s == S::SemiDeepInv ? build_semi_deep(b, ws, ch, fused_rgb)
            : s == S::DeepInv || s == S::DeepInvL2    ? build_deep_inv(b, ws, ch, fused_rgb)
                                                      : build_deep_l2(b, ws, ch));
    for (size_t i = first; i < ch.size(); ++i) {
        if (!ch[i].hbm && is_row) ch[i].tag = 1;
        if (ch[i].hbm && is_row && first_pass && x.type != SSW_DCT3 && x.rgb) ch[i].tag = 2;
    }
    return SSW_OK;
}

}

int build_transform(ssw_ctx* ctx, ssw_ctx::Lane& ws, const Xform& x, Chain& ch, bool* fused_rgb) {
    const bool f64 = (x.precision == SSW_PRECISION_F64);
    const size_t n = x.n, w = x.w, h = x.h;
    if (n == 0) return SSW_OK;
    const size_t max_frames = plan_frame_limit(plan_settings(ctx), f64, w, h);
    if (n > max_frames) {
        for (size_t f0 = 0; f0 < n; f0 += max_frames) {
            Xform s = x;
            s.n = std::min(max_frames, n - f0);
            s.data = x.data + f0 * w * h;
            s.tmp = x.tmp + f0 * w * h;
            if (x.rgb) s.rgb = static_cast<const char*>(x.rgb) + f0 * w * h * 3 * pix_bytes(x.rgb_u8);
            if (x.iq_i) s.iq_i = x.iq_i + f0 * w * h;
            if (x.iq_q) s.iq_q = x.iq_q + f0 * w * h;
            if (x.rgb_out) s.rgb_out = static_cast<char*>(x.rgb_out) + f0 * w * h * 3 * (x.rgb_out_u8 ? 1 : sizeof(float));
            SSW_TRY(build_transform(ctx, ws, s, ch, fused_rgb));
        }
        return SSW_OK;
    }
    const bool rows_first = (w >= h);
    Epilogue plain{1.f, 1.f};
    auto ortho = [&](size_t len) {
        Epilogue e{std::sqrt(1.0f / (4.0f * (float)len)), std::sqrt(1.0f / (2.0f * (float)len))};
        return e;
    };
    Epilogue last = plain;
    if (x.type == SSW_DCT3) last.first = last.base = (float)4 / (float)(w * h);
    for (int pass = 0; pass < 2; ++pass) {
        const bool is_row = (pass == 0) ? rows_first : !rows_first;
        const float* src = (pass == 0) ? x.data : x.tmp;
        float* dst = (pass == 0) ? x.tmp : x.data;
        const Epilogue ep = (x.type == SSW_DCT2_ORTHOGONAL) ? ortho(is_row ? w : h) : (pass == 1 ? last : plain);
        SSW_TRY(build_pass(ctx, ws, x, pass == 0, is_row, src, dst, ep, ch, fused_rgb));
    }
    return SSW_OK;
}

namespace {
PassPlan forward_rows_plan(const ssw_ctx* ctx, bool f64, size_t n, size_t w, size_t h, const float* a, const float* b) {
    return plan_pass({SSW_DCT2, f64 ? SSW_PRECISION_F64 : SSW_PRECISION_F32, n, w, h, 0, false, aligned_planes(a, b), plan_settings(ctx)}, true, true);
}
}

bool can_fuse_rgb(const ssw_ctx* ctx, bool f64, size_t w, size_t h, const float* y, const float* tmp, const void* rgb, int u8) {
    return forward_rows_plan(ctx, f64, 1, w, h, y, tmp).levels >= 2 && dct_pair_can_prep_from_rgb(w, h, rgb, u8);
}

int build_forward_from_rgb(ssw_ctx* ctx, ssw_ctx::Lane& ws, int precision, const void* rgb, int u8, size_t n, size_t w,
                           size_t h, float* y, float* i, float* q, float* tmp, Chain& ch) {
    const bool f64 = precision == SSW_PRECISION_F64;
    Xform x{SSW_DCT2, precision, n, w, h, y, tmp};
    if (can_fuse_rgb(ctx, f64, w, h, y, tmp, rgb, u8)) {
        x.rgb = rgb; x.rgb_u8 = u8; x.iq_i = i; x.iq_q = q;
        return build_transform(ctx, ws, x, ch);
    }
    const size_t npix = n * w * h;
    const double bytes = (double)npix * (3.0 * (double)pix_bytes(u8) + (i ? 12.0 : 4.0));
    ch.push_back({true, [=](hipStream_t st) -> int {
        StageTimer t(ctx, SSW_STAGE_RGB_TO_YIQ, st, bytes);
        if (u8 == SSW_PIX_U8) return launch_rgb8_to_yiq(st, static_cast<const uint8_t*>(rgb), npix, y, i, q);
        if (u8 == SSW_PIX_U16) return launch_rgb16_to_yiq(st, static_cast<const uint16_t*>(rgb), npix, y, i, q);
        return launch_rgb_to_yiq(st, static_cast<const float*>(rgb), npix, y, i, q);
    }});
    return build_transform(ctx, ws, x, ch);
}

bool can_split_forward_rows(const ssw_ctx* ctx, bool f64, size_t w, size_t h, size_t bands, const float* y, const float* tmp, const void* rgb, int u8) {
    return bands >= 2 && w >= h && h % 16 == 0 && h % bands == 0 && can_fuse_rgb(ctx, f64, w, h, y, tmp, rgb, u8) &&
           can_fuse_rgb(ctx, f64, w, h / bands, y, tmp, rgb, u8);
}
int build_forward_rows_band(ssw_ctx* ctx, ssw_ctx::Lane& ws, int precision, const void* rgb, int u8, size_t w, size_t rows,
                            size_t frame_h, float* tmp, float* i, float* q, Chain& ch) {
    Xform x{SSW_DCT2, precision, 1, w, rows, tmp , tmp};
    x.rgb = rgb; x.rgb_u8 = u8; x.iq_i = i; x.iq_q = q;
    x.full_h = frame_h;
    return build_pass(ctx, ws, x, true, true, tmp, tmp, Epilogue{1.f, 1.f}, ch);
}
int build_forward_cols_after_rows(ssw_ctx* ctx, ssw_ctx::Lane& ws, int precision, size_t w, size_t h, float* tmp, float* y, Chain& ch) {
    Xform x{SSW_DCT2, precision, 1, w, h, y, tmp};
    x.full_h = h;
    return build_pass(ctx, ws, x, false, false, tmp, y, Epilogue{1.f, 1.f}, ch);
}

int run_serial(Chain& ch, hipStream_t st) {
    for (auto& s : ch) SSW_TRY(s.run(st));
    return SSW_OK;
}

int dct2d_planes(ssw_ctx* ctx, int type, int precision, size_t n, size_t w, size_t h, float* data, float* tmp) {
    Chain ch;
    Xform x{type, precision, n, w, h, data, tmp};
    SSW_TRY(build_transform(ctx, ctx->lane[0], x, ch));
    return run_serial(ch, ctx->stream);
}

int topk(ssw_ctx* ctx, hipStream_t st, SelectWorkspace& sel, const float* coef, size_t n, size_t w, size_t h, int ordering,
         size_t k, uint32_t* idx) {
    const double bytes = 4.0 * (double)n * (double)w * (double)h;
    if (k > select_max_k()) {
        size_t sb = 0;
        SSW_TRY(full_sort_scratch_bytes(w * h, n, &sb));
        SSW_TRY(grow(ctx->sort_scratch, sb));
        StageTimer t(ctx, SSW_STAGE_SELECT, st, bytes);
        return launch_full_sort(st, coef, n, w, h, ordering, ctx->sort_scratch.p, ctx->sort_scratch.bytes, idx, k);
    }
    SSW_TRY(grow_select(st, sel, n, k));
    sel.fallbacks = ctx->select_fallbacks;
    ctx->select_frames += n;
    StageTimer t(ctx, SSW_STAGE_SELECT, st, bytes);
    return launch_topk(st, coef, n, w, h, ordering, k, sel, idx);
}

namespace {

int next_sync_event(ssw_ctx* ctx, hipEvent_t* out) {
    constexpr size_t RING = 256;
    if (ctx->sync_events.size() < RING) {
        hipEvent_t e = nullptr;
        SSW_HIP_CHECK(hipEventCreateWithFlags(&e, hipEventDisableTiming));
        ctx->sync_events.push_back(e);
        *out = e;
        return SSW_OK;
    }
    *out = ctx->sync_events[ctx->sync_next % RING];
    ctx->sync_next++;
    return SSW_OK;
}

int mark_done(ssw_ctx* ctx, ssw_ctx::Lane& ln) {
    SSW_TRY(next_sync_event(ctx, &ln.done));
    SSW_HIP_CHECK(hipEventRecord(ln.done, ln.cur));
    untimed_work(ctx);
    return SSW_OK;
}
// ... 289 lines not shown
    Xform xc{SSW_DCT2, SSW_PRECISION_F64, n, cap, h, (float*)ws.compact[1].p, t_compact};
    xc.natural_order = true;
    return build_pass(ctx, ws, xc, false, false, t_compact, (float*)ws.compact[1].p, Epilogue{1.f, 1.f}, ch);
}

}

int batch_embed_impl(ssw_ctx* ctx, const ssw_config* cfg, const void* dev_rgb, int u8_in, size_t n_frames, size_t w,
                     size_t h, const float* dev_marks, size_t k, void* dev_rgb_out, bool u8_out, float* dev_coef_out,
                     uint32_t* dev_indices_out) {
    if (!ctx || !dev_rgb || !dev_marks || !dev_rgb_out) return SSW_ERR_BAD_ARG;
    SSW_TRY(check_config(cfg));
    if (w == 0 || h == 0) return SSW_ERR_BAD_DIMS;
    const size_t plane = w * h;
    const size_t k_eff = std::min(k, plane - 1);
    CtxGuard g(ctx);
    const size_t chunk = effective_chunk(ctx, w, h, n_frames);
    const size_t n_chunks = (n_frames + chunk - 1) / chunk;
    const ssw_config c = *cfg;
    const size_t in_px = 3 * pix_bytes(u8_in), out_px = u8_out ? 3 : 3 * sizeof(float);
    auto build = [&](size_t ci, ssw_ctx::Lane& ws, Chain& ch) -> int {
        const size_t f0 = ci * chunk, n = std::min(chunk, n_frames - f0);
        for (int p = 0; p < 4; ++p) SSW_TRY(grow(ws.plane[p], chunk * plane * sizeof(float)));
        SSW_TRY(grow(ws.idx, chunk * std::max<size_t>(k_eff, 1) * sizeof(uint32_t)));
        float* y = (float*)ws.plane[0].p;
        float* pi = (float*)ws.plane[1].p;
        float* pq = (float*)ws.plane[2].p;
        float* tmp = (float*)ws.plane[3].p;
        const char* rgb = static_cast<const char*>(dev_rgb) + f0 * plane * in_px;
        char* out = static_cast<char*>(dev_rgb_out) + f0 * plane * out_px;
        uint32_t* idx = dev_indices_out ? dev_indices_out + f0 * k_eff : (uint32_t*)ws.idx.p;
        float* coef_out = dev_coef_out ? dev_coef_out + f0 * plane : nullptr;
        const float* marks = dev_marks + f0 * k;
        SelectWorkspace* sel = &ws.sel;
        SSW_TRY(build_forward_from_rgb(ctx, ws, c.precision, rgb, u8_in, n, w, h, y, pi, pq, tmp, ch));
        ch.push_back({true, [=](hipStream_t st) -> int {
            if (coef_out) { SSW_HIP_CHECK(hipMemcpyAsync(coef_out, y, n * plane * sizeof(float), hipMemcpyDeviceToDevice, st)); untimed_work(ctx); }
            if (k_eff == 0) return SSW_OK;
            SSW_TRY(topk(ctx, st, *sel, y, n, w, h, c.ordering, k_eff, idx));
            StageTimer t(ctx, SSW_STAGE_EMBED, st);
            return launch_embed(st, y, n, plane, idx, k_eff, marks, nullptr, nullptr, 1, k_eff, k, c.method, c.alpha);
        }});
        Xform inv{SSW_DCT3, c.precision, n, w, h, y, tmp};
        inv.iq_i = pi; inv.iq_q = pq; inv.rgb_out = out; inv.rgb_out_u8 = u8_out;
        bool fused_rgb = false;
        SSW_TRY(build_transform(ctx, ws, inv, ch, &fused_rgb));
        if (fused_rgb) return SSW_OK;
        const double out_bytes = (double)n * plane * (12.0 + (u8_out ? 3.0 : 12.0));
        ch.push_back({true, [=](hipStream_t st) -> int {
            StageTimer t(ctx, SSW_STAGE_YIQ_TO_RGB, st, out_bytes);
            if (u8_out) return launch_yiq_to_rgb8(st, y, pi, pq, n * plane, reinterpret_cast<uint8_t*>(out));
            return launch_yiq_to_rgb(st, y, pi, pq, n * plane, reinterpret_cast<float*>(out));
        }});
        return SSW_OK;
    };
    return run_pipeline(ctx, n_chunks, build);
}

int batch_extract_impl(ssw_ctx* ctx, const ssw_config* cfg, const void* dev_base_rgb, const void* dev_derived_rgb, int u8,
                       size_t n_frames, size_t w, size_t h, size_t k, float* dev_extracted, const float* dev_marks,
                       float* dev_sims) {
    if (!ctx || !dev_base_rgb || !dev_derived_rgb || !dev_extracted) return SSW_ERR_BAD_ARG;
    if ((dev_marks == nullptr) != (dev_sims == nullptr)) return SSW_ERR_BAD_ARG;
    SSW_TRY(check_config(cfg));
    if (w == 0 || h == 0) return SSW_ERR_BAD_DIMS;
    const size_t plane = w * h;
    if (k >= plane) return SSW_ERR_K_TOO_LARGE;
    if (n_frames == 0) return SSW_OK;
    CtxGuard g(ctx);
    const size_t chunk = effective_chunk(ctx, w, h, n_frames);
    const size_t n_chunks = (n_frames + chunk - 1) / chunk;
    const ssw_config c = *cfg;
    const bool f64 = c.precision == SSW_PRECISION_F64;
    const size_t px_bytes = 3 * pix_bytes(u8);
    for (int l = 0; l < (pipeline_uses_two_lanes(ctx, n_chunks) ? 2 : 1); ++l)
        for (int p : {0, 2}) SSW_TRY(grow(ctx->lane[l].plane[p], chunk * plane * sizeof(float)));
    hipStreamCaptureStatus capture = hipStreamCaptureStatusNone;
    if (hipStreamIsCapturing(ctx->stream, &capture) != hipSuccess) { (void)hipGetLastError(); capture = hipStreamCaptureStatusNone; }
    const bool allow_prune = capture == hipStreamCaptureStatusNone;
    const PruneSetup ps = !allow_prune ? PruneSetup() : make_prune_setup(ctx, f64, std::min(chunk, n_frames), w, h, k, (const float*)ctx->lane[0].plane[0].p,
                                           (const float*)ctx->lane[0].plane[2].p, dev_derived_rgb, u8);
    if (ps.on) SSW_TRY(grow(ctx->overflow, n_chunks * SSW_PRUNE_INFO * sizeof(uint32_t)));
    uint32_t* overflow = (uint32_t*)ctx->overflow.p;

    auto full_derived = [&](ssw_ctx::Lane& ws, size_t f0, size_t n, float* yb, float* tmp, uint32_t* idx, Chain& ch) -> int {
        SSW_TRY(grow(ws.plane[1], chunk * plane * sizeof(float)));
        float* yd = (float*)ws.plane[1].p;
        const char* drgb = static_cast<const char*>(dev_derived_rgb) + f0 * plane * px_bytes;
        SSW_TRY(build_forward_from_rgb(ctx, ws, c.precision, drgb, u8, n, w, h, yd, nullptr, nullptr, tmp, ch));
        float* ext = dev_extracted + f0 * k;
        const float* marks = dev_marks ? dev_marks + f0 * k : nullptr;
        float* sims = dev_sims ? dev_sims + f0 : nullptr;
        ch.push_back({true, [=](hipStream_t st) -> int {
            if (k > 0) {
                StageTimer t(ctx, SSW_STAGE_EXTRACT, st);
                SSW_TRY(launch_extract(st, yb, yd, n, plane, idx, k, c.method, c.alpha, ext));
            }
            if (marks) {
                StageTimer t(ctx, SSW_STAGE_SIMILARITY, st);
                SSW_TRY(launch_similarity(st, ext, marks, n, k, sims));
            }
            return SSW_OK;
        }});
        return SSW_OK;
    };
    auto build_chunk = [&](size_t ci, ssw_ctx::Lane& ws, Chain& ch, bool pruned) -> int {
        const size_t f0 = ci * chunk, n = std::min(chunk, n_frames - f0);
        for (int p : {0, 2}) SSW_TRY(grow(ws.plane[p], chunk * plane * sizeof(float)));
        SSW_TRY(grow(ws.idx, chunk * std::max<size_t>(k, 1) * sizeof(uint32_t)));
        float* yb = (float*)ws.plane[0].p;
        float* tmp = (float*)ws.plane[2].p;
        uint32_t* idx = (uint32_t*)ws.idx.p;
        const char* brgb = static_cast<const char*>(dev_base_rgb) + f0 * plane * px_bytes;
        SelectWorkspace* sel = &ws.sel;
        SSW_TRY(build_forward_from_rgb(ctx, ws, c.precision, brgb, u8, n, w, h, yb, nullptr, nullptr, tmp, ch));
        if (k > 0)
            ch.push_back({true, [=](hipStream_t st) -> int { return topk(ctx, st, *sel, yb, n, w, h, c.ordering, k, idx); }});
        if (!pruned) return full_derived(ws, f0, n, yb, tmp, idx, ch);
        const char* drgb = static_cast<const char*>(dev_derived_rgb) + f0 * plane * px_bytes;
        SSW_TRY(build_pruned_derived(ctx, ws, drgb, u8, n, w, h, k, idx, ps, overflow + ci * SSW_PRUNE_INFO, ch));
        const float* compact = (const float*)ws.compact[1].p;
        const uint32_t* pos = (const uint32_t*)ws.prune_u32.p + w;
        const size_t cap = ps.plan.cap_total;
        float* ext = dev_extracted + f0 * k;
        const float* marks = dev_marks ? dev_marks + f0 * k : nullptr;
        float* sims = dev_sims ? dev_sims + f0 : nullptr;
        ch.push_back({true, [=](hipStream_t st) -> int {
            {
                StageTimer t(ctx, SSW_STAGE_EXTRACT, st);
                SSW_TRY(launch_extract_pruned(st, yb, compact, n, w, h, cap, pos, idx, k, c.method, c.alpha, ext));
            }
            if (marks) {
                StageTimer t(ctx, SSW_STAGE_SIMILARITY, st);
                SSW_TRY(launch_similarity(st, ext, marks, n, k, sims));
            }
            return SSW_OK;
        }});
        return SSW_OK;
    };
    SSW_TRY(run_pipeline(ctx, n_chunks, [&](size_t ci, ssw_ctx::Lane& ws, Chain& ch) { return build_chunk(ci, ws, ch, ps.on); }));
    if (!ps.on) return SSW_OK;
    std::vector<uint32_t> info(n_chunks * SSW_PRUNE_INFO);
    SSW_HIP_CHECK(hipMemcpyAsync(info.data(), overflow, info.size() * sizeof(uint32_t), hipMemcpyDeviceToHost, ctx->stream));
    SSW_HIP_CHECK(hipStreamSynchronize(ctx->stream));
    for (size_t ci = 0; ci < n_chunks; ++ci) {
        ctx->pruned_chunks++;
        for (unsigned q = 0; q < ps.plan.n_classes; ++q) ctx->pruned_columns += info[ci * SSW_PRUNE_INFO + 1 + q];
        if (info[ci * SSW_PRUNE_INFO] == 0) continue;
        ctx->redone_chunks++;
        Chain ch;
        SSW_TRY(build_chunk(ci, ctx->lane[0], ch, false));
        SSW_TRY(run_serial(ch, ctx->stream));
    }
    return SSW_OK;
}

int trace_base(ssw_ctx* ctx, const ssw_config& c, const void* dev_base_rgb, int u8, size_t w, size_t h, size_t k, const float** y,
               const uint32_t** idx) {
    const size_t plane = w * h;
    ssw_ctx::Lane& ws = ctx->lane[0];
    SSW_TRY(grow(ctx->trace[0], plane * sizeof(float)));
    SSW_TRY(grow(ctx->trace[1], std::max<size_t>(k, 1) * sizeof(uint32_t)));
    SSW_TRY(grow(ws.plane[2], plane * sizeof(float)));
    float* yb = (float*)ctx->trace[0].p;
    uint32_t* ib = (uint32_t*)ctx->trace[1].p;
    Chain ch;
    SSW_TRY(build_forward_from_rgb(ctx, ws, c.precision, dev_base_rgb, u8, 1, w, h, yb, nullptr, nullptr, (float*)ws.plane[2].p, ch));
    SSW_TRY(run_serial(ch, ctx->stream));
    if (k > 0) SSW_TRY(topk(ctx, ctx->stream, ws.sel, yb, 1, w, h, c.ordering, k, ib));
    *y = yb;
    *idx = ib;
    return SSW_OK;
}

int trace_extract(ssw_ctx* ctx, const ssw_config& c, const float* yb, const uint32_t* idx, const void* dev_suspect_rgb, int u8,
                  size_t n_frames, size_t w, size_t h, size_t k, float* dev_extracted) {
    if (n_frames == 0) return SSW_OK;
    const size_t plane = w * h;
    const size_t chunk = effective_chunk(ctx, w, h, n_frames);
    const size_t n_chunks = (n_frames + chunk - 1) / chunk;
    const bool f64 = c.precision == SSW_PRECISION_F64;
    const size_t px_bytes = 3 * pix_bytes(u8);
    hipStreamCaptureStatus capture = hipStreamCaptureStatusNone;
    if (hipStreamIsCapturing(ctx->stream, &capture) != hipSuccess) { (void)hipGetLastError(); capture = hipStreamCaptureStatusNone; }
    const PruneSetup ps = capture != hipStreamCaptureStatusNone ? PruneSetup()
                          : make_prune_setup(ctx, f64, std::min(chunk, n_frames), w, h, k, yb, yb, dev_suspect_rgb, u8);
    uint32_t* info = nullptr;
    const PruneShared shared{&ctx->trace[2], &ctx->trace[3], &ctx->trace[4], false};
    if (ps.on) {
        SSW_TRY(grow(ctx->overflow, SSW_PRUNE_INFO * sizeof(uint32_t)));
        info = (uint32_t*)ctx->overflow.p;
        PruneShared make = shared;
        make.build = true;
        Chain ch;
        SSW_TRY(build_pruned_derived(ctx, ctx->lane[0], dev_suspect_rgb, u8, 1, w, h, k, idx, ps, info, ch, &make));
        SSW_TRY(run_serial(ch, ctx->stream));
    }
    auto build_chunk = [&](size_t ci, ssw_ctx::Lane& ws, Chain& ch, bool pruned) -> int {
        const size_t f0 = ci * chunk, n = std::min(chunk, n_frames - f0);
        const char* srgb = static_cast<const char*>(dev_suspect_rgb) + f0 * plane * px_bytes;
        float* ext = dev_extracted + f0 * k;
        if (!pruned) {
            for (int p : {1, 2}) SSW_TRY(grow(ws.plane[p], chunk * plane * sizeof(float)));
            float* yd = (float*)ws.plane[1].p;
            SSW_TRY(build_forward_from_rgb(ctx, ws, c.precision, srgb, u8, n, w, h, yd, nullptr, nullptr, (float*)ws.plane[2].p, ch));
            ch.push_back({true, [=](hipStream_t st) -> int {
                StageTimer t(ctx, SSW_STAGE_EXTRACT, st);
                return launch_extract_shared(st, yb, yd, n, plane, idx, k, c.method, c.alpha, ext);
            }});
            return SSW_OK;
        }
        SSW_TRY(build_pruned_derived(ctx, ws, srgb, u8, n, w, h, k, idx, ps, info, ch, &shared));
        const float* compact = (const float*)ws.compact[1].p;
        const uint32_t* pos = (const uint32_t*)ctx->trace[2].p + w;
        const size_t cap = ps.plan.cap_total;
        ch.push_back({true, [=](hipStream_t st) -> int {
            StageTimer t(ctx, SSW_STAGE_EXTRACT, st);
            return launch_extract_shared_pruned(st, yb, compact, n, w, h, cap, pos, idx, k, c.method, c.alpha, ext);
        }});
        return SSW_OK;
    };
    SSW_TRY(run_pipeline(ctx, n_chunks, [&](size_t ci, ssw_ctx::Lane& ws, Chain& ch) { return build_chunk(ci, ws, ch, ps.on); }));
    if (!ps.on) return SSW_OK;
    uint32_t host_info[SSW_PRUNE_INFO];
    SSW_HIP_CHECK(hipMemcpyAsync(host_info, info, sizeof(host_info), hipMemcpyDeviceToHost, ctx->stream));
    SSW_HIP_CHECK(hipStreamSynchronize(ctx->stream));
    ctx->pruned_chunks += n_chunks;
    for (unsigned q = 0; q < ps.plan.n_classes; ++q) ctx->pruned_columns += host_info[1 + q];
    if (host_info[0] == 0) return SSW_OK;
    ctx->redone_chunks += n_chunks;
    for (size_t ci = 0; ci < n_chunks; ++ci) {
        Chain ch;
        SSW_TRY(build_chunk(ci, ctx->lane[0], ch, false));
        SSW_TRY(run_serial(ch, ctx->stream));
    }
    return SSW_OK;
}

int extract_single_pruned(ssw_ctx* ctx, int precision, const void* derived_rgb, int u8, size_t w, size_t h, const float* base_y,
// ... 27 lines not shown
```

### spread_spectrum_watermarking_amd/csrc/tuning.hip

```cpp
#include <atomic>
#include <cstdlib>
#include <cstring>
#include <mutex>

#include "ssw_internal.hpp"

namespace ssw {
namespace {

struct Entry {
    const char* name;
    const char* env;
    long long dflt;
    std::atomic<long long> value{0};
    std::atomic<int> state{0};
    Entry(const char* n, const char* e, long long d) : name(n), env(e), dflt(d) {}
};

Entry g_tune[TUNE_COUNT] = {
    {"efold_min", "SSW_EFOLD_MIN", 1280},
    {"efold_inv_min", "SSW_EFOLD_INV_MIN", 1280},
    {"efold_cols_min", "SSW_EFOLD_COLS_MIN", 720},
    {"class_tile", "SSW_CLASS_TILE", 1},
    {"deep_min_rows", "SSW_DEEP_MIN_ROWS", 256},
    {"deep_min_cols", "SSW_DEEP_MIN_COLS", 256},
    {"prep_staged", "SSW_PREP_STAGED", 1},
    {"merge_max_lines", "SSW_MERGE_MAX_LINES", 8192},
    {"bn32", "SSW_BN32", -1},
    {"band_split", "SSW_BAND_SPLIT", 1},
    {"fuse_cols", "SSW_FUSE_COLS", 1},
    {"upload_bands", "SSW_UPLOAD_BANDS", 3},
    {"speculate_k", "SSW_SPECULATE_K", 1},
    {"prep_light", "SSW_PREP_LIGHT", 1},
    {"lane_stagger", "SSW_LANE_STAGGER", 1},
    {"derived_fused", "SSW_DERIVED_FUSED", 1},
    {"tile48", "SSW_TILE48", 1},
};

std::mutex g_tune_lock;

}

long long tuning(int which) {
    Entry& e = g_tune[which];
    if (e.state.load(std::memory_order_acquire) == 0) {
        std::lock_guard<std::mutex> lk(g_tune_lock);
        if (e.state.load(std::memory_order_relaxed) == 0) {
            const char* s = std::getenv(e.env);
            long long v = s ? std::atoll(s) : e.dflt;
            if (which == TUNE_BAND_SPLIT && std::getenv("SSW_NO_SPLIT")) v = 0;
            e.value.store(v, std::memory_order_relaxed);
            e.state.store(1, std::memory_order_release);
        }
    }
    return e.value.load(std::memory_order_relaxed);
}

}

extern "C" {

int ssw_tuning_set(const char* name, long long value) {
    if (!name) return SSW_ERR_BAD_ARG;
    for (int i = 0; i < ssw::TUNE_COUNT; ++i)
        if (std::strcmp(ssw::g_tune[i].name, name) == 0) {
            std::lock_guard<std::mutex> lk(ssw::g_tune_lock);
            ssw::g_tune[i].value.store(value, std::memory_order_relaxed);
            ssw::g_tune[i].state.store(2, std::memory_order_release);
            return SSW_OK;
        }
    return SSW_ERR_BAD_ARG;
}

int ssw_tuning_get(const char* name, long long* value) {
    if (!name || !value) return SSW_ERR_BAD_ARG;
    for (int i = 0; i < ssw::TUNE_COUNT; ++i)
        if (std::strcmp(ssw::g_tune[i].name, name) == 0) { *value = ssw::tuning(i); return SSW_OK; }
    return SSW_ERR_BAD_ARG;
}

int ssw_tuning_reset(const char* name) {
    for (int i = 0; i < ssw::TUNE_COUNT; ++i)
        if (!name || std::strcmp(ssw::g_tune[i].name, name) == 0) {
            std::lock_guard<std::mutex> lk(ssw::g_tune_lock);
            ssw::g_tune[i].state.store(0, std::memory_order_release);
            if (name) return SSW_OK;
        }
    return name ? SSW_ERR_BAD_ARG : SSW_OK;
}

}
```

Baseline: 15260.

## Prune base-image column DCT tiles using row-energy bounds before top-k selection

Adds a base-image pruning path for f64 energy orderings. The fused row pass accumulates per-column energy. The column DCT then runs in two phases: first only the leading 128-wide tile, then a per-frame histogram top-k threshold decides which other tiles could hold a selected coefficient, given a gain-scaled energy bound. Tiles that cannot contribute are zeroed instead of transformed. This aims to skip most of the column GEMM work, at the cost of extra kernels, atomics in the row epilogue, and added correctness risk if the bound is not tight.

After: 15900, median of 6. +4.2%, better.

```diff
diff --git a/include/ssw.h b/include/ssw.h
--- a/include/ssw.h
+++ b/include/ssw.h
@@ -80,6 +80,9 @@
 int ssw_ctx_set_overlap(ssw_ctx* ctx, int enable);
 int ssw_ctx_set_prune(ssw_ctx* ctx, int enable);
 int ssw_ctx_get_prune_stats(ssw_ctx* ctx, uint64_t* stats);
+int ssw_ctx_get_base_prune_stats(ssw_ctx* ctx, uint64_t* stats);
+int ssw_debug_base_prune_bound(ssw_ctx* ctx, const ssw_config* cfg, const float* dev_rgb, size_t n_frames, size_t w, size_t h,
+                               size_t k, float* dev_bound);
 int ssw_ctx_get_select_stats(ssw_ctx* ctx, uint64_t* stats);
 
 #define SSW_DCT_FOLDING_DEFAULT 5
diff --git a/spread_spectrum_watermarking_amd/_lib.py b/spread_spectrum_watermarking_amd/_lib.py
--- a/spread_spectrum_watermarking_amd/_lib.py
+++ b/spread_spectrum_watermarking_amd/_lib.py
@@ -73,6 +73,8 @@
     "ssw_tuning_get": (C.c_int, [C.c_char_p, C.POINTER(C.c_longlong)]),
     "ssw_tuning_reset": (C.c_int, [C.c_char_p]),
     "ssw_ctx_get_prune_stats": (C.c_int, [_vp, C.POINTER(C.c_uint64)]),
+    "ssw_ctx_get_base_prune_stats": (C.c_int, [_vp, C.POINTER(C.c_uint64)]),
+    "ssw_debug_base_prune_bound": (C.c_int, [_vp, _vp, _vp, _sz, _sz, _sz, _sz, _vp]),
     "ssw_ctx_get_select_stats": (C.c_int, [_vp, C.POINTER(C.c_uint64)]),
     "ssw_dev_mem_info": (C.c_int, [_vp, C.POINTER(_sz), C.POINTER(_sz)]),
     "ssw_dev_alloc": (C.c_int, [_vp, _sz, C.POINTER(_vp)]),
diff --git a/spread_spectrum_watermarking_amd/api.py b/spread_spectrum_watermarking_amd/api.py
--- a/spread_spectrum_watermarking_amd/api.py
+++ b/spread_spectrum_watermarking_amd/api.py
@@ -86,7 +86,10 @@
     def prune_stats(self) -> dict:
         st = (C.c_uint64 * 3)()
         check(self._lib.ssw_ctx_get_prune_stats(self.handle, st), "ssw_ctx_get_prune_stats")
-        return {"pruned_chunks": int(st[0]), "redone_chunks": int(st[1]), "columns_needed": int(st[2])}
+        bp = (C.c_uint64 * 3)()
+        check(self._lib.ssw_ctx_get_base_prune_stats(self.handle, bp), "ssw_ctx_get_base_prune_stats")
+        return {"pruned_chunks": int(st[0]), "redone_chunks": int(st[1]), "columns_needed": int(st[2]),
+                "base_tiles": int(bp[0]), "base_tiles_computed": int(bp[1]), "base_frames_extended": int(bp[2])}
 
     def select_stats(self) -> dict:
         st = (C.c_uint64 * 2)()
diff --git a/spread_spectrum_watermarking_amd/csrc/base_prune.hip b/spread_spectrum_watermarking_amd/csrc/base_prune.hip
--- /dev/null
+++ b/spread_spectrum_watermarking_amd/csrc/base_prune.hip
@@ -0,0 +1,181 @@
+#include <algorithm>
+#include <cmath>
+
+#include "dct_pair_common.hpp"
+#include "dct_pair_colops.hpp"
+
+namespace ssw {
+
+namespace {
+
+constexpr int BP_BINS = 2048;
+constexpr int BP_THREADS = 1024;
+
+struct BpKey {
+    int ordering;
+    float s[2];
+    float s0[2];
+    float gain;
+};
+
+__device__ inline uint32_t bp_sortable(float v) {
+    const uint32_t b = __float_as_uint(v);
+    return (b & 0x80000000u) ? ~b : (b | 0x80000000u);
+}
+
+__global__ __launch_bounds__(BP_THREADS) void base_prune_decide_kernel(const float* __restrict__ coef, const float* __restrict__ energy,
+                                                                       unsigned W, unsigned H, BpKey kp, unsigned k,
+                                                                       unsigned* __restrict__ need, unsigned long long* __restrict__ stats,
+                                                                       double* __restrict__ work, double tile_flop, double tile_bytes,
+                                                                       double zero_bytes) {
+    __shared__ unsigned hist[BP_BINS];
+    __shared__ unsigned part[BP_THREADS / 64];
+    __shared__ float t_sh;
+    __shared__ unsigned any_sh;
+    const unsigned tid = threadIdx.x, f = blockIdx.x, tiles = W / SSW_BASE_PRUNE_TILE;
+    for (unsigned b = tid; b < BP_BINS; b += BP_THREADS) hist[b] = 0u;
+    if (tid == 0) { t_sh = 0.0f; any_sh = 0u; }
+    __syncthreads();
+    const float* plane = coef + (size_t)f * W * H;
+    const unsigned quads = H * (SSW_BASE_PRUNE_TILE / 4);
+    for (unsigned q = tid; q < quads; q += BP_THREADS) {
+        const unsigned y = q / (SSW_BASE_PRUNE_TILE / 4), x = 4 * (q % (SSW_BASE_PRUNE_TILE / 4));
+        const f32x4 c = *reinterpret_cast<const f32x4*>(plane + (size_t)y * W + x);
+#pragma unroll
+        for (int e = 0; e < 4; ++e) {
+            if (y == 0 && x + e == 0) continue;
+            float key;
+            if (kp.ordering == SSW_ORDER_ENERGY) key = c[e] * c[e];
+            else {
+                const float scaled = ((x + e) == 0 ? kp.s0[y == 0] : kp.s[y == 0]) * c[e];
+                key = scaled * scaled;
+            }
+            atomicAdd(&hist[bp_sortable(key) >> 21], 1u);
+        }
+    }
+    __syncthreads();
+    const unsigned b0 = BP_BINS - 2 - 2 * tid;
+    const unsigned h1 = hist[b0 + 1], h0 = hist[b0];
+    unsigned v = h1 + h0;
+#pragma unroll
+    for (int o = 1; o < 64; o <<= 1) {
+        const unsigned u = __shfl_up(v, o);
+        if ((tid & 63u) >= (unsigned)o) v += u;
+    }
+    if ((tid & 63u) == 63u) part[tid >> 6] = v;
+    __syncthreads();
+    unsigned before = 0;
+    for (unsigned wv = 0; wv < (tid >> 6); ++wv) before += part[wv];
+    const unsigned incl = before + v, excl = incl - h1 - h0;
+    if (excl < k && incl >= k) {
+        const unsigned bin = excl + h1 >= k ? b0 + 1 : b0;
+        const uint32_t sb = (uint32_t)bin << 21;
+        t_sh = (sb & 0x80000000u) ? __uint_as_float(sb & 0x7FFFFFFFu) : 0.0f;
+    }
+    __syncthreads();
+    const float T = t_sh;
+    const float* e = energy + (size_t)f * W;
+    unsigned* nd = need + (size_t)f * tiles;
+    for (unsigned t = tid; t < tiles; t += BP_THREADS) nd[t] = t == 0 ? 1u : 0u;
+    __syncthreads();
+    for (unsigned x = SSW_BASE_PRUNE_TILE + tid; x < W; x += BP_THREADS) {
+        const float bound = kp.gain * e[x];
+        if (!(T > 1e-30f) || !(bound < T)) { nd[x / SSW_BASE_PRUNE_TILE] = 1u; any_sh = 1u; }
+    }
+    __syncthreads();
+    if (tid == 0 && stats) {
+        unsigned computed = 0;
+        for (unsigned t = 0; t < tiles; ++t) computed += nd[t];
+        if (work) {
+            if (computed > 1) { atomicAdd(&work[0], (computed - 1) * tile_flop); atomicAdd(&work[1], (computed - 1) * tile_bytes); }
+            if (computed < tiles) atomicAdd(&work[2], (tiles - computed) * zero_bytes);
+        }
+        atomicAdd(&stats[0], (unsigned long long)tiles);
+        atomicAdd(&stats[1], (unsigned long long)computed);
+        if (any_sh) atomicAdd(&stats[2], 1ull);
+    }
+}
+
+__global__ __launch_bounds__(256) void base_prune_zero_kernel(float* __restrict__ coef, const unsigned* __restrict__ need, unsigned W,
+                                                              unsigned H, unsigned tiles) {
+    const unsigned ft = blockIdx.x;
+    if (need[ft] != 0u) return;
+    const unsigned f = ft / tiles, t = ft - f * tiles;
+    float* p = coef + (size_t)f * W * H + (size_t)t * SSW_BASE_PRUNE_TILE;
+    const unsigned qx = 4 * (threadIdx.x & 31u), ry = threadIdx.x >> 5;
+    for (unsigned y = blockIdx.y * 8 + ry; y < H; y += gridDim.y * 8)
+        *reinterpret_cast<f32x4*>(p + (size_t)y * W + qx) = (f32x4){0.f, 0.f, 0.f, 0.f};
+}
+
+__global__ __launch_bounds__(256) void base_prune_bound_kernel(const float* __restrict__ energy, unsigned W, size_t total, float gain,
+                                                               float* __restrict__ out) {
+    const size_t i = blockIdx.x * (size_t)blockDim.x + threadIdx.x;
+    if (i >= total) return;
+    const size_t f = i / W;
+    const unsigned x = (unsigned)(i - f * W), tb = x / SSW_BASE_PRUNE_TILE * SSW_BASE_PRUNE_TILE;
+    out[i] = gain * energy[f * W + tb + fwd_cm128_pos(x - tb)];
+}
+
+BpKey make_key(size_t w, size_t h, int ordering) {
+    float s[2][2];
+    select_ortho_scales(w, h, s);
+    BpKey kp;
+    kp.ordering = ordering;
+    kp.s[0] = s[0][0]; kp.s[1] = s[1][0];
+    kp.s0[0] = s[0][1]; kp.s0[1] = s[1][1];
+    kp.gain = base_prune_gain(w, h, ordering);
+    return kp;
+}
+
+}
+
+float base_prune_gain(size_t w, size_t h, int ordering) {
+    if (ordering != SSW_ORDER_ENERGY && ordering != SSW_ORDER_ENERGY_ORTHOGONAL) return 0.0f;
+    if (h == 0 || h >= ((size_t)1 << 17)) return 0.0f;
+    double g = 4.0 * (double)h;
+    if (ordering == SSW_ORDER_ENERGY_ORTHOGONAL) {
+        float s[2][2];
+        select_ortho_scales(w, h, s);
+        double m = 0.0;
+        for (int a = 0; a < 2; ++a) for (int b = 0; b < 2; ++b) m = std::max(m, (double)s[a][b]);
+        g *= m * m;
+    }
+    g *= 1.0 + 1.0 / 32.0;
+    return nextafterf((float)g, INFINITY);
+}
+
+int launch_base_prune_decide(hipStream_t st, const float* coef, const BasePrune& bp, size_t n_frames, size_t w, size_t h) {
+    if (n_frames == 0) return SSW_OK;
+    if (!coef || !bp.energy || !bp.need || (reinterpret_cast<uintptr_t>(coef) & 15) != 0 || w % SSW_BASE_PRUNE_TILE != 0 || w > 0xFFFFFFull || h > 0xFFFFFFull || n_frames > 0x7FFFFFFFull ||
+        bp.k == 0 || bp.k > 0xFFFFFFFFull) return SSW_ERR_BAD_ARG;
+    const BpKey kp = make_key(w, h, bp.ordering);
+    if (!(kp.gain > 0.0f)) return SSW_ERR_BAD_ARG;
+    base_prune_decide_kernel<<<(unsigned)n_frames, BP_THREADS, 0, st>>>(coef, bp.energy, (unsigned)w, (unsigned)h, kp, (unsigned)bp.k, bp.need,
+                                                                       bp.stats, bp.work, bp.tile_flop, bp.tile_bytes, bp.zero_bytes);
+    SSW_HIP_CHECK(hipGetLastError());
+    return SSW_OK;
+}
+
+int launch_base_prune_zero(hipStream_t st, float* coef, const unsigned* need, size_t n_frames, size_t w, size_t h) {
+    if (n_frames == 0) return SSW_OK;
+    const size_t tiles = w / SSW_BASE_PRUNE_TILE;
+    if (!coef || !need || w % SSW_BASE_PRUNE_TILE != 0 || n_frames * tiles > 0x7FFFFFFFull || (reinterpret_cast<uintptr_t>(coef) & 15) != 0)
+        return SSW_ERR_BAD_ARG;
+    const unsigned gy = (unsigned)std::min<size_t>((h + 7) / 8, 16);
+    base_prune_zero_kernel<<<dim3((unsigned)(n_frames * tiles), gy), 256, 0, st>>>(coef, need, (unsigned)w, (unsigned)h, (unsigned)tiles);
+    SSW_HIP_CHECK(hipGetLastError());
+    return SSW_OK;
+}
+
+int launch_base_prune_bound(hipStream_t st, const float* energy, size_t n_frames, size_t w, size_t h, int ordering, float* out) {
+    const size_t total = n_frames * w;
+    if (total == 0) return SSW_OK;
+    if (!energy || !out || w % SSW_BASE_PRUNE_TILE != 0) return SSW_ERR_BAD_ARG;
+    const float gain = base_prune_gain(w, h, ordering);
+    if (!(gain > 0.0f)) return SSW_ERR_UNSUPPORTED;
+    base_prune_bound_kernel<<<(unsigned)((total + 255) / 256), 256, 0, st>>>(energy, (unsigned)w, total, gain, out);
+    SSW_HIP_CHECK(hipGetLastError());
+    return SSW_OK;
+}
+
+}
diff --git a/spread_spectrum_watermarking_amd/csrc/dct_pair_common.hpp b/spread_spectrum_watermarking_amd/csrc/dct_pair_common.hpp
--- a/spread_spectrum_watermarking_amd/csrc/dct_pair_common.hpp
+++ b/spread_spectrum_watermarking_amd/csrc/dct_pair_common.hpp
@@ -42,6 +42,7 @@
     unsigned cop_k16 = 0, cop_lines = 0, cop_hup = 0;
     const double *crot1 = nullptr, *crot2 = nullptr, *crot3 = nullptr;
     unsigned xperm = 0;
+    float* col_energy = nullptr;
 };
 
 struct ForwardClassLayout {
diff --git a/spread_spectrum_watermarking_amd/csrc/dct_pair_f64.hip b/spread_spectrum_watermarking_amd/csrc/dct_pair_f64.hip
--- a/spread_spectrum_watermarking_amd/csrc/dct_pair_f64.hip
+++ b/spread_spectrum_watermarking_amd/csrc/dct_pair_f64.hip
@@ -100,6 +100,13 @@
         inst.epi = EPI_FWD_COLOP;
     }
     if (fuse_cols) po.xperm = 1;
+    const bool energy = fuse_rows && fuse->energy != nullptr;
+    po.col_energy = energy ? fuse->energy : nullptr;
+    ml.need = nullptr; ml.need_mode = 0; ml.need_tpf = 1;
+    if (fuse_cols && fuse->tile_mode) {
+        if (inst.epi != EPI_FWD || inst.samex || small || (fuse->tile_mode == 2 && !fuse->need)) return SSW_ERR_BAD_ARG;
+        ml.need = fuse->need; ml.need_mode = (unsigned)fuse->tile_mode; ml.need_tpf = (unsigned)(w / 128);
+    }
     auto al = [](const void* p, unsigned a) { return (reinterpret_cast<uintptr_t>(p) & (a - 1)) == 0; };
     po.wide = (!is_row && w % 4 == 0 && al(out, 16) && (n_frames * w) % 4 == 0 && (!tmp || al(tmp, 16)) && (!tmp_out || al(tmp_out, 16))) ? 1u : 0u;
     if (with_sink && !(al(sink->iq_i, 16) && al(sink->iq_q, 16) && al(sink->rgb, sink->u8 ? 4 : 16))) po.wide = 0;
@@ -110,12 +117,14 @@
     ml.po = po;
     switch (inst.epi) {
     case EPI_FWD_COLOP:
-        if (inst.subname == 4) SSW_LAUNCH_PAIR_BM(false, EPI_FWD_COLOP, false, 4, 128);
+        if (energy) { if (inst.subname == 4) SSW_LAUNCH_PAIR_BM(false, EPI_FWD_COLOP, false, 14, 128); else SSW_LAUNCH_PAIR_BM(false, EPI_FWD_COLOP, false, 13, 128); }
+        else if (inst.subname == 4) SSW_LAUNCH_PAIR_BM(false, EPI_FWD_COLOP, false, 4, 128);
         else SSW_LAUNCH_PAIR_BM(false, EPI_FWD_COLOP, false, 3, 128);
         break;
     case EPI_FWD_ADJ: SSW_LAUNCH_PAIR(false, EPI_FWD_ADJ, false); break;
     case EPI_FWD:
-        if (inst.subname == 4) SSW_LAUNCH_PAIR_SUB(false, EPI_FWD, false, 4);
+        if (ml.need_mode) SSW_LAUNCH_PAIR_BM(true, EPI_FWD, false, 13, 128);
+        else if (inst.subname == 4) SSW_LAUNCH_PAIR_SUB(false, EPI_FWD, false, 4);
         else if (inst.subname == 3) { if (is_row) SSW_LAUNCH_PAIR_SUB(false, EPI_FWD, false, 3); else SSW_LAUNCH_PAIR_SUB(true, EPI_FWD, false, 3); }
         else if (inst.samex) SSW_LAUNCH_ROWCOL(EPI_FWD, true);
         else SSW_LAUNCH_ROWCOL(EPI_FWD, false);
diff --git a/spread_spectrum_watermarking_amd/csrc/dct_pair_f64_kernel.hpp b/spread_spectrum_watermarking_amd/csrc/dct_pair_f64_kernel.hpp
--- a/spread_spectrum_watermarking_amd/csrc/dct_pair_f64_kernel.hpp
+++ b/spread_spectrum_watermarking_amd/csrc/dct_pair_f64_kernel.hpp
@@ -26,6 +26,8 @@
     PairClassArgs c[8];
     unsigned n_classes, L, tiles_m, tiles_n_total;
     PairOut po;
+    const unsigned* need = nullptr;
+    unsigned need_mode = 0, need_tpf = 1;
 };
 
 template <bool COLS, int EPI, bool SAMEX, int SUB = 0, int BM = 128>
@@ -53,6 +55,10 @@
     unsigned tm, tn, cls = 0;
     tile_of_block(blockIdx.x, gridDim.x, ml.tiles_m, ml.tiles_n_total, tm, tn);
     while (cls + 1 < ml.n_classes && tn >= ml.c[cls].tiles_n) { tn -= ml.c[cls].tiles_n; ++cls; }
+    if constexpr (COLS && EPI == EPI_FWD && BM == 128 && SUB >= 10) {
+        const unsigned t = tm % ml.need_tpf;
+        if (ml.need_mode == 1 ? t != 0 : (t == 0 || ml.need[tm] == 0)) return;
+    }
     const PairClassArgs& ca = ml.c[cls];
     const double* __restrict__ X1g = ca.x1;
     const double* __restrict__ X2g = ca.x2;
@@ -328,6 +334,15 @@
             f1[jn] = fpos1(pair) == 0 ? ep.first : ep.base;
             f2[jn] = fpos2(pair) == 0 ? ep.first : ep.base;
         }
+        constexpr bool ENERGY = SUB >= 10;
+        float en1[NJ], en2[NJ];
+        float* eb = reinterpret_cast<float*>(lds + 4 * 128 * 8);
+        if constexpr (ENERGY) {
+            static_assert(4 * 128 * 64 + 128 * 4 <= (int)sizeof(lds), "energy totals above the slabs");
+#pragma unroll
+            for (int jn = 0; jn < NJ; ++jn) { en1[jn] = 0.f; en2[jn] = 0.f; }
+            if (tid < 128) eb[tid] = 0.f;
+        }
         double o[NC][NI][16];
 #pragma unroll
         for (int i = 0; i < NI; ++i) {
@@ -338,6 +353,7 @@
                 for (int r = 0; r < 4; ++r) {
                     float v1 = (float)acc1[i][jn][r], v2 = (float)acc2[i][jn][r];
                     if (!plain) { v1 *= f1[jn]; v2 *= f2[jn]; }
+                    if constexpr (ENERGY) { en1[jn] = __builtin_fmaf(v1, v1, en1[jn]); en2[jn] = __builtin_fmaf(v2, v2, en2[jn]); }
                     tw[lpos(32 * jn + li, lq + 4 * r)] = v1;
                     tw[lpos(32 * jn + 16 + li, lq + 4 * r)] = v2;
                 }
@@ -358,6 +374,20 @@
                 if (!unit_ok) {
 #pragma unroll
                     for (int a = 0; a < 16; ++a) o[c][i][a] = 0.0;
+                }
+            }
+        }
+        if constexpr (ENERGY) {
+            __syncthreads();
+#pragma unroll
+            for (int jn = 0; jn < NJ; ++jn) {
+                float a = en1[jn], b = en2[jn];
+                a += __shfl_xor(a, 16); a += __shfl_xor(a, 32);
+                b += __shfl_xor(b, 16); b += __shfl_xor(b, 32);
+                if (lq == 0) {
+                    const unsigned pl = wn + 16 * jn + li;
+                    atomicAdd(eb + pl, a);
+                    atomicAdd(eb + 64 + pl, b);
                 }
             }
         }
@@ -386,6 +416,14 @@
 #pragma unroll
         for (int rnd = 0; rnd < 4; ++rnd) {
             __syncthreads();
+            if constexpr (ENERGY) {
+                if (rnd == 0 && tid < 128) {
+                    const unsigned pl = tid & 63u, pair = p0 + pl;
+                    const bool second = tid >= 64;
+                    const bool ok = pl < (unsigned)NPT && pair < NP && (second ? (pair >= po.p2lo && second_out) : pair < po.np1);
+                    if (ok) unsafeAtomicAdd(po.col_energy + (size_t)z * po.W + (second ? fpos2(pair) : fpos1(pair)), eb[tid]);
+                }
+            }
 #pragma unroll
             for (int c = 0; c < NC; ++c) {
                 if ((lane + 64 * c) >= (unsigned)NIT) continue;
diff --git a/spread_spectrum_watermarking_amd/csrc/select.hip b/spread_spectrum_watermarking_amd/csrc/select.hip
--- a/spread_spectrum_watermarking_amd/csrc/select.hip
+++ b/spread_spectrum_watermarking_amd/csrc/select.hip
@@ -432,6 +432,20 @@
     }
 }
 
+void select_ortho_scales(size_t w, size_t h, float s[2][2]) {
+    const float s_k0_w = sqrtf(1.0f / (4.0f * (float)w));
+    const float s_k0_h = sqrtf(1.0f / (4.0f * (float)h));
+    const float s_w = sqrtf(1.0f / (2.0f * (float)w));
+    const float s_h = sqrtf(1.0f / (2.0f * (float)h));
+    for (int fr = 0; fr < 2; ++fr)
+        for (int fc = 0; fc < 2; ++fc) {
+            volatile float sc = 1.0f;
+            sc = sc * (fr ? s_k0_w : s_w);
+            sc = sc * (fc ? s_k0_h : s_h);
+            s[fr][fc] = sc;
+        }
+}
+
 int launch_topk(hipStream_t st, const float* coef, size_t n_frames, size_t w, size_t h, int ordering,
                 size_t k, const SelectWorkspace& ws, uint32_t* indices) {
     const size_t plane_len = w * h;
@@ -445,19 +459,7 @@
     KeyParams kp;
     kp.ordering = ordering;
     kp.w = (unsigned)w;
-    {
-        const float s_k0_w = sqrtf(1.0f / (4.0f * (float)w));
-        const float s_k0_h = sqrtf(1.0f / (4.0f * (float)h));
-        const float s_w = sqrtf(1.0f / (2.0f * (float)w));
-        const float s_h = sqrtf(1.0f / (2.0f * (float)h));
-        for (int fr = 0; fr < 2; ++fr)
-            for (int fc = 0; fc < 2; ++fc) {
-                volatile float sc = 1.0f;
-                sc = sc * (fr ? s_k0_w : s_w);
-                sc = sc * (fc ? s_k0_h : s_h);
-                kp.s[fr][fc] = sc;
-            }
-    }
+    select_ortho_scales(w, h, kp.s);
     const unsigned stride_s = sample_stride_for(k);
     const size_t groups = (plane_len + stride_s * 4 - 1) / (stride_s * 4);
     size_t sb = (groups + 256 * 2 - 1) / (256 * 2);
diff --git a/spread_spectrum_watermarking_amd/csrc/ssw_host.hpp b/spread_spectrum_watermarking_amd/csrc/ssw_host.hpp
--- a/spread_spectrum_watermarking_amd/csrc/ssw_host.hpp
+++ b/spread_spectrum_watermarking_amd/csrc/ssw_host.hpp
@@ -88,11 +88,12 @@
     bool rgb_out_u8 = false;
     size_t full_h = 0;
     bool natural_order = false;
+    const BasePrune* base_prune = nullptr;
 };
 int build_transform(ssw_ctx* ctx, ssw_ctx::Lane& ws, const Xform& x, Chain& ch, bool* fused_rgb = nullptr);
 bool can_fuse_rgb(const ssw_ctx* ctx, bool f64, size_t w, size_t h, const float* y, const float* tmp, const void* rgb, int u8);
 int build_forward_from_rgb(ssw_ctx* ctx, ssw_ctx::Lane& ws, int precision, const void* rgb, int u8, size_t n, size_t w,
-                           size_t h, float* y, float* i, float* q, float* tmp, Chain& ch);
+                           size_t h, float* y, float* i, float* q, float* tmp, Chain& ch, const BasePrune* base_prune = nullptr);
 bool can_split_forward_rows(const ssw_ctx* ctx, bool f64, size_t w, size_t h, size_t bands, const float* y, const float* tmp, const void* rgb, int u8);
 int build_forward_rows_band(ssw_ctx* ctx, ssw_ctx::Lane& ws, int precision, const void* rgb, int u8, size_t w, size_t rows,
                             size_t frame_h, float* tmp, float* i, float* q, Chain& ch);
@@ -109,6 +110,9 @@
 int batch_extract_impl(ssw_ctx* ctx, const ssw_config* cfg, const void* dev_base_rgb, const void* dev_derived_rgb, int u8,
                        size_t n_frames, size_t w, size_t h, size_t k, float* dev_extracted, const float* dev_marks,
                        float* dev_sims);
+
+int base_prune_bound_impl(ssw_ctx* ctx, const ssw_config* cfg, const float* dev_rgb, size_t n_frames, size_t w, size_t h, size_t k,
+                          float* dev_bound);
 
 int trace_base(ssw_ctx* ctx, const ssw_config& c, const void* dev_base_rgb, int u8, size_t w, size_t h, size_t k, const float** y,
                const uint32_t** idx);
diff --git a/spread_spectrum_watermarking_amd/csrc/ssw_internal.hpp b/spread_spectrum_watermarking_amd/csrc/ssw_internal.hpp
--- a/spread_spectrum_watermarking_amd/csrc/ssw_internal.hpp
+++ b/spread_spectrum_watermarking_amd/csrc/ssw_internal.hpp
@@ -78,7 +78,12 @@
 int launch_dct_pair_prep8_cols(hipStream_t st, const float* in, size_t n_frames, size_t w, size_t h,
                                double* r1, double* r2, double* m, double* p);
 enum { FUSE_ROWS_COP = 1, FUSE_COLS = 2 };
-struct FuseCols { int mode = 0; double* cop = nullptr; const double *rot1 = nullptr, *rot2 = nullptr, *rot3 = nullptr; };
+struct FuseCols {
+    int mode = 0; double* cop = nullptr; const double *rot1 = nullptr, *rot2 = nullptr, *rot3 = nullptr;
+    float* energy = nullptr;
+    const unsigned* need = nullptr;
+    int tile_mode = 0;
+};
 struct PairClassDesc { PairClass cls; const double *x1, *x2, *y1, *y2; };
 int launch_dct_pair_gemm_multi_f64(hipStream_t st, bool is_row, bool inverse, int n_classes, const PairClassDesc* desc, float* out,
                                    double* tmp, size_t n_frames, size_t w, size_t h, Epilogue ep, const RgbSink* sink = nullptr,
@@ -96,7 +101,7 @@
                                                 unsigned out_stride, size_t lines);
 size_t dct_pair_split_kpad(size_t len);
 enum { TUNE_EFOLD_MIN, TUNE_EFOLD_INV_MIN, TUNE_EFOLD_COLS_MIN, TUNE_CLASS_TILE, TUNE_DEEP_MIN_ROWS, TUNE_DEEP_MIN_COLS, TUNE_PREP_STAGED,
-       TUNE_MERGE_MAX_LINES, TUNE_BN32, TUNE_BAND_SPLIT, TUNE_FUSE_COLS, TUNE_UPLOAD_BANDS, TUNE_SPECULATE_K, TUNE_PREP_LIGHT, TUNE_LANE_STAGGER, TUNE_DERIVED_FUSED, TUNE_TILE48, TUNE_COUNT };
+       TUNE_MERGE_MAX_LINES, TUNE_BN32, TUNE_BAND_SPLIT, TUNE_FUSE_COLS, TUNE_UPLOAD_BANDS, TUNE_SPECULATE_K, TUNE_PREP_LIGHT, TUNE_LANE_STAGGER, TUNE_DERIVED_FUSED, TUNE_TILE48, TUNE_BASE_PRUNE, TUNE_COUNT };
 long long tuning(int which);
 int launch_prep16_cols_l2(hipStream_t st, const float* in, size_t n_frames, size_t w, size_t h, double* base,
                           const double* rot1, const double* rot2, const double* rot3, bool class_major, bool in_l2, unsigned K16);
@@ -156,6 +161,21 @@
                           size_t cap, const uint32_t* pos, const uint32_t* indices, size_t k, int method, float alpha,
                           float* out);
 
+constexpr unsigned SSW_BASE_PRUNE_TILE = 128;
+struct BasePrune {
+    float* energy = nullptr;
+    unsigned* need = nullptr;
+    unsigned long long* stats = nullptr;
+    size_t k = 0;
+    int ordering = 0;
+    double* work = nullptr;
+    double tile_flop = 0.0, tile_bytes = 0.0, zero_bytes = 0.0;
+};
+float base_prune_gain(size_t w, size_t h, int ordering);
+int launch_base_prune_decide(hipStream_t st, const float* coef, const BasePrune& bp, size_t n_frames, size_t w, size_t h);
+int launch_base_prune_zero(hipStream_t st, float* coef, const unsigned* need, size_t n_frames, size_t w, size_t h);
+int launch_base_prune_bound(hipStream_t st, const float* energy, size_t n_frames, size_t w, size_t h, int ordering, float* out);
+
 struct SelectWorkspace {
     uint32_t* hist = nullptr;
     uint32_t* ctrl = nullptr;
@@ -165,6 +185,7 @@
 };
 size_t select_cand_capacity(size_t k);
 size_t select_max_k();
+void select_ortho_scales(size_t w, size_t h, float s[2][2]);
 int launch_topk(hipStream_t st, const float* coef, size_t n_frames, size_t w, size_t h, int ordering,
                 size_t k, const SelectWorkspace& ws, uint32_t* indices);
 struct ResizeTaps {
@@ -243,6 +264,7 @@
         Buf compact[2];
         Buf gathered;
         Buf prune_u32;
+        Buf base_prune;
         hipStream_t cur = nullptr;
         hipEvent_t done = nullptr;
     };
@@ -257,6 +279,8 @@
     Buf overflow;
     uint64_t pruned_chunks = 0, redone_chunks = 0;
     uint64_t pruned_columns = 0;
+    Buf base_prune_stats;
+    double base_prune_billed[3] = {0.0, 0.0, 0.0};
     hipStream_t copy_stream = nullptr;
     struct FrameStage {
         Buf buf;
diff --git a/spread_spectrum_watermarking_amd/csrc/ssw_lib.hip b/spread_spectrum_watermarking_amd/csrc/ssw_lib.hip
--- a/spread_spectrum_watermarking_amd/csrc/ssw_lib.hip
+++ b/spread_spectrum_watermarking_amd/csrc/ssw_lib.hip
@@ -335,10 +335,12 @@
         release(ln.idx);
         release(ln.gathered);
         release(ln.prune_u32);
+        release(ln.base_prune);
         release_select(ln.sel);
     }
     if (ctx->select_fallbacks) (void)hipFree(ctx->select_fallbacks);
     release(ctx->overflow);
+    release(ctx->base_prune_stats);
     release(ctx->small);
     release(ctx->sort_scratch);
     release(ctx->resize_tmp);
@@ -426,6 +428,8 @@
     SSW_HIP_CHECK(hipStreamSynchronize(ctx->stream));
     if (ctx->aux_stream) SSW_HIP_CHECK(hipStreamSynchronize(ctx->aux_stream));
     SSW_HIP_CHECK(hipMemset(ctx->select_fallbacks, 0, sizeof(uint32_t)));
+    if (ctx->base_prune_stats.p) SSW_HIP_CHECK(hipMemset(ctx->base_prune_stats.p, 0, 8 * sizeof(unsigned long long)));
+    for (double& b : ctx->base_prune_billed) b = 0.0;
     return SSW_OK;
 }
 
@@ -480,6 +484,27 @@
     stats[1] = ctx->redone_chunks;
     stats[2] = ctx->pruned_columns;
     return SSW_OK;
+}
+
+int ssw_ctx_get_base_prune_stats(ssw_ctx* ctx, uint64_t* stats) {
+    if (!ctx || !stats) return SSW_ERR_BAD_ARG;
+    CtxGuard g(ctx);
+    stats[0] = stats[1] = stats[2] = 0;
+    if (!ctx->base_prune_stats.p) return SSW_OK;
+    SSW_HIP_CHECK(hipStreamSynchronize(ctx->stream));
+    if (ctx->aux_stream) SSW_HIP_CHECK(hipStreamSynchronize(ctx->aux_stream));
+    unsigned long long v[4] = {0, 0, 0, 0};
+    SSW_HIP_CHECK(hipMemcpy(v, ctx->base_prune_stats.p, sizeof(v), hipMemcpyDeviceToHost));
+    for (int i = 0; i < 3; ++i) stats[i] = v[i];
+    return SSW_OK;
+}
+
+int ssw_debug_base_prune_bound(ssw_ctx* ctx, const ssw_config* cfg, const float* dev_rgb, size_t n_frames, size_t w, size_t h,
+                               size_t k, float* dev_bound) {
+    if (!ctx || !dev_rgb || !dev_bound) return SSW_ERR_BAD_ARG;
+    SSW_TRY(check_config(cfg));
+    CtxGuard g(ctx);
+    return base_prune_bound_impl(ctx, cfg, dev_rgb, n_frames, w, h, k, dev_bound);
 }
 
 int ssw_ctx_get_select_stats(ssw_ctx* ctx, uint64_t* stats) {
diff --git a/spread_spectrum_watermarking_amd/csrc/ssw_pipeline.hip b/spread_spectrum_watermarking_amd/csrc/ssw_pipeline.hip
--- a/spread_spectrum_watermarking_amd/csrc/ssw_pipeline.hip
+++ b/spread_spectrum_watermarking_amd/csrc/ssw_pipeline.hip
@@ -149,6 +149,17 @@
     used.erase(std::unique(used.begin(), used.end()), used.end());
     for (hipEvent_t e : used) ctx->free_events.push_back(e);
     ctx->tail_event = nullptr; ctx->tail_fresh = false;
+    if (ctx->base_prune_stats.p) {
+        double wk[3] = {0.0, 0.0, 0.0};
+        SSW_HIP_CHECK(hipMemcpy(wk, (const char*)ctx->base_prune_stats.p + 4 * sizeof(unsigned long long), sizeof(wk), hipMemcpyDeviceToHost));
+        if (ctx->timing) {
+            ctx->stage_work[SSW_STAGE_DCT_COL] += wk[0] - ctx->base_prune_billed[0];
+            ctx->stage_bytes[SSW_STAGE_DCT_COL] += wk[1] - ctx->base_prune_billed[1];
+            ctx->stage_work[SSW_STAGE_SELECT] += wk[2] - ctx->base_prune_billed[2];
+            ctx->stage_bytes[SSW_STAGE_SELECT] += wk[2] - ctx->base_prune_billed[2];
+        }
+        for (int i = 0; i < 3; ++i) ctx->base_prune_billed[i] = wk[i];
+    }
     return SSW_OK;
 }
 
@@ -466,6 +477,8 @@
     SSW_TRY(deep_rot(b, true, &rot2, &rot3));
     const size_t n = b.n, w = b.w, h = b.h;
     FuseCols fc;
+    const bool bprune = fused && b.x.base_prune != nullptr;
+    BasePrune bp = bprune ? *b.x.base_prune : BasePrune();
     double pad = 1.0;
     double bytes = b.gemm_bytes(0.0);
     float* out = b.dst;
@@ -484,6 +497,7 @@
             pp.l2_plane = lpad * dct_pair_split_kpad(b.len / 2);
             pad = (double)lpad / (double)(n * h);
             fc = FuseCols{FUSE_ROWS_COP, cop, (const double*)crot1, (const double*)crot2, (const double*)crot3};
+            if (bprune) fc.energy = bp.energy;
             bytes = b.px * 16.0;
             out = nullptr;
         }
@@ -500,7 +514,37 @@
     const double f_main = b.flop(PairClass::O5), f_all = 8.0 * f_main;
     std::array<PairClassDesc, 8> d;
     for (int c = 0; c < 8; ++c) SSW_TRY(deep_desc(b, pp, true, kLevel2Classes[c], d[c]));
+    if (bprune && !b.is_row) {
+        const double tiles = (double)(w / SSW_BASE_PRUNE_TILE);
+        bp.tile_flop = f_all / ((double)n * tiles);
+        bp.tile_bytes = bytes / ((double)n * tiles);
+        bp.zero_bytes = (double)h * SSW_BASE_PRUNE_TILE * 4.0;
+        auto phase = [=](hipStream_t st, int mode) {
+            FuseCols f2 = fc;
+            f2.tile_mode = mode; f2.need = bp.need;
+            return launch_dct_pair_gemm_multi_f64(st, false, false, 8, d.data(), out, nullptr, n, w, h, b.ep, nullptr, nullptr, b.gemm_layout(), &f2);
+        };
+        ch.push_back({false, [=](hipStream_t st) -> int {
+            StageTimer t(ctx, b.st_pass, st, f_all / tiles);
+            t.traffic(bytes / tiles);
+            return phase(st, 1);
+        }});
+        ch.push_back({true, [=](hipStream_t st) -> int {
+            StageTimer t(ctx, SSW_STAGE_SELECT, st, (double)n * ((double)h * SSW_BASE_PRUNE_TILE + (double)w) * 4.0);
+            SSW_TRY(launch_base_prune_decide(st, out, bp, n, w, h));
+            return launch_base_prune_zero(st, out, bp.need, n, w, h);
+        }});
+        ch.push_back({false, [=](hipStream_t st) -> int {
+            StageTimer t(ctx, b.st_pass, st, 0.0);
+            return phase(st, 2);
+        }});
+        return SSW_OK;
+    }
     ch.push_back({false, [=](hipStream_t st) -> int {
+        if (bprune) {
+            SSW_HIP_CHECK(hipMemsetAsync(bp.energy, 0, n * w * sizeof(float), st));
+            untimed_work(ctx);
+        }
         StageTimer t(ctx, b.st_pass, st, f_all * pad, b.p.merge ? b.st_main : -1);
         t.traffic(bytes);
         auto launch = [&](int nc, const PairClassDesc* dd) {
@@ -687,9 +731,10 @@
 }
 
 int build_forward_from_rgb(ssw_ctx* ctx, ssw_ctx::Lane& ws, int precision, const void* rgb, int u8, size_t n, size_t w,
-                           size_t h, float* y, float* i, float* q, float* tmp, Chain& ch) {
+                           size_t h, float* y, float* i, float* q, float* tmp, Chain& ch, const BasePrune* base_prune) {
     const bool f64 = precision == SSW_PRECISION_F64;
     Xform x{SSW_DCT2, precision, n, w, h, y, tmp};
+    x.base_prune = base_prune;
     if (can_fuse_rgb(ctx, f64, w, h, y, tmp, rgb, u8)) {
         x.rgb = rgb; x.rgb_u8 = u8; x.iq_i = i; x.iq_q = q;
         return build_transform(ctx, ws, x, ch);
@@ -1145,6 +1190,21 @@
                                            (const float*)ctx->lane[0].plane[2].p, dev_derived_rgb, u8);
     if (ps.on) SSW_TRY(grow(ctx->overflow, n_chunks * SSW_PRUNE_INFO * sizeof(uint32_t)));
     uint32_t* overflow = (uint32_t*)ctx->overflow.p;
+    const size_t bp_tiles = w / SSW_BASE_PRUNE_TILE;
+    bool base_prune = ctx->prune && tuning(TUNE_BASE_PRUNE) != 0 && f64 && k > 0 && k <= select_max_k() && w % SSW_BASE_PRUNE_TILE == 0 && bp_tiles >= 2 &&
+                      base_prune_gain(w, h, c.ordering) > 0.0f && w >= h &&
+                      can_fuse_rgb(ctx, f64, w, h, (const float*)ctx->lane[0].plane[0].p, (const float*)ctx->lane[0].plane[2].p, dev_base_rgb, u8);
+    for (size_t f0 = 0; base_prune && f0 < n_frames; f0 += chunk) {
+        const size_t n = std::min(chunk, n_frames - f0);
+        const PlanInput in{SSW_DCT2, c.precision, n, w, h, 0, false, true, plan_settings(ctx)};
+        base_prune = n <= plan_frame_limit(plan_settings(ctx), f64, w, h) && plan_pass(in, true, true).strategy == PassStrategy::FusedRows &&
+                     plan_pass(in, false, false).strategy == PassStrategy::FusedCols;
+    }
+    if (base_prune && !ctx->base_prune_stats.p) {
+        SSW_TRY(grow(ctx->base_prune_stats, 8 * sizeof(unsigned long long)));
+        SSW_HIP_CHECK(hipMemsetAsync(ctx->base_prune_stats.p, 0, 8 * sizeof(unsigned long long), ctx->stream));
+        untimed_work(ctx);
+    }
 
     auto full_derived = [&](ssw_ctx::Lane& ws, size_t f0, size_t n, float* yb, float* tmp, uint32_t* idx, Chain& ch) -> int {
         SSW_TRY(grow(ws.plane[1], chunk * plane * sizeof(float)));
@@ -1176,7 +1236,17 @@
         uint32_t* idx = (uint32_t*)ws.idx.p;
         const char* brgb = static_cast<const char*>(dev_base_rgb) + f0 * plane * px_bytes;
         SelectWorkspace* sel = &ws.sel;
-        SSW_TRY(build_forward_from_rgb(ctx, ws, c.precision, brgb, u8, n, w, h, yb, nullptr, nullptr, tmp, ch));
+        BasePrune bp;
+        if (base_prune) {
+            const size_t e_bytes = chunk * w * sizeof(float);
+            SSW_TRY(grow(ws.base_prune, e_bytes + chunk * bp_tiles * sizeof(unsigned)));
+            bp.energy = (float*)ws.base_prune.p;
+            bp.need = (unsigned*)((char*)ws.base_prune.p + e_bytes);
+            bp.stats = (unsigned long long*)ctx->base_prune_stats.p;
+            bp.work = (double*)(bp.stats + 4);
+            bp.k = k; bp.ordering = c.ordering;
+        }
+        SSW_TRY(build_forward_from_rgb(ctx, ws, c.precision, brgb, u8, n, w, h, yb, nullptr, nullptr, tmp, ch, base_prune ? &bp : nullptr));
         if (k > 0)
             ch.push_back({true, [=](hipStream_t st) -> int { return topk(ctx, st, *sel, yb, n, w, h, c.ordering, k, idx); }});
         if (!pruned) return full_derived(ws, f0, n, yb, tmp, idx, ch);
@@ -1218,6 +1288,35 @@
     return SSW_OK;
 }
 
+int base_prune_bound_impl(ssw_ctx* ctx, const ssw_config* cfg, const float* dev_rgb, size_t n_frames, size_t w, size_t h, size_t k,
+                          float* dev_bound) {
+    const ssw_config c = *cfg;
+    const bool f64 = c.precision == SSW_PRECISION_F64;
+    if (w == 0 || h == 0) return SSW_ERR_BAD_DIMS;
+    if (n_frames == 0) return SSW_OK;
+    const size_t plane = w * h, tiles = w / SSW_BASE_PRUNE_TILE;
+    ssw_ctx::Lane& ws = ctx->lane[0];
+    for (int p : {0, 2}) SSW_TRY(grow(ws.plane[p], n_frames * plane * sizeof(float)));
+    const PlanInput in{SSW_DCT2, c.precision, n_frames, w, h, 0, false, true, plan_settings(ctx)};
+    if (!f64 || k == 0 || k >= plane || w % SSW_BASE_PRUNE_TILE != 0 || tiles < 2 || w < h || !(base_prune_gain(w, h, c.ordering) > 0.0f) ||
+        !can_fuse_rgb(ctx, f64, w, h, (const float*)ws.plane[0].p, (const float*)ws.plane[2].p, dev_rgb, SSW_PIX_F32) ||
+        n_frames > plan_frame_limit(plan_settings(ctx), f64, w, h) || plan_pass(in, true, true).strategy != PassStrategy::FusedRows ||
+        plan_pass(in, false, false).strategy != PassStrategy::FusedCols)
+        return SSW_ERR_UNSUPPORTED;
+    const size_t e_bytes = n_frames * w * sizeof(float);
+    SSW_TRY(grow(ws.base_prune, e_bytes + n_frames * tiles * sizeof(unsigned)));
+    BasePrune bp;
+    bp.energy = (float*)ws.base_prune.p;
+    bp.need = (unsigned*)((char*)ws.base_prune.p + e_bytes);
+    bp.k = k; bp.ordering = c.ordering;
+    Chain ch;
+    SSW_TRY(build_forward_from_rgb(ctx, ws, c.precision, dev_rgb, SSW_PIX_F32, n_frames, w, h, (float*)ws.plane[0].p, nullptr, nullptr,
+                                   (float*)ws.plane[2].p, ch, &bp));
+    SSW_TRY(run_serial(ch, ctx->stream));
+    untimed_work(ctx);
+    return launch_base_prune_bound(ctx->stream, bp.energy, n_frames, w, h, c.ordering, dev_bound);
+}
+
 int trace_base(ssw_ctx* ctx, const ssw_config& c, const void* dev_base_rgb, int u8, size_t w, size_t h, size_t k, const float** y,
                const uint32_t** idx) {
     const size_t plane = w * h;
diff --git a/spread_spectrum_watermarking_amd/csrc/tuning.hip b/spread_spectrum_watermarking_amd/csrc/tuning.hip
--- a/spread_spectrum_watermarking_amd/csrc/tuning.hip
+++ b/spread_spectrum_watermarking_amd/csrc/tuning.hip
@@ -35,6 +35,7 @@
     {"lane_stagger", "SSW_LANE_STAGGER", 1},
     {"derived_fused", "SSW_DERIVED_FUSED", 1},
     {"tile48", "SSW_TILE48", 1},
+    {"base_prune", "SSW_BASE_PRUNE", 1},
 };
 
 std::mutex g_tune_lock;
```
